# lostinc0de/sparsemat

Measured on AMD Instinct MI355X. Metric: csr_spmv_effective_hbm_GBps, higher is better.
Workload: dtype f32

## Files before the change

### include/sparsemat_hip.h

```cpp
#ifndef SPARSEMAT_HIP_H
#define SPARSEMAT_HIP_H

#include <stddef.h>
#include <stdint.h>

#ifdef __cplusplus
extern "C" {
#endif

#define SMH_ABI_VERSION 3

enum {
    SMH_OK = 0,
    SMH_ERR_DIM_MISMATCH = 1,
    SMH_ERR_NOT_SQUARE = 2,
    SMH_ERR_INDEX_RANGE = 3,
    SMH_ERR_INVALID = 4,
    SMH_ERR_HIP = 5,
    SMH_ERR_OOM = 6,
    SMH_ERR_NO_DEVICE = 7,
    SMH_ERR_CAPACITY = 8,
    SMH_ERR_COMM = 9
};

// ... 28 lines not shown
int smh_crs_create(smh_dtype dtype, size_t n_rows, size_t n_cols, size_t nnz,
                   const uint32_t *offset_rows, const uint32_t *columns, const void *values,
                   int validate, smh_crs **out);
int smh_crs_create_dev(smh_dtype dtype, size_t n_rows, size_t n_cols, size_t nnz,
                       const uint32_t *offset_rows_dev, const uint32_t *columns_dev,
                       const void *values_dev, int validate, smh_crs **out);
int smh_crs_assemble(smh_dtype dtype, size_t n_ops, const uint32_t *rows, const uint32_t *cols,
                     const void *values, const uint8_t *ops, smh_crs **out);
int smh_crs_assemble_dev(smh_dtype dtype, size_t n_ops, const uint32_t *rows_dev,
                         const uint32_t *cols_dev, const void *values_dev, const uint8_t *ops_dev,
                         smh_crs **out);
int smh_crs_replay(smh_dtype dtype, size_t n_ops, const uint32_t *rows, const uint32_t *cols,
                   const void *values, const uint8_t *ops, smh_crs **out);
int smh_crs_replay_dev(smh_dtype dtype, size_t n_ops, const uint32_t *rows_dev,
                       const uint32_t *cols_dev, const void *values_dev, const uint8_t *ops_dev,
                       smh_crs **out);
int smh_crs_transpose(const smh_crs *a, smh_crs **out);
int smh_last_transpose_route(void);
int smh_crs_column_info(const smh_crs *m, uint32_t *rows, uint32_t *col_ptr, uint32_t *entries);
int smh_crs_column_info_dev(const smh_crs *m, uint32_t *rows_dev, uint32_t *col_ptr_dev,
                            uint32_t *entries_dev);
int smh_crs_prod(const smh_crs *a, const smh_crs *b, smh_crs **out);
int smh_crs_permute(const smh_crs *a, const uint32_t *row_perm, size_t n_row_perm, const uint32_t *col_perm, size_t n_col_perm, smh_crs **out);
int smh_crs_permute_dev(const smh_crs *a, const uint32_t *row_perm_dev, size_t n_row_perm, const uint32_t *col_perm_dev, size_t n_col_perm,
                        smh_crs **out);
int smh_crs_permute_symmetric(const smh_crs *a, const uint32_t *perm, size_t n_perm, smh_crs **out);
int smh_crs_permute_symmetric_dev(const smh_crs *a, const uint32_t *perm_dev, size_t n_perm, smh_crs **out);
int smh_crs_bandwidth(const smh_crs *m, uint32_t *lower_out, uint32_t *upper_out);
int smh_crs_span_fraction(smh_crs *m, double *out);
int smh_crs_rcm(const smh_crs *m, uint32_t *perm_out, size_t *n_components_out, size_t *n_levels_out);
int smh_crs_rcm_dev(const smh_crs *m, uint32_t *perm_out_dev, size_t *n_components_out, size_t *n_levels_out);
int smh_crs_color(const smh_crs *m, uint32_t seed, uint32_t *colors_out, uint32_t *perm_out, size_t *n_colors_out, size_t *n_rounds_out);
int smh_crs_color_dev(const smh_crs *m, uint32_t seed, uint32_t *colors_out_dev, uint32_t *perm_out_dev, size_t *n_colors_out, size_t *n_rounds_out);
int smh_crs_clone(const smh_crs *a, smh_crs **out);
int smh_crs_add(const smh_crs *a, const smh_crs *b, smh_crs **out);
int smh_crs_sub(const smh_crs *a, const smh_crs *b, smh_crs **out);
int smh_crs_add_assign(smh_crs *a, const smh_crs *b);
int smh_crs_sub_assign(smh_crs *a, const smh_crs *b);
int smh_last_add_route(void);
int smh_crs_get(const smh_crs *m, size_t i, size_t j, void *value_out);
int smh_crs_get_many(const smh_crs *m, size_t n, const uint32_t *rows, const uint32_t *cols, void *values_out);
int smh_crs_get_many_dev(const smh_crs *m, size_t n, const uint32_t *rows_dev, const uint32_t *cols_dev, void *values_out_dev);
int smh_crs_apply(smh_crs *m, size_t n_ops, const uint32_t *rows, const uint32_t *cols, const void *values, const uint8_t *ops);
int smh_crs_apply_dev(smh_crs *m, size_t n_ops, const uint32_t *rows_dev, const uint32_t *cols_dev, const void *values_dev,
                      const uint8_t *ops_dev);
int smh_last_apply_route(void);
typedef struct smh_update_plan smh_update_plan;
int smh_update_plan_create(const smh_crs *m, size_t n_ops, const uint32_t *rows, const uint32_t *cols, const uint8_t *ops,
                           smh_update_plan **out);
int smh_update_plan_create_dev(const smh_crs *m, size_t n_ops, const uint32_t *rows_dev, const uint32_t *cols_dev,
                               const uint8_t *ops_dev, smh_update_plan **out);
int smh_update_plan_execute(smh_update_plan *p, smh_crs *m, const void *values, int from_zero);
int smh_update_plan_execute_dev(smh_update_plan *p, smh_crs *m, const void *values_dev, int from_zero);
int smh_update_plan_stats(const smh_update_plan *p, size_t *n_ops, size_t *n_targets, size_t *n_live_ops, size_t *longest_run,
                          size_t *long_run_threshold, size_t *device_bytes);
int smh_update_plan_destroy(smh_update_plan *p);
int smh_crs_eye(smh_dtype dtype, size_t dim, smh_crs **out);
int smh_crs_is_symmetric(const smh_crs *m, int *out);
int smh_crs_is_sorted(const smh_crs *m, int *out);
int smh_crs_sort_rows(smh_crs *m);
int smh_crs_destroy(smh_crs *m);
int smh_crs_update_values(smh_crs *m, const void *values_host);
int smh_crs_download(const smh_crs *m, uint32_t *offset_rows, uint32_t *columns, void *values);
size_t smh_crs_n_rows(const smh_crs *m);
size_t smh_crs_n_cols(const smh_crs *m);
size_t smh_crs_nnz(const smh_crs *m);
size_t smh_crs_orphans(const smh_crs *m);
int smh_crs_dtype(const smh_crs *m);
int smh_crs_max_row_len(const smh_crs *m, uint32_t *out);
int smh_crs_col_range(const smh_crs *m, uint32_t *min_out, uint32_t *max_out);
int smh_crs_scale(smh_crs *m, double a);
int smh_crs_resolved_variant(const smh_crs *m, int *variant_out, int *lanes_out);
int smh_crs_set_vector_lanes(smh_crs *m, int lanes);
int smh_crs_set_stream_xs(smh_crs *m, int mode);
int smh_crs_stream_layout(smh_crs *m, int *coded_out, int *byte_lengths_out, int *small_tiles_out, int *xs_chunks_out);
int smh_crs_stream_value_dict(smh_crs *m, int *n_values_out, void *values_out);
int smh_crs_set_stream_value_dict(smh_crs *m, int mode);
int smh_crs_set_stream_direct(smh_crs *m, int mode);
int smh_crs_stream_direct(smh_crs *m, int *direct_out);
int smh_crs_set_vector_chunks(smh_crs *m, int chunks);
int smh_crs_set_ring(smh_crs *m, int mode);
int smh_crs_ring_entries(smh_crs *m, uint32_t *out);
int smh_crs_ring_column_form(smh_crs *m, int *form_out);
int smh_crs_ring_bands(smh_crs *m, uint32_t *bands_out, uint32_t *intervals_out);
int smh_crs_ring_plan(smh_crs *m, uint32_t *n_blocks_out, size_t *n_phases_out,
                      double *ring_fraction_out, int *active_out, uint32_t *phase_ptr_out,
                      uint32_t *phases_out);
int smh_crs_ring_regular(smh_crs *m, uint32_t *len_out);

int smh_crs_set_colblock_shift(smh_crs *m, uint32_t shift);
int smh_crs_colblock(smh_crs *m, uint32_t *shift_out, size_t *n_blocks_out, int *rows_per_thread_out,
                     double *span_fraction_out, uint32_t *offsets_out, uint32_t *columns_out,
                     void *values_out);

int smh_crs_colfused(smh_crs *m, int *fits_out, uint32_t *shift_out, size_t *n_blocks_out, uint32_t *rows_per_lane_out,
                     size_t *n_tiles_out, uint32_t *tile_rows_out, uint32_t *segments_out, uint8_t *counts_out,
                     uint32_t *columns_out, void *values_out);

int smh_crs_tiled_layout(smh_crs *m, uint32_t *n_slices_out, uint32_t *slice_columns_out, uint32_t *rows_per_block_out,
                         uint32_t *n_row_blocks_out, size_t *copy_entries_out);
int smh_crs_tiled_products(smh_crs *m, size_t *n_products_out);

int smh_crs_tiled_array(smh_crs *m, int which, void *out, size_t capacity_bytes, size_t *bytes_out);

int smh_crs_colsplit(smh_crs *m, int *split_out, uint32_t *min_long_out, size_t *n_long_out, uint32_t *long_rows_out,
                     smh_crs **long_out, smh_crs **short_out);

int smh_crs_spmv(smh_crs *m, const void *x_host, size_t x_len, void *y_host, int variant);
int smh_crs_prepare(smh_crs *m, int variant);
int smh_crs_prepare_stats(smh_crs *m, int variant, double *prepare_ms_out, size_t *derived_bytes_out);
int smh_crs_spmv_dev(smh_crs *m, const void *x_dev, size_t x_len, void *y_dev, int variant,
                     void *stream);
int smh_crs_inner_prod(smh_crs *m, const void *lhs_host, size_t lhs_len, const void *rhs_host,
                       size_t rhs_len, int variant, double *out);
size_t smh_crs_merge_tiles(const smh_crs *m);
size_t smh_crs_merge_tile_items(const smh_crs *m);
int smh_crs_merge_table(smh_crs *m, uint32_t *row_out, uint32_t *nnz_out);

int smh_vec_create(smh_dtype dtype, size_t n, smh_vec **out);
int smh_vec_from_host(smh_dtype dtype, size_t n, const void *host, smh_vec **out);
int smh_vec_wrap_dev(smh_dtype dtype, size_t n, void *dev_ptr, smh_vec **out);
int smh_vec_destroy(smh_vec *v);
int smh_vec_upload(smh_vec *v, const void *host);
int smh_vec_download(const smh_vec *v, void *host);
size_t smh_vec_dim(const smh_vec *v);
int smh_vec_dtype(const smh_vec *v);
void *smh_vec_data(const smh_vec *v);
int smh_vec_copy(smh_vec *dst, const smh_vec *src);
int smh_vec_permute(smh_vec *dst, const smh_vec *src, const uint32_t *perm, size_t n_perm, int inverse);
int smh_vec_permute_dev(smh_vec *dst, const smh_vec *src, const uint32_t *perm_dev, size_t n_perm, int inverse);
int smh_vec_add(smh_vec *x, const smh_vec *y);
int smh_vec_sub(smh_vec *x, const smh_vec *y);
int smh_vec_scale(smh_vec *x, double a);
int smh_vec_axpy(smh_vec *y, double a, const smh_vec *x);
int smh_vec_xpby(smh_vec *p, double b, const smh_vec *r);
int smh_vec_dot(const smh_vec *x, const smh_vec *y, double *out);
int smh_vec_norm_squared(const smh_vec *x, double *out);
int smh_vec_norm(const smh_vec *x, double *out);
int smh_blas_dot_dev(smh_dtype dtype, const void *x_dev, const void *y_dev, size_t n, void *result_dev,
                     void *scratch_dev, void *stream);
size_t smh_blas_dot_scratch_bytes(void);
int smh_blas_axpy_dev(smh_dtype dtype, void *y_dev, const void *a_dev, const void *x_dev, size_t n, void *stream);
int smh_blas_xpby_dev(smh_dtype dtype, void *p_dev, const void *b_dev, const void *r_dev, size_t n, void *stream);
int smh_crs_spmv_vec(smh_crs *m, const smh_vec *x, smh_vec *y, int variant);
int smh_crs_inner_prod_vec(smh_crs *m, const smh_vec *lhs, const smh_vec *rhs, int variant, double *out);

int smh_mvec_create(smh_dtype dtype, size_t n, size_t k, smh_mvec **out);
int smh_mvec_from_host(smh_dtype dtype, size_t n, size_t k, const void *host, smh_mvec **out);
int smh_mvec_upload(smh_mvec *mv, const void *host);
int smh_mvec_download(const smh_mvec *mv, void *host);
int smh_mvec_destroy(smh_mvec *mv);
size_t smh_mvec_dim(const smh_mvec *mv);
size_t smh_mvec_count(const smh_mvec *mv);
size_t smh_mvec_ld(const smh_mvec *mv);
int smh_mvec_dtype(const smh_mvec *mv);
void *smh_mvec_data(const smh_mvec *mv);
int smh_mvec_set_column(smh_mvec *mv, size_t c, const smh_vec *v);
int smh_mvec_get_column(const smh_mvec *mv, size_t c, smh_vec *v);
int smh_mvec_copy(smh_mvec *dst, const smh_mvec *src);
int smh_mvec_add(smh_mvec *x, const smh_mvec *y);
int smh_mvec_sub(smh_mvec *x, const smh_mvec *y);
int smh_mvec_scale(smh_mvec *x, const double *a);
int smh_mvec_dot(const smh_mvec *x, const smh_mvec *y, double *out);
int smh_mvec_norm_squared(const smh_mvec *x, double *out);

int smh_crs_spmv_many(smh_crs *m, const smh_mvec *x, smh_mvec *y);
// ... 211 lines not shown
```

### rust/src/ffi.rs

```rust
#![allow(non_camel_case_types)]
use std::os::raw::{c_char, c_double, c_int, c_void};

#[repr(C)] pub struct smh_crs { _private: [u8; 0] }
#[repr(C)] pub struct smh_vec { _private: [u8; 0] }
#[repr(C)] pub struct smh_update_plan { _private: [u8; 0] }
#[repr(C)] pub struct smh_par { _private: [u8; 0] }
#[repr(C)] pub struct smh_par_vec { _private: [u8; 0] }
#[repr(C)] pub struct smh_comm { _private: [u8; 0] }

pub const SMH_OK: c_int = 0;
pub const SMH_ERR_DIM_MISMATCH: c_int = 1;
pub const SMH_F32: c_int = 0;
pub const SMH_F64: c_int = 1;
pub const SMH_SPMV_AUTO: c_int = 0;
pub const SMH_TRI_LOWER: c_int = 0;
pub const SMH_TRI_UPPER: c_int = 1;
pub const SMH_DIAG_NON_UNIT: c_int = 0;
pub const SMH_DIAG_UNIT: c_int = 1;
pub const SMH_PRECOND_NONE: c_int = 0;
pub const SMH_PRECOND_JACOBI: c_int = 1;
pub const SMH_PRECOND_SGS: c_int = 2;
pub const SMH_PRECOND_ILU: c_int = 3;
pub const SMH_PRECOND_FSAI: c_int = 4;
pub const SMH_INNER_CG: c_int = 0;
// ... 43 lines not shown
                                   iters_out: *mut usize, rr_out: *mut c_double, cycles_out: *mut usize, breakdown_out: *mut c_int) -> c_int;
    pub fn smh_gmres_precond_solve_vec(a: *mut smh_crs, precond: c_int, f: *mut smh_crs, b: *const smh_vec, x: *mut smh_vec,
                                       tol: c_double, iter_max: usize, restart: usize, variant: c_int, check_every: usize,
                                       iters_out: *mut usize, rr_out: *mut c_double, cycles_out: *mut usize, breakdown_out: *mut c_int) -> c_int;
    pub fn smh_bicgstab_precond_solve(a: *mut smh_crs, precond: c_int, f: *mut smh_crs, b_host: *const c_void, b_len: usize,
                                      x_host_inout: *mut c_void, x_len: usize, tol: c_double, iter_max: usize, variant: c_int,
                                      iters_out: *mut usize, rr_out: *mut c_double, breakdown_out: *mut c_int) -> c_int;
    pub fn smh_bicgstab_precond_solve_vec(a: *mut smh_crs, precond: c_int, f: *mut smh_crs, b: *const smh_vec, x: *mut smh_vec,
                                          tol: c_double, iter_max: usize, variant: c_int, check_every: usize,
                                          iters_out: *mut usize, rr_out: *mut c_double, breakdown_out: *mut c_int) -> c_int;
    pub fn smh_crs_trisolve_levels(m: *mut smh_crs, uplo: c_int, n_levels_out: *mut usize, level_of_row_out: *mut u32,
                                   n_launches_out: *mut usize, small_level_rows_out: *mut usize) -> c_int;
    pub fn smh_crs_trisolve(m: *mut smh_crs, uplo: c_int, diag: c_int, b_host: *const c_void, b_len: usize, x_host: *mut c_void,
                            x_len: usize) -> c_int;
    pub fn smh_crs_trisolve_vec(m: *mut smh_crs, uplo: c_int, diag: c_int, b: *const smh_vec, x: *mut smh_vec) -> c_int;
    pub fn smh_crs_sgs_apply_vec(m: *mut smh_crs, r: *const smh_vec, z: *mut smh_vec) -> c_int;
    pub fn smh_pcg_sgs_solve(m: *mut smh_crs, b_host: *const c_void, b_len: usize, x_host_inout: *mut c_void,
                             x_len: usize, tol: c_double, iter_max: usize, variant: c_int,
                             iters_out: *mut usize, rr_out: *mut c_double) -> c_int;
    pub fn smh_pcg_sgs_solve_vec(m: *mut smh_crs, b: *const smh_vec, x: *mut smh_vec, tol: c_double, iter_max: usize,
                                 variant: c_int, check_every: usize, iters_out: *mut usize, rr_out: *mut c_double) -> c_int;
    pub fn smh_crs_ilu0(a: *const smh_crs, f_out: *mut *mut smh_crs, zero_pivot_out: *mut usize) -> c_int;
    pub fn smh_crs_ilu0_refactor(f: *mut smh_crs, a: *const smh_crs, zero_pivot_out: *mut usize) -> c_int;
    pub fn smh_crs_ilu_apply_vec(f: *mut smh_crs, r: *const smh_vec, z: *mut smh_vec) -> c_int;
    pub fn smh_pcg_ilu_solve(a: *mut smh_crs, f: *mut smh_crs, b_host: *const c_void, b_len: usize, x_host_inout: *mut c_void,
                             x_len: usize, tol: c_double, iter_max: usize, variant: c_int,
                             iters_out: *mut usize, rr_out: *mut c_double) -> c_int;
    pub fn smh_pcg_ilu_solve_vec(a: *mut smh_crs, f: *mut smh_crs, b: *const smh_vec, x: *mut smh_vec, tol: c_double, iter_max: usize,
                                 variant: c_int, check_every: usize, iters_out: *mut usize, rr_out: *mut c_double) -> c_int;
    pub fn smh_crs_fsai(a: *const smh_crs, g_out: *mut *mut smh_crs, gt_out: *mut *mut smh_crs, not_spd_out: *mut usize) -> c_int;
    pub fn smh_crs_fsai_apply_vec(g: *mut smh_crs, gt: *mut smh_crs, r: *const smh_vec, z: *mut smh_vec) -> c_int;
    pub fn smh_pcg_fsai_solve(a: *mut smh_crs, g: *mut smh_crs, gt: *mut smh_crs, b_host: *const c_void, b_len: usize, x_host_inout: *mut c_void,
                              x_len: usize, tol: c_double, iter_max: usize, variant: c_int, iters_out: *mut usize, rr_out: *mut c_double) -> c_int;
    pub fn smh_pcg_fsai_solve_vec(a: *mut smh_crs, g: *mut smh_crs, gt: *mut smh_crs, b: *const smh_vec, x: *mut smh_vec, tol: c_double,
                                  iter_max: usize, variant: c_int, check_every: usize, iters_out: *mut usize, rr_out: *mut c_double) -> c_int;
    pub fn smh_crs_fsai_ns(a: *const smh_crs, gl_out: *mut *mut smh_crs, gu_out: *mut *mut smh_crs, singular_out: *mut usize) -> c_int;
    pub fn smh_crs_fsai_ns_apply_vec(gl: *mut smh_crs, gu: *mut smh_crs, r: *const smh_vec, z: *mut smh_vec) -> c_int;
    pub fn smh_gmres_fsai_solve(a: *mut smh_crs, g: *mut smh_crs, gt: *mut smh_crs, b_host: *const c_void, b_len: usize, x_host_inout: *mut c_void,
                                x_len: usize, tol: c_double, iter_max: usize, restart: usize, variant: c_int, iters_out: *mut usize,
                                rr_out: *mut c_double, cycles_out: *mut usize, breakdown_out: *mut c_int) -> c_int;
    pub fn smh_gmres_fsai_solve_vec(a: *mut smh_crs, g: *mut smh_crs, gt: *mut smh_crs, b: *const smh_vec, x: *mut smh_vec, tol: c_double,
                                    iter_max: usize, restart: usize, variant: c_int, check_every: usize, iters_out: *mut usize,
                                    rr_out: *mut c_double, cycles_out: *mut usize, breakdown_out: *mut c_int) -> c_int;
    pub fn smh_bicgstab_fsai_solve(a: *mut smh_crs, g: *mut smh_crs, gt: *mut smh_crs, b_host: *const c_void, b_len: usize, x_host_inout: *mut c_void,
                                   x_len: usize, tol: c_double, iter_max: usize, variant: c_int, iters_out: *mut usize, rr_out: *mut c_double,
                                   breakdown_out: *mut c_int) -> c_int;
    pub fn smh_bicgstab_fsai_solve_vec(a: *mut smh_crs, g: *mut smh_crs, gt: *mut smh_crs, b: *const smh_vec, x: *mut smh_vec, tol: c_double,
                                       iter_max: usize, variant: c_int, check_every: usize, iters_out: *mut usize, rr_out: *mut c_double,
                                       breakdown_out: *mut c_int) -> c_int;
    pub fn smh_crs_cast(a: *const smh_crs, dtype: c_int, out: *mut *mut smh_crs, overflow_out: *mut usize) -> c_int;
    pub fn smh_vec_cast(src: *const smh_vec, dst: *mut smh_vec) -> c_int;
    pub fn smh_refine_solve_vec(a: *mut smh_crs, a_lo: *mut smh_crs, inner: c_int, precond: c_int, f_lo: *mut smh_crs, f2_lo: *mut smh_crs,
                                b: *const smh_vec, x: *mut smh_vec, tol: c_double, outer_max: usize, inner_tol: c_double, inner_iter_max: usize,
                                restart: usize, variant: c_int, variant_lo: c_int, check_every: usize, outer_out: *mut usize,
                                inner_iters_out: *mut usize, rr_out: *mut c_double, code_out: *mut c_int) -> c_int;
    pub fn smh_refine_solve(a: *mut smh_crs, a_lo: *mut smh_crs, inner: c_int, precond: c_int, f_lo: *mut smh_crs, f2_lo: *mut smh_crs,
                            b_host: *const c_void, b_len: usize, x_host_inout: *mut c_void, x_len: usize, tol: c_double, outer_max: usize,
                            inner_tol: c_double, inner_iter_max: usize, restart: usize, variant: c_int, variant_lo: c_int, check_every: usize,
                            outer_out: *mut usize, inner_iters_out: *mut usize, rr_out: *mut c_double, code_out: *mut c_int) -> c_int;
    pub fn smh_crs_inner_prod(m: *mut smh_crs, lhs_host: *const c_void, lhs_len: usize, rhs_host: *const c_void,
                              rhs_len: usize, variant: c_int, out: *mut c_double) -> c_int;
    pub fn smh_crs_assemble(dtype: c_int, n_ops: usize, rows: *const u32, cols: *const u32, values: *const c_void,
                            ops: *const u8, out: *mut *mut smh_crs) -> c_int;
    pub fn smh_crs_replay(dtype: c_int, n_ops: usize, rows: *const u32, cols: *const u32, values: *const c_void,
                          ops: *const u8, out: *mut *mut smh_crs) -> c_int;
    pub fn smh_crs_transpose(a: *const smh_crs, out: *mut *mut smh_crs) -> c_int;
    pub fn smh_crs_set_stream_xs(m: *mut smh_crs, mode: c_int) -> c_int;
    pub fn smh_crs_set_stream_direct(m: *mut smh_crs, mode: c_int) -> c_int;
    pub fn smh_crs_stream_direct(m: *mut smh_crs, direct_out: *mut c_int) -> c_int;
    pub fn smh_crs_stream_layout(m: *mut smh_crs, coded_out: *mut c_int, byte_lengths_out: *mut c_int, small_tiles_out: *mut c_int, xs_chunks_out: *mut c_int) -> c_int;
    pub fn smh_last_transpose_route() -> c_int;
    pub fn smh_crs_orphans(m: *const smh_crs) -> usize;
    pub fn smh_crs_prod(a: *const smh_crs, b: *const smh_crs, out: *mut *mut smh_crs) -> c_int;
    pub fn smh_crs_clone(a: *const smh_crs, out: *mut *mut smh_crs) -> c_int;
    pub fn smh_crs_permute(a: *const smh_crs, row_perm: *const u32, n_row_perm: usize, col_perm: *const u32, n_col_perm: usize,
                           out: *mut *mut smh_crs) -> c_int;
    pub fn smh_crs_permute_dev(a: *const smh_crs, row_perm_dev: *const u32, n_row_perm: usize, col_perm_dev: *const u32,
                               n_col_perm: usize, out: *mut *mut smh_crs) -> c_int;
    pub fn smh_crs_permute_symmetric(a: *const smh_crs, perm: *const u32, n_perm: usize, out: *mut *mut smh_crs) -> c_int;
    pub fn smh_crs_permute_symmetric_dev(a: *const smh_crs, perm_dev: *const u32, n_perm: usize, out: *mut *mut smh_crs) -> c_int;
    pub fn smh_crs_bandwidth(m: *const smh_crs, lower_out: *mut u32, upper_out: *mut u32) -> c_int;
    pub fn smh_crs_span_fraction(m: *mut smh_crs, out: *mut f64) -> c_int;
    pub fn smh_crs_ring_regular(m: *mut smh_crs, len_out: *mut u32) -> c_int;
    pub fn smh_crs_rcm(m: *const smh_crs, perm_out: *mut u32, n_components_out: *mut usize, n_levels_out: *mut usize) -> c_int;
    pub fn smh_crs_rcm_dev(m: *const smh_crs, perm_out_dev: *mut u32, n_components_out: *mut usize, n_levels_out: *mut usize) -> c_int;
    pub fn smh_crs_color(m: *const smh_crs, seed: u32, colors_out: *mut u32, perm_out: *mut u32, n_colors_out: *mut usize, n_rounds_out: *mut usize) -> c_int;
    pub fn smh_crs_color_dev(m: *const smh_crs, seed: u32, colors_out_dev: *mut u32, perm_out_dev: *mut u32, n_colors_out: *mut usize, n_rounds_out: *mut usize) -> c_int;
    pub fn smh_vec_permute(dst: *mut smh_vec, src: *const smh_vec, perm: *const u32, n_perm: usize, inverse: c_int) -> c_int;
    pub fn smh_vec_permute_dev(dst: *mut smh_vec, src: *const smh_vec, perm_dev: *const u32, n_perm: usize, inverse: c_int) -> c_int;
    pub fn smh_crs_add(a: *const smh_crs, b: *const smh_crs, out: *mut *mut smh_crs) -> c_int;
    pub fn smh_crs_sub(a: *const smh_crs, b: *const smh_crs, out: *mut *mut smh_crs) -> c_int;
    pub fn smh_crs_add_assign(a: *mut smh_crs, b: *const smh_crs) -> c_int;
    pub fn smh_crs_sub_assign(a: *mut smh_crs, b: *const smh_crs) -> c_int;
    pub fn smh_last_add_route() -> c_int;
    pub fn smh_crs_get(m: *const smh_crs, i: usize, j: usize, value_out: *mut c_void) -> c_int;
    pub fn smh_crs_get_many(m: *const smh_crs, n: usize, rows: *const u32, cols: *const u32, values_out: *mut c_void) -> c_int;
    pub fn smh_crs_get_many_dev(m: *const smh_crs, n: usize, rows_dev: *const u32, cols_dev: *const u32,
                                values_out_dev: *mut c_void) -> c_int;
    pub fn smh_crs_apply(m: *mut smh_crs, n_ops: usize, rows: *const u32, cols: *const u32, values: *const c_void,
                         ops: *const u8) -> c_int;
    pub fn smh_crs_apply_dev(m: *mut smh_crs, n_ops: usize, rows_dev: *const u32, cols_dev: *const u32,
                             values_dev: *const c_void, ops_dev: *const u8) -> c_int;
    pub fn smh_last_apply_route() -> c_int;
    pub fn smh_last_solve_replays() -> c_int;
    pub fn smh_update_plan_create(m: *const smh_crs, n_ops: usize, rows: *const u32, cols: *const u32, ops: *const u8,
                                  out: *mut *mut smh_update_plan) -> c_int;
    pub fn smh_update_plan_create_dev(m: *const smh_crs, n_ops: usize, rows_dev: *const u32, cols_dev: *const u32,
                                      ops_dev: *const u8, out: *mut *mut smh_update_plan) -> c_int;
    pub fn smh_update_plan_execute(p: *mut smh_update_plan, m: *mut smh_crs, values: *const c_void, from_zero: c_int) -> c_int;
    pub fn smh_update_plan_execute_dev(p: *mut smh_update_plan, m: *mut smh_crs, values_dev: *const c_void, from_zero: c_int) -> c_int;
    pub fn smh_update_plan_stats(p: *const smh_update_plan, n_ops: *mut usize, n_targets: *mut usize, n_live_ops: *mut usize,
                                 longest_run: *mut usize, long_run_threshold: *mut usize, device_bytes: *mut usize) -> c_int;
    pub fn smh_update_plan_destroy(p: *mut smh_update_plan) -> c_int;
    pub fn smh_crs_eye(dtype: c_int, dim: usize, out: *mut *mut smh_crs) -> c_int;
    pub fn smh_crs_is_symmetric(m: *const smh_crs, out: *mut c_int) -> c_int;
    pub fn smh_crs_is_sorted(m: *const smh_crs, out: *mut c_int) -> c_int;
    pub fn smh_crs_column_info(m: *const smh_crs, rows: *mut u32, col_ptr: *mut u32, entries: *mut u32) -> c_int;
    pub fn smh_crs_sort_rows(m: *mut smh_crs) -> c_int;
    pub fn smh_par_create(dtype: c_int, n_blocks: usize, device_ids: *const c_int, n_rows: usize, n_cols: usize,
                          offset_rows: *const u32, columns: *const u32, values: *const c_void, validate: c_int,
                          out: *mut *mut smh_par) -> c_int;
    pub fn smh_par_create_split(dtype: c_int, n_blocks: usize, device_ids: *const c_int, n_rows: usize, n_cols: usize,
                                offset_rows: *const u32, columns: *const u32, values: *const c_void, validate: c_int,
                                split_mode: c_int, out: *mut *mut smh_par) -> c_int;
    pub fn smh_par_split(p: *const smh_par, rows_out: *mut usize) -> c_int;
    pub fn smh_par_set_overlap(p: *mut smh_par, on: c_int) -> c_int;
    pub fn smh_par_interior(p: *const smh_par, local_block: usize, variant: c_int, row_begin: *mut usize, row_end: *mut usize) -> c_int;
    pub fn smh_par_destroy(p: *mut smh_par) -> c_int;
    pub fn smh_par_spmv(p: *mut smh_par, x_host: *const c_void, x_len: usize, y_host: *mut c_void, variant: c_int) -> c_int;
    pub fn smh_par_cg_solve(p: *mut smh_par, b_host: *const c_void, b_len: usize, x_host_inout: *mut c_void, x_len: usize,
                            tol: c_double, iter_max: usize, variant: c_int, iters_out: *mut usize,
                            rr_out: *mut c_double) -> c_int;
    pub fn smh_par_vec_create(p: *mut smh_par, n: usize, out: *mut *mut smh_par_vec) -> c_int;
    pub fn smh_par_vec_destroy(v: *mut smh_par_vec) -> c_int;
    pub fn smh_par_vec_upload(v: *mut smh_par_vec, host: *const c_void) -> c_int;
    pub fn smh_par_vec_download(v: *const smh_par_vec, host: *mut c_void) -> c_int;
    pub fn smh_par_spmv_dev(p: *mut smh_par, x: *const smh_par_vec, y: *mut smh_par_vec, variant: c_int, exchange: c_int) -> c_int;
    pub fn smh_par_exchange(p: *mut smh_par, v: *mut smh_par_vec, mode: c_int) -> c_int;
    pub fn smh_par_synchronize(p: *mut smh_par) -> c_int;
    pub fn smh_par_cg_solve_vec(p: *mut smh_par, b: *const smh_par_vec, x: *mut smh_par_vec, tol: c_double, iter_max: usize,
                                variant: c_int, check_every: usize, iters_out: *mut usize, rr_out: *mut c_double) -> c_int;
    pub fn smh_comm_unique_id(id_out: *mut c_void) -> c_int;
    pub fn smh_comm_create(id: *const c_void, n_ranks: c_int, rank: c_int, out: *mut *mut smh_comm) -> c_int;
    pub fn smh_comm_destroy(c: *mut smh_comm) -> c_int;
    pub fn smh_par_create_rank(comm: *mut smh_comm, n_rows: usize, block: *mut smh_crs, out: *mut *mut smh_par) -> c_int;
    pub fn smh_par_create_rank_split(comm: *mut smh_comm, n_rows: usize, block: *mut smh_crs, row_begin: usize, out: *mut *mut smh_par) -> c_int;
    pub fn smh_crs_n_rows(m: *const smh_crs) -> usize;
    pub fn smh_crs_n_cols(m: *const smh_crs) -> usize;
    pub fn smh_crs_dtype(m: *const smh_crs) -> c_int;
    pub fn smh_crs_nnz(m: *const smh_crs) -> usize;
    pub fn smh_crs_download(m: *const smh_crs, offset_rows: *mut u32, columns: *mut u32, values: *mut c_void) -> c_int;
}
```

### sparsemat_amd/_lib.py

```python
import ctypes as C
import os

_HERE = os.path.dirname(os.path.abspath(__file__))
LIB_PATH = os.environ.get("SPARSEMAT_HIP_LIB") or os.path.join(_HERE, "libsparsemat_hip.so")

SMH_OK = 0
SMH_ERR_DIM_MISMATCH, SMH_ERR_NOT_SQUARE, SMH_ERR_INDEX_RANGE, SMH_ERR_INVALID = 1, 2, 3, 4
SMH_ERR_HIP, SMH_ERR_OOM, SMH_ERR_NO_DEVICE, SMH_ERR_CAPACITY, SMH_ERR_COMM = 5, 6, 7, 8, 9
SMH_F32, SMH_F64 = 0, 1
SMH_TRI_LOWER, SMH_TRI_UPPER = 0, 1
SMH_DIAG_NON_UNIT, SMH_DIAG_UNIT = 0, 1
SMH_PRECOND_NONE, SMH_PRECOND_JACOBI, SMH_PRECOND_SGS, SMH_PRECOND_ILU = 0, 1, 2, 3
PRECONDS = {None: SMH_PRECOND_NONE, "jacobi": SMH_PRECOND_JACOBI, "sgs": SMH_PRECOND_SGS, "ilu": SMH_PRECOND_ILU}
PRECOND_NAMES = tuple(PRECONDS) + ("fsai",)
SMH_INNER_CG, SMH_INNER_BICGSTAB, SMH_INNER_GMRES = 0, 1, 2
INNERS = {"cg": SMH_INNER_CG, "bicgstab": SMH_INNER_BICGSTAB, "gmres": SMH_INNER_GMRES}
SMH_PRECOND_FSAI = 4
REFINE_PRECONDS = dict(PRECONDS, fsai=SMH_PRECOND_FSAI)
UPLO = {"lower": SMH_TRI_LOWER, "upper": SMH_TRI_UPPER}
EXCHANGE_NONE, EXCHANGE_ALLGATHER, EXCHANGE_WINDOW, EXCHANGE_AUTO = 0, 1, 2, 3
EXCHANGES = {"none": EXCHANGE_NONE, "allgather": EXCHANGE_ALLGATHER, "window": EXCHANGE_WINDOW, "halo": EXCHANGE_WINDOW, "auto": EXCHANGE_AUTO}
EXCHANGE_NAMES = {EXCHANGE_NONE: "none", EXCHANGE_ALLGATHER: "allgather", EXCHANGE_WINDOW: "window", EXCHANGE_AUTO: "auto"}
PAR_BACKEND_AUTO, PAR_BACKEND_PEER, PAR_BACKEND_RCCL = 0, 1, 2
PAR_BACKENDS = {"auto": PAR_BACKEND_AUTO, "peer": PAR_BACKEND_PEER, "rccl": PAR_BACKEND_RCCL}
COMM_ID_BYTES = 128
SPMV_AUTO, SPMV_VECTOR, SPMV_MERGE, SPMV_SEQ, SPMV_STREAM, SPMV_COLBLOCK, SPMV_COLFUSED, SPMV_COLSPLIT, SPMV_TILED = 0, 1, 2, 3, 4, 5, 6, 7, 8
VARIANTS = {"auto": SPMV_AUTO, "vector": SPMV_VECTOR, "merge": SPMV_MERGE, "seq": SPMV_SEQ, "stream": SPMV_STREAM,
            "colblock": SPMV_COLBLOCK, "colfused": SPMV_COLFUSED, "colsplit": SPMV_COLSPLIT, "tiled": SPMV_TILED}

_sz = C.c_size_t
_vp = C.c_void_p
_u32p = C.POINTER(C.c_uint32)
_int = C.c_int

SIGNATURES = {
    "smh_abi_version": (_int, []),
    "smh_last_error": (C.c_char_p, []),
    "smh_status_string": (C.c_char_p, [_int]),
    "smh_device_count": (_int, [C.POINTER(_int)]),
    "smh_set_device": (_int, [_int]),
    "smh_device_synchronize": (_int, []),
    "smh_crs_create": (_int, [_int, _sz, _sz, _sz, _vp, _vp, _vp, _int, C.POINTER(_vp)]),
    "smh_crs_create_dev": (_int, [_int, _sz, _sz, _sz, _vp, _vp, _vp, _int, C.POINTER(_vp)]),
    "smh_crs_assemble": (_int, [_int, _sz, _vp, _vp, _vp, _vp, C.POINTER(_vp)]),
    "smh_crs_assemble_dev": (_int, [_int, _sz, _vp, _vp, _vp, _vp, C.POINTER(_vp)]),
    "smh_crs_replay": (_int, [_int, _sz, _vp, _vp, _vp, _vp, C.POINTER(_vp)]),
    "smh_crs_replay_dev": (_int, [_int, _sz, _vp, _vp, _vp, _vp, C.POINTER(_vp)]),
    "smh_crs_transpose": (_int, [_vp, C.POINTER(_vp)]),
    "smh_crs_column_info": (_int, [_vp, _vp, _vp, _vp]),
    "smh_crs_column_info_dev": (_int, [_vp, _vp, _vp, _vp]),
    "smh_crs_prod": (_int, [_vp, _vp, C.POINTER(_vp)]),
    "smh_crs_permute": (_int, [_vp, _vp, _sz, _vp, _sz, C.POINTER(_vp)]),
    "smh_crs_permute_dev": (_int, [_vp, _vp, _sz, _vp, _sz, C.POINTER(_vp)]),
    "smh_crs_permute_symmetric": (_int, [_vp, _vp, _sz, C.POINTER(_vp)]),
    "smh_crs_permute_symmetric_dev": (_int, [_vp, _vp, _sz, C.POINTER(_vp)]),
    "smh_crs_bandwidth": (_int, [_vp, _u32p, _u32p]),
    "smh_crs_span_fraction": (_int, [_vp, C.POINTER(C.c_double)]),
    "smh_crs_rcm": (_int, [_vp, _vp, C.POINTER(_sz), C.POINTER(_sz)]),
    "smh_crs_rcm_dev": (_int, [_vp, _vp, C.POINTER(_sz), C.POINTER(_sz)]),
    "smh_crs_color": (_int, [_vp, C.c_uint32, _vp, _vp, C.POINTER(_sz), C.POINTER(_sz)]),
    "smh_crs_color_dev": (_int, [_vp, C.c_uint32, _vp, _vp, C.POINTER(_sz), C.POINTER(_sz)]),
    "smh_vec_permute": (_int, [_vp, _vp, _vp, _sz, _int]),
    "smh_vec_permute_dev": (_int, [_vp, _vp, _vp, _sz, _int]),
    "smh_crs_clone": (_int, [_vp, C.POINTER(_vp)]),
    "smh_crs_add": (_int, [_vp, _vp, C.POINTER(_vp)]),
    "smh_crs_sub": (_int, [_vp, _vp, C.POINTER(_vp)]),
    "smh_crs_add_assign": (_int, [_vp, _vp]),
    "smh_crs_sub_assign": (_int, [_vp, _vp]),
    "smh_last_add_route": (_int, []),
    "smh_crs_get": (_int, [_vp, _sz, _sz, _vp]),
    "smh_crs_get_many": (_int, [_vp, _sz, _vp, _vp, _vp]),
    "smh_crs_get_many_dev": (_int, [_vp, _sz, _vp, _vp, _vp]),
    "smh_crs_apply": (_int, [_vp, _sz, _vp, _vp, _vp, _vp]),
    "smh_crs_apply_dev": (_int, [_vp, _sz, _vp, _vp, _vp, _vp]),
    "smh_last_apply_route": (_int, []),
    "smh_last_solve_replays": (_int, []),
    "smh_update_plan_create": (_int, [_vp, _sz, _vp, _vp, _vp, _vp]),
    "smh_update_plan_create_dev": (_int, [_vp, _sz, _vp, _vp, _vp, _vp]),
    "smh_update_plan_execute": (_int, [_vp, _vp, _vp, _int]),
    "smh_update_plan_execute_dev": (_int, [_vp, _vp, _vp, _int]),
    "smh_update_plan_stats": (_int, [_vp, _vp, _vp, _vp, _vp, _vp, _vp]),
    "smh_update_plan_destroy": (_int, [_vp]),
    "smh_crs_eye": (_int, [_int, _sz, C.POINTER(_vp)]),
    "smh_crs_is_symmetric": (_int, [_vp, C.POINTER(_int)]),
    "smh_crs_is_sorted": (_int, [_vp, C.POINTER(_int)]),
    "smh_crs_sort_rows": (_int, [_vp]),
    "smh_crs_destroy": (_int, [_vp]),
    "smh_crs_update_values": (_int, [_vp, _vp]),
    "smh_crs_download": (_int, [_vp, _vp, _vp, _vp]),
    "smh_crs_n_rows": (_sz, [_vp]),
    "smh_crs_n_cols": (_sz, [_vp]),
    "smh_crs_nnz": (_sz, [_vp]),
    "smh_crs_orphans": (_sz, [_vp]),
    "smh_crs_dtype": (_int, [_vp]),
    "smh_crs_max_row_len": (_int, [_vp, _u32p]),
    "smh_crs_col_range": (_int, [_vp, _u32p, _u32p]),
    "smh_crs_scale": (_int, [_vp, C.c_double]),
    "smh_crs_resolved_variant": (_int, [_vp, C.POINTER(_int), C.POINTER(_int)]),
    "smh_crs_set_vector_lanes": (_int, [_vp, _int]),
    "smh_crs_set_vector_chunks": (_int, [_vp, _int]),
    "smh_crs_set_ring": (_int, [_vp, _int]),
    "smh_crs_ring_entries": (_int, [_vp, _u32p]),
    "smh_crs_ring_column_form": (_int, [_vp, C.POINTER(_int)]),
    "smh_crs_ring_bands": (_int, [_vp, _u32p, _vp]),
    "smh_crs_ring_regular": (_int, [_vp, _vp]),
    "smh_crs_ring_plan": (_int, [_vp, _u32p, C.POINTER(_sz), C.POINTER(C.c_double), C.POINTER(_int), _vp, _vp]),
    "smh_crs_set_colblock_shift": (_int, [_vp, C.c_uint32]),
    "smh_crs_tiled_layout": (_int, [_vp, _u32p, _u32p, _u32p, _u32p, C.POINTER(_sz)]),
    "smh_crs_tiled_products": (_int, [_vp, C.POINTER(_sz)]),
    "smh_crs_prepare_stats": (_int, [_vp, _int, C.POINTER(C.c_double), C.POINTER(_sz)]),
    "smh_crs_tiled_array": (_int, [_vp, _int, _vp, _sz, C.POINTER(_sz)]),
    "smh_crs_colblock": (_int, [_vp, _u32p, C.POINTER(_sz), C.POINTER(_int), C.POINTER(C.c_double), _vp, _vp, _vp]),
    "smh_crs_colfused": (_int, [_vp, C.POINTER(_int), _u32p, C.POINTER(_sz), _u32p, C.POINTER(_sz), _vp, _vp, _vp, _vp, _vp]),
    "smh_crs_colsplit": (_int, [_vp, C.POINTER(_int), _u32p, C.POINTER(_sz), _vp, C.POINTER(_vp), C.POINTER(_vp)]),
    "smh_crs_spmv": (_int, [_vp, _vp, _sz, _vp, _int]),
    "smh_crs_spmv_dev": (_int, [_vp, _vp, _sz, _vp, _int, _vp]),
    "smh_crs_prepare": (_int, [_vp, _int]),
    "smh_crs_merge_tiles": (_sz, [_vp]),
    "smh_crs_merge_tile_items": (_sz, [_vp]),
    "smh_crs_merge_table": (_int, [_vp, _vp, _vp]),
    "smh_vec_create": (_int, [_int, _sz, C.POINTER(_vp)]),
    "smh_vec_from_host": (_int, [_int, _sz, _vp, C.POINTER(_vp)]),
    "smh_vec_wrap_dev": (_int, [_int, _sz, _vp, C.POINTER(_vp)]),
    "smh_vec_destroy": (_int, [_vp]),
    "smh_vec_upload": (_int, [_vp, _vp]),
    "smh_vec_download": (_int, [_vp, _vp]),
    "smh_vec_dim": (_sz, [_vp]),
    "smh_vec_dtype": (_int, [_vp]),
    "smh_vec_data": (_vp, [_vp]),
    "smh_vec_copy": (_int, [_vp, _vp]),
    "smh_vec_add": (_int, [_vp, _vp]),
    "smh_vec_sub": (_int, [_vp, _vp]),
    "smh_vec_scale": (_int, [_vp, C.c_double]),
    "smh_vec_axpy": (_int, [_vp, C.c_double, _vp]),
    "smh_vec_xpby": (_int, [_vp, C.c_double, _vp]),
    "smh_vec_dot": (_int, [_vp, _vp, C.POINTER(C.c_double)]),
    "smh_vec_norm_squared": (_int, [_vp, C.POINTER(C.c_double)]),
    "smh_vec_norm": (_int, [_vp, C.POINTER(C.c_double)]),
    "smh_blas_dot_dev": (_int, [_int, _vp, _vp, _sz, _vp, _vp, _vp]),
    "smh_blas_dot_scratch_bytes": (_sz, []),
    "smh_blas_axpy_dev": (_int, [_int, _vp, _vp, _vp, _sz, _vp]),
    "smh_blas_xpby_dev": (_int, [_int, _vp, _vp, _vp, _sz, _vp]),
    "smh_crs_spmv_vec": (_int, [_vp, _vp, _vp, _int]),
    "smh_crs_inner_prod": (_int, [_vp, _vp, _sz, _vp, _sz, _int, C.POINTER(C.c_double)]),
    "smh_crs_inner_prod_vec": (_int, [_vp, _vp, _vp, _int, C.POINTER(C.c_double)]),
    "smh_mvec_create": (_int, [_int, _sz, _sz, C.POINTER(_vp)]),
    "smh_mvec_from_host": (_int, [_int, _sz, _sz, _vp, C.POINTER(_vp)]),
    "smh_mvec_upload": (_int, [_vp, _vp]),
    "smh_mvec_download": (_int, [_vp, _vp]),
    "smh_mvec_destroy": (_int, [_vp]),
    "smh_mvec_dim": (_sz, [_vp]),
    "smh_mvec_count": (_sz, [_vp]),
    "smh_mvec_ld": (_sz, [_vp]),
    "smh_mvec_dtype": (_int, [_vp]),
    "smh_mvec_data": (_vp, [_vp]),
    "smh_mvec_set_column": (_int, [_vp, _sz, _vp]),
    "smh_mvec_get_column": (_int, [_vp, _sz, _vp]),
    "smh_mvec_copy": (_int, [_vp, _vp]),
    "smh_mvec_add": (_int, [_vp, _vp]),
    "smh_mvec_sub": (_int, [_vp, _vp]),
    "smh_mvec_scale": (_int, [_vp, C.POINTER(C.c_double)]),
    "smh_mvec_dot": (_int, [_vp, _vp, C.POINTER(C.c_double)]),
    "smh_mvec_norm_squared": (_int, [_vp, C.POINTER(C.c_double)]),
    "smh_crs_spmv_many": (_int, [_vp, _vp, _vp]),
    "smh_crs_spmv_many_dev": (_int, [_vp, _vp, _sz, _vp, _sz, _sz, _vp]),
    "smh_crs_spmv_many_host": (_int, [_vp, _vp, _sz, _sz, _vp]),
    "smh_cg_solve": (_int, [_vp, _vp, _sz, _vp, _sz, C.c_double, _sz, _int, C.POINTER(_sz),
                            C.POINTER(C.c_double)]),
    "smh_cg_solve_vec": (_int, [_vp, _vp, _vp, C.c_double, _sz, _int, _sz, C.POINTER(_sz),
                                C.POINTER(C.c_double)]),
    "smh_cg_solve_many": (_int, [_vp, _vp, _vp, C.c_double, _sz, _sz, C.POINTER(_sz), C.POINTER(C.c_double)]),
    "smh_cg_solve_many_host": (_int, [_vp, _vp, _sz, _sz, _vp, C.c_double, _sz, C.POINTER(_sz), C.POINTER(C.c_double)]),
    "smh_pcg_jacobi_solve": (_int, [_vp, _vp, _sz, _vp, _sz, C.c_double, _sz, _int, C.POINTER(_sz),
                                    C.POINTER(C.c_double)]),
    "smh_crs_trisolve_levels": (_int, [_vp, _int, C.POINTER(_sz), _vp, C.POINTER(_sz), C.POINTER(_sz)]),
    "smh_crs_trisolve": (_int, [_vp, _int, _int, _vp, _sz, _vp, _sz]),
    "smh_crs_trisolve_vec": (_int, [_vp, _int, _int, _vp, _vp]),
    "smh_crs_sgs_apply_vec": (_int, [_vp, _vp, _vp]),
    "smh_pcg_sgs_solve": (_int, [_vp, _vp, _sz, _vp, _sz, C.c_double, _sz, _int, C.POINTER(_sz),
                                 C.POINTER(C.c_double)]),
    "smh_pcg_sgs_solve_vec": (_int, [_vp, _vp, _vp, C.c_double, _sz, _int, _sz, C.POINTER(_sz),
                                     C.POINTER(C.c_double)]),
    "smh_crs_ilu0": (_int, [_vp, C.POINTER(_vp), C.POINTER(_sz)]),
    "smh_crs_ilu0_refactor": (_int, [_vp, _vp, C.POINTER(_sz)]),
    "smh_crs_ilu_apply_vec": (_int, [_vp, _vp, _vp]),
    "smh_pcg_ilu_solve": (_int, [_vp, _vp, _vp, _sz, _vp, _sz, C.c_double, _sz, _int, C.POINTER(_sz),
# ... 174 lines not shown
```

### sparsemat_amd/build.py

```python
import os
import subprocess
import sys

HERE = os.path.dirname(os.path.abspath(__file__))
CSRC = os.path.join(HERE, "csrc")
LIB = os.path.join(HERE, "libsparsemat_hip.so")
SOURCES = ["capi.hip", "crs_forms.hip", "spmv_dispatch.hip", "spmv_vector.hip", "spmv_ring.hip", "spmv_ring2.hip", "spmv_stream.hip", "spmv_stream_xd.hip", "spmv_many.hip", "mvec.hip", "mvec_blas.hip", "cg_many.hip","spmv_colblock.hip", "spmv_colfused.hip", "spmv_colsplit.hip", "spmv_tiled.hip", "spmv_merge.hip", "blas1.hip", "cg.hip", "synth.hip", "assemble.hip", "matops.hip", "matadd.hip", "matupdate.hip", "matplan.hip", "par.hip", "pcg.hip", "trisolve.hip", "bicgstab.hip", "gmres.hip", "pool.hip", "transpose_bucket.hip", "permute.hip", "reorder.hip", "color.hip", "ilu.hip", "fsai.hip", "refine.hip"]
HEADERS = [os.path.join(CSRC, "internal.hpp"), os.path.join(CSRC, "crs_forms.hpp"), os.path.join(CSRC, "mvec_tree.hpp"), os.path.join(CSRC, "ring_col12.hpp"), os.path.join(CSRC, "solver_tree.hpp"), os.path.join(CSRC, "solver_host.hpp"), os.path.join(CSRC, "precond.hpp"), os.path.join(HERE, "..", "include", "sparsemat_hip.h")]
FLAGS = ["-O3", "-std=c++17", "--offload-arch=gfx950", "-fPIC", "-Wall", "-Wno-unused-function",
         "-fno-gpu-rdc", "-ffp-contract=off"]


def hipcc():
    for cand in (os.environ.get("HIPCC"), "/opt/rocm/bin/hipcc", "hipcc"):
        if cand and (os.path.isabs(cand) and os.path.exists(cand) or not os.path.isabs(cand)):
            return cand
    raise RuntimeError("hipcc not found")


def stale():
    if not os.path.exists(LIB):
        return True
    t = os.path.getmtime(LIB)
    deps = [os.path.join(CSRC, s) for s in SOURCES] + HEADERS + [os.path.abspath(__file__)]
    return any(os.path.getmtime(d) > t for d in deps)


def build(force=False, verbose=False, extra_flags=(), out=None, objsuffix=""):
    global LIB
    lib = out or LIB
    if out is None and not force and not stale():
        return LIB
    objdir = os.path.join(HERE, "csrc", "_obj" + objsuffix)
    os.makedirs(objdir, exist_ok=True)
    objs = []
    procs = []
    for s in SOURCES:
        o = os.path.join(objdir, s.replace(".hip", ".o"))
        objs.append(o)
        cmd = [hipcc()] + FLAGS + list(extra_flags) + ["-c", os.path.join(CSRC, s), "-o", o]
        if verbose:
            print(" ".join(cmd))
        procs.append((s, subprocess.Popen(cmd, stdout=subprocess.PIPE, stderr=subprocess.STDOUT)))
    failed = []
    for s, p in procs:
        log, _ = p.communicate()
        if p.returncode != 0:
            failed.append((s, log.decode(errors="replace")))
        elif verbose and log:
            print(log.decode(errors="replace"))
    if failed:
        raise RuntimeError("hipcc failed:\n" + "\n".join("%s:\n%s" % f for f in failed))
    cmd = [hipcc(), "--offload-arch=gfx950", "-shared", "-fPIC", "-o", lib] + objs + ["-L/opt/rocm/lib", "-lrccl", "-Wl,-rpath,/opt/rocm/lib"]
    subprocess.check_call(cmd)
    return lib


if __name__ == "__main__":
    print(build(force="--force" in sys.argv, verbose=True))
```

### sparsemat_amd/csrc/capi.hip

```cpp
#include <atomic>
#include <chrono>
#include <cmath>
#include <cstdarg>
#include <cstdlib>
#include <cstring>
#include <new>
#include <thread>
#include <vector>

#include "crs_forms.hpp"
#include "solver_host.hpp"

namespace smh {

static thread_local char g_err[512] = "";

void set_error(const char *fmt, ...) {
    va_list ap;
    va_start(ap, fmt);
    vsnprintf(g_err, sizeof g_err, fmt, ap);
    va_end(ap);
}

void clear_error() { g_err[0] = 0; }
// ... 976 lines not shown
    SMH_TRY(build_eye(dtype, dim, arrays.off, arrays.col, arrays.val, nullptr));
    return wrap_arrays(dtype, nullptr, dim, dim, dim, arrays, 0, out);
}

int smh_crs_is_symmetric(const smh_crs *m, int *out) {
    if (!m || !out) return fail(SMH_ERR_INVALID, "NULL argument");
    return crs_is_symmetric(m->dtype, m->d_off, m->d_col, m->d_val, m->n_rows, out, m->stream);
}

int smh_crs_is_sorted(const smh_crs *m, int *out) {
    if (!m || !out) return fail(SMH_ERR_INVALID, "NULL argument");
    return crs_is_sorted(m->d_off, m->d_col, m->n_rows, out, m->stream);
}

int smh_crs_sort_rows(smh_crs *m) {
    if (!m) return fail(SMH_ERR_INVALID, "NULL handle");
    SMH_TRY(sort_rows(m->dtype, m->d_off, m->d_col, m->d_val, m->n_rows, m->nnz, m->max_col, m->stream));
    invalidate(m, Changed::Order);
    ++m->epoch;
    return SMH_OK;
}

int smh_crs_destroy(smh_crs *m) {
    if (!m) return SMH_OK;
    if (m->stream) { (void)hipStreamSynchronize(m->stream); (void)hipStreamDestroy(m->stream); }
    if (m->owns) { (void)hipFree(m->d_off); (void)hipFree(m->d_col); (void)hipFree(m->d_val); }
    (void)hipGetLastError();
    delete m;
    return SMH_OK;
}

int smh_crs_update_values(smh_crs *m, const void *values_host) {
    if (!m) return fail(SMH_ERR_INVALID, "NULL argument");
    if (m->nnz && values_host) SMH_HIP(hipMemcpy(m->d_val, values_host, m->nnz * dtype_size(m->dtype), hipMemcpyHostToDevice));
    invalidate(m, Changed::Values);
    if (m->codes.state != Form::NotTried && m->codes.direct) {
        StreamCfg c;
        SMH_TRY(stream_cfg(m, &c, true));
    }
    return SMH_OK;
}

int smh_crs_download(const smh_crs *m, uint32_t *offset_rows, uint32_t *columns, void *values) {
    if (!m) return fail(SMH_ERR_INVALID, "NULL handle");
    SMH_HIP(hipStreamSynchronize(m->stream));
    if (offset_rows) SMH_HIP(hipMemcpy(offset_rows, m->d_off, (m->n_rows + 1) * sizeof(uint32_t), hipMemcpyDeviceToHost));
    if (columns && m->nnz) SMH_HIP(hipMemcpy(columns, m->d_col, m->nnz * sizeof(uint32_t), hipMemcpyDeviceToHost));
    if (values && m->nnz) SMH_HIP(hipMemcpy(values, m->d_val, m->nnz * dtype_size(m->dtype), hipMemcpyDeviceToHost));
    return SMH_OK;
}

size_t smh_crs_n_rows(const smh_crs *m) { return m ? m->n_rows : 0; }
size_t smh_crs_n_cols(const smh_crs *m) { return m ? m->n_cols : 0; }
size_t smh_crs_nnz(const smh_crs *m) { return m ? m->nnz : 0; }
size_t smh_crs_orphans(const smh_crs *m) { return m ? m->orphans : 0; }
int smh_crs_dtype(const smh_crs *m) { return m ? m->dtype : -1; }

int smh_crs_max_row_len(const smh_crs *m, uint32_t *out) {
    if (!m || !out) return fail(SMH_ERR_INVALID, "NULL argument");
    *out = m->max_row_len;
    return SMH_OK;
}

int smh_crs_col_range(const smh_crs *m, uint32_t *min_out, uint32_t *max_out) {
    if (!m) return fail(SMH_ERR_INVALID, "NULL handle");
    if (min_out) *min_out = m->min_col;
    if (max_out) *max_out = m->max_col;
    return SMH_OK;
}

int smh_crs_scale(smh_crs *m, double a) {
    if (!m) return fail(SMH_ERR_INVALID, "NULL handle");
    SMH_TRY(launch_scale_values(m->dtype, m->d_val, m->nnz, a, m->stream));
    if (m->has_first_op) {
        Scratch scr;
        char *d = nullptr;
        SMH_TRY(scr.alloc(&d, 16));
        SMH_HIP(hipMemcpyAsync(d, &m->first_val_bits, 8, hipMemcpyHostToDevice, m->stream));
        SMH_TRY(launch_scale_values(m->dtype, d, 1, a, m->stream));
        SMH_HIP(hipMemcpyAsync(&m->first_val_bits, d, 8, hipMemcpyDeviceToHost, m->stream));
        SMH_HIP(hipStreamSynchronize(m->stream));
    }
    if (m->dict.state == Form::Ready) SMH_TRY(launch_scale_values(m->dtype, m->dict.values.get(), 32, a, m->stream));
    if (m->cb.state == Form::Ready) SMH_TRY(launch_scale_values(m->dtype, m->cb.val.get(), m->nnz, a, m->stream));
    if (m->cf.state == Form::Ready) SMH_TRY(launch_scale_values(m->dtype, m->cf.val.get(), m->nnz, a, m->stream));
    if (m->tiled.state == Form::Ready) SMH_TRY(launch_scale_values(m->dtype, m->tiled.val.get(), (size_t)m->tiled.tot, a, m->stream));
    if (m->split.state == Form::Ready) {
        SMH_TRY(smh_crs_scale(m->split.long_part, a));
        SMH_TRY(smh_crs_scale(m->split.short_part, a));
    }
    SMH_HIP(hipStreamSynchronize(m->stream));
    return SMH_OK;
}

int smh_crs_tiled_layout(smh_crs *m, uint32_t *n_slices_out, uint32_t *slice_columns_out, uint32_t *rows_per_block_out, uint32_t *n_row_blocks_out,
                         size_t *copy_entries_out) {
    if (!m) return fail(SMH_ERR_INVALID, "NULL handle");
    SMH_TRY(tiled_build(m));
    if (n_slices_out) *n_slices_out = m->tiled.n_cb;
    if (slice_columns_out) *slice_columns_out = tiled_slice_columns(m->dtype);
    if (rows_per_block_out) *rows_per_block_out = m->tiled.R;
    if (n_row_blocks_out) *n_row_blocks_out = m->tiled.n_rb;
    if (copy_entries_out) *copy_entries_out = (size_t)m->tiled.tot;
    return SMH_OK;
}

int smh_crs_tiled_products(smh_crs *m, size_t *n_products_out) {
    if (!m) return fail(SMH_ERR_INVALID, "NULL handle");
    SMH_TRY(tiled_build(m));
    if (n_products_out) *n_products_out = (size_t)m->tiled.n_prod;
    return SMH_OK;
}

int smh_crs_tiled_array(smh_crs *m, int which, void *out, size_t capacity_bytes, size_t *bytes_out) {
    if (!m) return fail(SMH_ERR_INVALID, "NULL handle");
    SMH_TRY(tiled_build(m));
    return tiled_array(m, which, out, capacity_bytes, bytes_out);
}

int smh_crs_set_colblock_shift(smh_crs *m, uint32_t shift) {
    if (!m) return fail(SMH_ERR_INVALID, "NULL handle");
    if (shift > 31) return fail(SMH_ERR_INVALID, "column block shift must be 0 (automatic) or 1..31");
    if (shift != m->knobs.cb_forced_shift) invalidate(m, Changed::BlockWidth);
    m->knobs.cb_forced_shift = shift;
    return SMH_OK;
}

int smh_crs_colblock(smh_crs *m, uint32_t *shift_out, size_t *n_blocks_out, int *rows_per_thread_out,
                     double *span_fraction_out, uint32_t *offsets_out, uint32_t *columns_out, void *values_out) {
    if (!m) return fail(SMH_ERR_INVALID, "NULL handle");
    SMH_TRY(ensure_ring_plan(m, false));
    SMH_TRY(ensure_colblock(m));
    if (shift_out) *shift_out = m->cb.shift;
    if (n_blocks_out) *n_blocks_out = m->cb.blocks;
    if (rows_per_thread_out) *rows_per_thread_out = m->cb.rpt;
    if (span_fraction_out) *span_fraction_out = m->span_fraction;
    if (offsets_out)
        SMH_HIP(hipMemcpy(offsets_out, m->cb.off.get(), m->cb.blocks * (m->n_rows + 1) * sizeof(uint32_t), hipMemcpyDeviceToHost));
    if (columns_out && m->nnz) SMH_HIP(hipMemcpy(columns_out, m->cb.col.get(), m->nnz * sizeof(uint32_t), hipMemcpyDeviceToHost));
    if (values_out && m->nnz) SMH_HIP(hipMemcpy(values_out, m->cb.val.get(), m->nnz * dtype_size(m->dtype), hipMemcpyDeviceToHost));
    return SMH_OK;
}

int smh_crs_colfused(smh_crs *m, int *fits_out, uint32_t *shift_out, size_t *n_blocks_out, uint32_t *rows_per_lane_out,
                     size_t *n_tiles_out, uint32_t *tile_rows_out, uint32_t *segments_out, uint8_t *counts_out, uint32_t *columns_out,
                     void *values_out) {
    if (!m) return fail(SMH_ERR_INVALID, "NULL handle");
    SMH_TRY(ensure_colfused(m));
    const size_t tile_rows = (size_t)64 * m->cf.rt, n_tiles = (m->cf.state == Form::Ready) ? m->cf.tiles : 0;
    if (fits_out) *fits_out = (m->cf.state == Form::Ready) ? 1 : 0;
    if (shift_out) *shift_out = m->cf.shift;
    if (n_blocks_out) *n_blocks_out = m->cf.blocks;
    if (rows_per_lane_out) *rows_per_lane_out = m->cf.rt;
    if (n_tiles_out) *n_tiles_out = n_tiles;
    if (m->cf.state != Form::Ready) return SMH_OK;
    SMH_HIP(hipStreamSynchronize(m->stream));
    if (tile_rows_out) SMH_HIP(hipMemcpy(tile_rows_out, m->cf.tile_row.get(), (n_tiles + 1) * sizeof(uint32_t), hipMemcpyDeviceToHost));
    if (segments_out) SMH_HIP(hipMemcpy(segments_out, m->cf.seg.get(), (n_tiles * m->cf.blocks + 1) * sizeof(uint32_t), hipMemcpyDeviceToHost));
    if (counts_out && n_tiles) SMH_HIP(hipMemcpy(counts_out, m->cf.cnt.get(), n_tiles * m->cf.blocks * tile_rows, hipMemcpyDeviceToHost));
    if (columns_out && m->nnz) SMH_HIP(hipMemcpy(columns_out, m->cf.col.get(), m->nnz * sizeof(uint32_t), hipMemcpyDeviceToHost));
    if (values_out && m->nnz) SMH_HIP(hipMemcpy(values_out, m->cf.val.get(), m->nnz * dtype_size(m->dtype), hipMemcpyDeviceToHost));
    return SMH_OK;
}

int smh_crs_colsplit(smh_crs *m, int *split_out, uint32_t *min_long_out, size_t *n_long_out, uint32_t *long_rows_out, smh_crs **long_out,
                     smh_crs **short_out) {
// ... 32 lines not shown
}

int smh_crs_stream_direct(smh_crs *m, int *direct_out) {
    if (!m || !direct_out) return fail(SMH_ERR_INVALID, "NULL argument");
    StreamCfg c;
    SMH_TRY(stream_cfg(m, &c));
    *direct_out = c.direct && c.xs != 0;
    return SMH_OK;
}

int smh_crs_stream_value_dict(smh_crs *m, int *n_values_out, void *values_out) {
    if (!m || !n_values_out) return fail(SMH_ERR_INVALID, "NULL argument");
    StreamCfg c;
    SMH_TRY(stream_cfg(m, &c));
    *n_values_out = c.dict ? (int)m->dict.n : 0;
    if (c.dict && values_out) {
        SMH_HIP(hipMemcpyAsync(values_out, m->dict.values.get(), (size_t)m->dict.n * dtype_size(m->dtype), hipMemcpyDeviceToHost, m->stream));
        SMH_HIP(hipStreamSynchronize(m->stream));
    }
    return SMH_OK;
}

int smh_crs_set_stream_value_dict(smh_crs *m, int mode) {
    if (!m) return fail(SMH_ERR_INVALID, "NULL handle");
    if (mode < -1 || mode > 0) return fail(SMH_ERR_INVALID, "mode must be -1 (automatic: whenever the values allow) or 0 (never)");
    m->knobs.use_stream_vdict = mode;
    return recode_stream(m);
}

int smh_crs_stream_layout(smh_crs *m, int *coded_out, int *byte_lengths_out, int *small_tiles_out, int *xs_chunks_out) {
    if (!m) return fail(SMH_ERR_INVALID, "NULL handle");
    StreamCfg c;
    SMH_TRY(stream_cfg(m, &c));
    if (coded_out) *coded_out = c.code && c.cwin;
    if (byte_lengths_out) *byte_lengths_out = c.len8 && c.tbase;
    if (small_tiles_out) *small_tiles_out = c.small;
    if (xs_chunks_out) *xs_chunks_out = c.xs;
    return SMH_OK;
}

int smh_crs_set_vector_chunks(smh_crs *m, int chunks) {
    if (!m) return fail(SMH_ERR_INVALID, "NULL handle");
    if (chunks < 0 || chunks > 3) return fail(SMH_ERR_INVALID, "chunks per lane must be 0 (automatic), 1, 2 or 3");
    m->knobs.forced_chunks = chunks;
    return SMH_OK;
}

int smh_crs_set_ring(smh_crs *m, int mode) {
    if (!m) return fail(SMH_ERR_INVALID, "NULL handle");
    if (mode < -1 || mode > 1) return fail(SMH_ERR_INVALID, "ring mode must be -1 (auto), 0 (plain K1) or 1 (K1r)");
    m->knobs.use_ring = mode;
    return SMH_OK;
}

int smh_crs_ring_plan(smh_crs *m, uint32_t *n_blocks_out, size_t *n_phases_out, double *ring_fraction_out,
                      int *active_out, uint32_t *phase_ptr_out, uint32_t *phases_out) {
    if (!m) return fail(SMH_ERR_INVALID, "NULL handle");
    SMH_TRY(ensure_ring_plan(m));
    bool ring = false;
    SMH_TRY(vector_uses_ring(m, &ring));
    if (n_blocks_out) *n_blocks_out = m->ring.blocks;
    if (n_phases_out) *n_phases_out = m->ring.n_phases;
    if (ring_fraction_out) *ring_fraction_out = m->ring.fraction;
    if (active_out) *active_out = ring ? 1 : 0;
    if (phase_ptr_out)
        SMH_HIP(hipMemcpy(phase_ptr_out, m->ring.phase_ptr.get(), (m->ring.blocks + 1) * sizeof(uint32_t), hipMemcpyDeviceToHost));
    if (phases_out && m->ring.n_phases)
        SMH_HIP(hipMemcpy(phases_out, m->ring.phases.get(), m->ring.n_phases * sizeof(RingPhase), hipMemcpyDeviceToHost));
    return SMH_OK;
}

int smh_crs_ring_regular(smh_crs *m, uint32_t *len_out) {
    if (!m || !len_out) return fail(SMH_ERR_INVALID, "NULL argument");
    SMH_TRY(ensure_ring_plan(m));
    if (m->ring.n_phases)
        SMH_HIP(hipMemcpy(len_out, m->ring.reg_len.get(), m->ring.n_phases * sizeof(uint32_t), hipMemcpyDeviceToHost));
    return SMH_OK;
}

int smh_crs_ring_column_form(smh_crs *m, int *form_out) {
    if (!m || !form_out) return fail(SMH_ERR_INVALID, "NULL argument");
    bool ring = false;
    SMH_TRY(vector_uses_ring(m, &ring));
    *form_out = !ring ? 0 : m->ring.lo8.get() ? 2 : m->ring.col16.get() ? 1 : 0;
    return SMH_OK;
}

int smh_crs_ring_entries(smh_crs *m, uint32_t *out) {
    if (!m || !out) return fail(SMH_ERR_INVALID, "NULL argument");
    SMH_TRY(ensure_ring_plan(m));
    *out = m->ring.entries;
    return SMH_OK;
}

int smh_crs_ring_bands(smh_crs *m, uint32_t *bands_out, uint32_t *intervals_out) {
    if (!m || !bands_out) return fail(SMH_ERR_INVALID, "NULL argument");
    SMH_TRY(ensure_ring_plan(m));
    *bands_out = m->ring.bands;
    if (intervals_out && m->ring.bands == 4 && m->ring.win.get())
        SMH_HIP(hipMemcpy(intervals_out, m->ring.win.get(), ((m->n_rows + 63) / 64) * 8 * sizeof(uint32_t), hipMemcpyDeviceToHost));
    return SMH_OK;
}

int smh_crs_set_vector_lanes(smh_crs *m, int lanes) {
    if (!m) return fail(SMH_ERR_INVALID, "NULL handle");
    if (lanes != 0 && (lanes < 1 || lanes > 64 || (lanes & (lanes - 1))))
        return fail(SMH_ERR_INVALID, "lanes per row must be 0 or a power of two in 1..64");
    m->knobs.forced_lanes = lanes;
    return SMH_OK;
}

int smh_crs_prepare(smh_crs *m, int variant) {
    if (!m) return fail(SMH_ERR_INVALID, "NULL handle");
    const auto t0 = std::chrono::steady_clock::now();
    const long long b0 = pool_thread_net_bytes();
    int rc = prepare_forms(m, variant);
    if (rc == SMH_OK && m->stream) {
        const hipError_t e = hipStreamSynchronize(m->stream);
        if (e != hipSuccess) rc = hip_fail(e, "hipStreamSynchronize", __FILE__, __LINE__);
    }
    m->prepare_ms += std::chrono::duration<double, std::milli>(std::chrono::steady_clock::now() - t0).count();
    m->prepare_bytes += pool_thread_net_bytes() - b0;
    return rc;
}

int smh_crs_prepare_stats(smh_crs *m, int variant, double *prepare_ms_out, size_t *derived_bytes_out) {
    if (!m) return fail(SMH_ERR_INVALID, "NULL handle");
    SMH_TRY(smh_crs_prepare(m, variant));
    if (prepare_ms_out) *prepare_ms_out = m->create_ms + m->prepare_ms;
    if (derived_bytes_out) *derived_bytes_out = (size_t)(m->prepare_bytes + m->create_bytes > 0 ? m->prepare_bytes + m->create_bytes : 0);
    return SMH_OK;
}

int smh_crs_spmv_dev(smh_crs *m, const void *x_dev, size_t x_len, void *y_dev, int variant, void *stream) {
    if (!m) return fail(SMH_ERR_INVALID, "NULL handle");
    if (m->n_rows && (!y_dev || (m->nnz && !x_dev))) return fail(SMH_ERR_INVALID, "NULL device vector");
    return spmv_enqueue(m, x_dev, x_len, y_dev, variant, (hipStream_t)stream);
}

int smh_crs_spmv(smh_crs *m, const void *x_host, size_t x_len, void *y_host, int variant) {
    if (!m) return fail(SMH_ERR_INVALID, "NULL handle");
    if (m->n_rows == 0) return SMH_OK;
    if (!y_host || (x_len && !x_host)) return fail(SMH_ERR_INVALID, "NULL host vector");
    const size_t vs = dtype_size(m->dtype);
    SMH_TRY(m->stage_x.ensure_cap(x_len * vs));
    SMH_TRY(m->stage_y.ensure_cap(m->n_rows * vs));
    if (x_len) SMH_HIP(hipMemcpyAsync(m->stage_x.d.get(), x_host, x_len * vs, hipMemcpyHostToDevice, m->stream));
    SMH_TRY(spmv_enqueue(m, m->stage_x.d.get(), x_len, m->stage_y.d.get(), variant, m->stream));
    SMH_HIP(hipMemcpyAsync(y_host, m->stage_y.d.get(), m->n_rows * vs, hipMemcpyDeviceToHost, m->stream));
    SMH_HIP(hipStreamSynchronize(m->stream));
    return SMH_OK;
}

size_t smh_crs_merge_tiles(const smh_crs *m) {
    if (!m) return 0;
    return (size_t)(((uint64_t)m->n_rows + m->nnz + kMergeTile - 1) / kMergeTile);
}

size_t smh_crs_merge_tile_items(const smh_crs *) { return kMergeTile; }

int smh_crs_merge_table(smh_crs *m, uint32_t *row_out, uint32_t *nnz_out) {
    if (!m || !row_out || !nnz_out) return fail(SMH_ERR_INVALID, "NULL argument");
    SMH_TRY(ensure_merge_ws(m));
    if (m->merge.n_tiles == 0) { row_out[0] = 0; nnz_out[0] = 0; return SMH_OK; }
    SMH_HIP(hipMemcpy(row_out, m->merge.tile_row.get(), (m->merge.n_tiles + 1) * sizeof(uint32_t), hipMemcpyDeviceToHost));
    SMH_HIP(hipMemcpy(nnz_out, m->merge.tile_nz.get(), (m->merge.n_tiles + 1) * sizeof(uint32_t), hipMemcpyDeviceToHost));
    return SMH_OK;
// ... 366 lines not shown
```

### sparsemat_amd/csrc/crs_forms.hip

```cpp
#include <cstdlib>
#include <cstring>
#include <vector>

#include "crs_forms.hpp"

namespace smh {

void build_ring_plan(size_t n_rows, size_t ring_entries, const uint32_t *cmin, const uint32_t *cmax, size_t n_blocks,
                     uint32_t noring_mode, std::vector<uint32_t> &phase_ptr, std::vector<RingPhase> &phases,
                     double *ring_row_fraction);
void build_ring_plan_banded(size_t n_rows, size_t ring_entries, const uint32_t *win, size_t n_blocks, uint32_t noring_mode,
                            std::vector<uint32_t> &phase_ptr, std::vector<RingPhase> &phases, double *ring_row_fraction);

int ensure_merge_ws(smh_crs *m) {
    if (m->merge.state == Form::Ready) return SMH_OK;
    MergeTable t;
    const uint64_t items = (uint64_t)m->n_rows + (uint64_t)m->nnz;
    t.n_tiles = (size_t)((items + kMergeTile - 1) / kMergeTile);
    if (t.n_tiles) {
        SMH_TRY(t.tile_row.alloc(t.n_tiles + 1));
        SMH_TRY(t.tile_nz.alloc(t.n_tiles + 1));
        SMH_TRY(t.carry_row.alloc(t.n_tiles));
        SMH_TRY(t.carry_val.alloc(t.n_tiles * dtype_size(m->dtype)));
        SMH_TRY(launch_merge_table(m->d_off, m->n_rows, m->nnz, t.n_tiles, t.tile_row.get(), t.tile_nz.get(), m->stream));
        SMH_HIP(hipStreamSynchronize(m->stream));
    }
    t.state = Form::Ready;
    m->merge = std::move(t);
    return SMH_OK;
}

int ensure_ring_plan(smh_crs *m, bool with_bands) {
    if (m->ring.state == Form::Ready && (!with_bands || m->ring.bands_tried)) return SMH_OK;
    m->ring = RingPlan();
    RingPlan p;
    p.bands_tried = with_bands;
    const size_t n_tiles = (m->n_rows + 63) / 64;
    int cus = 256;
    hipDeviceProp_t prop;
    if (hipGetDeviceProperties(&prop, m->device) == hipSuccess && prop.multiProcessorCount > 0) cus = prop.multiProcessorCount;
    unsigned per_cu = 6;
    if (const char *e = getenv("SMH_RING_BLOCKS_PER_CU")) {
        const int v = atoi(e);
        if (v >= 1 && v <= 64) per_cu = (unsigned)v;
    }
    unsigned blocks = per_cu * (unsigned)cus;
    blocks = (blocks + 7u) & ~7u;
    std::vector<uint32_t> cmin(n_tiles), cmax(n_tiles);
    if (n_tiles) {
        Scratch scr;
        uint32_t *d_min = nullptr, *d_max = nullptr;
        SMH_TRY(scr.alloc(&d_min, n_tiles));
        SMH_TRY(scr.alloc(&d_max, n_tiles));
        SMH_TRY(read_back(d_min, cmin.data(), n_tiles, m->stream, [&](uint32_t *) -> int {
            SMH_TRY(launch_tile_span(m->d_off, m->d_col, m->n_rows, n_tiles, d_min, d_max, m->stream));
            SMH_HIP(hipMemcpyAsync(cmax.data(), d_max, n_tiles * sizeof(uint32_t), hipMemcpyDeviceToHost, m->stream));
            return SMH_OK;
        }));
    }
    double span_fraction = 0.0;
    {
        double acc = 0.0;
        size_t used = 0;
        for (size_t t = 0; t < n_tiles; ++t)
            if (cmin[t] <= cmax[t]) { acc += (double)(cmax[t] - cmin[t]) + 1.0; ++used; }
        span_fraction = used && m->n_cols ? acc / (double)used / (double)m->n_cols : 0.0;
    }
    std::vector<uint32_t> phase_ptr;
    std::vector<RingPhase> phases;
    uint32_t noring_mode = 0;
    if (const char *e = getenv("SMH_GATHER_NT")) noring_mode = atoi(e) ? 2u : 0u;
    build_ring_plan(m->n_rows, kRingEntries, cmin.data(), cmax.data(), blocks, noring_mode, phase_ptr, phases,
                    &p.fraction);
    p.entries = kRingEntries;
    const char *wide_env = getenv("SMH_RING_WIDE");
    if (m->dtype == SMH_F32 && p.fraction < 0.5 && !(wide_env && atoi(wide_env) == 0)) {
        std::vector<uint32_t> phase_ptr_w;
        std::vector<RingPhase> phases_w;
        double frac_w = 0.0;
        const unsigned blocks_w = ((blocks / 2) + 7u) & ~7u;
        build_ring_plan(m->n_rows, kRingEntriesWide, cmin.data(), cmax.data(), blocks_w, noring_mode, phase_ptr_w, phases_w, &frac_w);
        if (frac_w >= 0.5) {
            phase_ptr.swap(phase_ptr_w);
            phases.swap(phases_w);
            p.fraction = frac_w;
            p.entries = kRingEntriesWide;
            blocks = blocks_w;
// ... 133 lines not shown
int ensure_split(smh_crs *m) {
    if (m->split.state != Form::NotTried) return SMH_OK;
    SMH_TRY(columns_within_n_cols(m, "row-length split"));
    m->split.state = Form::Refused;
    if (m->no_split || m->n_rows == 0 || m->nnz == 0) return SMH_OK;
    RowSplit sp;
    size_t nnz_long = 0;
    uint32_t *rows = nullptr;
    CrsArrays long_part, short_part;
    SMH_TRY(build_colsplit(m->dtype, m->d_off, m->d_col, m->d_val, m->n_rows, m->nnz, kSplitMinLong, &sp.n_long, &nnz_long, &rows, &long_part.off,
                           &long_part.col, &long_part.val, &short_part.off, &short_part.col, &short_part.val, m->stream));
    sp.rows.reset(rows);
    const bool worth = sp.n_long > 0 && sp.n_long * 4 <= m->n_rows && nnz_long * 4 >= m->nnz;
    if (!worth) return SMH_OK;
    auto part = [&](size_t n_rows, size_t nnz, CrsArrays &arrays, uint32_t shift, smh_crs **out) -> int {
        SMH_TRY(wrap_arrays(m->dtype, nullptr, n_rows, m->n_cols, nnz, arrays, 0, out));
        (*out)->no_split = true;
        (*out)->knobs.cb_forced_shift = shift;
        return SMH_OK;
    };
    SMH_TRY(part(sp.n_long, nnz_long, long_part, 18u, &sp.long_part));
    SMH_TRY(part(m->n_rows, m->nnz - nnz_long, short_part, 19u, &sp.short_part));
    SMH_TRY(sp.y.alloc(sp.n_long * dtype_size(m->dtype)));
    SMH_HIP(hipStreamCreateWithFlags(&sp.side, hipStreamNonBlocking));
    SMH_HIP(hipEventCreateWithFlags(&sp.fork, hipEventDisableTiming));
    SMH_HIP(hipEventCreateWithFlags(&sp.join, hipEventDisableTiming));
    sp.state = Form::Ready;
    m->split = std::move(sp);
    return SMH_OK;
}
RowSplit::~RowSplit() {
    (void)smh_crs_destroy(long_part);
    (void)smh_crs_destroy(short_part);
    rows.reset();
    y.reset();
    if (side) { (void)hipStreamSynchronize(side); (void)hipStreamDestroy(side); }
    if (fork) (void)hipEventDestroy(fork);
    if (join) (void)hipEventDestroy(join);
}

static int ensure_stream_codes(smh_crs *m) {
    if (m->codes.state != Form::NotTried) return SMH_OK;
    StreamCodes c;
    c.state = Form::Refused;
    const size_t n_tiles = (m->n_rows + kStreamRows - 1) / kStreamRows;
    if (n_tiles && m->nnz) {
        uint32_t h_count = 0;
        SMH_TRY(c.cwin.alloc(n_tiles * 8));
        SMH_TRY(read_back(&h_count, 1, m->stream, [&](uint32_t *d_count) {
            return launch_stream_windows(m->d_off, m->d_col, m->n_rows, c.cwin.get(), d_count, m->stream);
        }));
        if ((size_t)h_count == n_tiles) c.state = Form::Ready;
        else c.cwin.reset();
    }
    if (c.state == Form::Ready) {
        const size_t n_out = ((m->nnz + 3) & ~size_t(3)) + 4;
        SMH_TRY(c.code.alloc(n_out));
        SMH_HIP(hipMemsetAsync(c.code.get(), 0, n_out * sizeof(uint16_t), m->stream));
        SMH_TRY(launch_stream_codes(m->d_off, m->d_col, c.cwin.get(), m->n_rows, c.code.get(), m->stream));
        if (m->max_row_len <= 255u) {
            SMH_TRY(c.len8.alloc(n_tiles * kStreamRows));
            SMH_TRY(c.tbase.alloc(n_tiles + 1));
            SMH_TRY(launch_stream_len8(m->d_off, m->n_rows, c.len8.get(), c.tbase.get(), m->stream));
            uint32_t h_xs[2] = {0xFFFFFFFFu, 0};
            SMH_TRY(read_back(h_xs, 2, m->stream, [&](uint32_t *d_xs) { return launch_stream_xs_stats(c.cwin.get(), n_tiles, d_xs, m->stream); }));
            c.xs_chunks = h_xs[0];
            c.xs_end = h_xs[1];
            unsigned long long h_odd = 0;
            SMH_TRY(read_back(&h_odd, 1, m->stream, [&](unsigned long long *d_odd) {
                return launch_stream_odd_rows(c.len8.get(), n_tiles * kStreamRows, d_odd, m->stream);
            }));
            c.odd_rows = (uint64_t)h_odd;
        }
        SMH_HIP(hipStreamSynchronize(m->stream));
    }
    m->codes = std::move(c);
    return SMH_OK;
}

static void drop_ring_col12(smh_crs *m) {
    m->ring.lo8.reset();
    m->ring.hdr.reset();
    m->ring.escapes.reset();
}
static int ensure_ring_col12(smh_crs *m, bool forced, bool *use) {
    RingPlan &r = m->ring;
    *use = forced || r.c12 == Form::Ready;
    if (r.c12 != Form::NotTried && (!*use || r.lo8.get())) return SMH_OK;
    Scratch scr;
    uint32_t *jobs = nullptr;
    unsigned long long *d_counts = nullptr, h_counts[2] = {0, 0};
    SMH_TRY(scr.alloc(&jobs, 2 * r.n_phases));
    SMH_TRY(scr.alloc(&d_counts, 2));
    SMH_TRY(read_back(d_counts, h_counts, 2, m->stream, [&](unsigned long long *d) {
        return launch_col12_count(m->d_off, m->d_col, m->nnz, r.phases.get(), r.n_phases, jobs, d, m->stream);
    }));
    r.c12_chunks = h_counts[0];
    r.c12_escapes = h_counts[1];
    r.c12 = r.c12_escapes * 1024ull <= r.c12_chunks ? Form::Ready : Form::Refused;
    *use = forced || r.c12 == Form::Ready;
    if (!*use) return SMH_OK;
    const size_t n_chunks_out = ((m->nnz + 3) >> 2) + 1;
    DevArray<uint8_t> lo8;
    DevArray<uint16_t> hdr;
    DevArray<uint32_t> escapes;
    SMH_TRY(lo8.alloc(n_chunks_out * 4));
    SMH_TRY(hdr.alloc(n_chunks_out));
    SMH_TRY(escapes.alloc(2 * (size_t)(r.c12_escapes ? r.c12_escapes : 1)));
    SMH_TRY(launch_col12_encode(m->d_col, m->nnz, jobs, r.n_phases, n_chunks_out, lo8.get(), hdr.get(), escapes.get(), d_counts, m->stream));
    SMH_HIP(hipStreamSynchronize(m->stream));
    r.lo8 = std::move(lo8);
    r.hdr = std::move(hdr);
    r.escapes = std::move(escapes);
    return SMH_OK;
}

int vector_uses_ring(smh_crs *m, bool *out) {
    *out = false;
    if (m->knobs.use_ring == 0 || m->n_rows == 0) return SMH_OK;
    SMH_TRY(ensure_ring_plan(m));
    *out = true;
    int want = m->knobs.use_col16;
    if (const char *e = getenv("SMH_RING_COL16")) want = atoi(e) ? 1 : 0;
    int want12 = m->knobs.use_col12;
    if (const char *e = getenv("SMH_RING_COL12")) want12 = strcmp(e, "auto") == 0 ? -1 : (atoi(e) ? 1 : 0);
    const bool can12 = m->dtype == SMH_F32 && m->ring.bands == 1 && m->ring.entries == (unsigned)kRingEntries && m->nnz > 0;
    bool use12 = can12 && (want12 == 1 || (want12 < 0 && want < 0 && m->ring.fraction >= 0.25));
    if (use12) SMH_TRY(ensure_ring_col12(m, want12 == 1, &use12));
    if (!use12) drop_ring_col12(m);
    const bool use16 = m->ring.bands == 4 || want == 1 || (want < 0 && m->ring.fraction >= 0.25);
    if (use16 && !m->ring.col16.get() && m->nnz) {
        const size_t n_out = ((m->nnz + 3) & ~size_t(3)) + 4;
        DevArray<uint16_t> col16;
        SMH_TRY(col16.alloc(n_out));
        if (m->ring.bands == 4) {
            SMH_HIP(hipMemsetAsync(col16.get(), 0, n_out * sizeof(uint16_t), m->stream));
            SMH_TRY(launch_ring_band_codes(m->d_off, m->d_col, m->ring.win.get(), m->n_rows, m->ring.entries / 4, col16.get(), m->stream));
        } else {
            SMH_TRY(launch_narrow_columns(m->d_col, m->nnz, col16.get(), n_out, m->stream));
        }
        SMH_HIP(hipStreamSynchronize(m->stream));
        m->ring.col16 = std::move(col16);
    } else if (!use16) {
        m->ring.col16.reset();
    }
    return SMH_OK;
}

void invalidate(smh_crs *m, Changed what) {
    m->cb = ColBlock();
    m->cf = ColFused();
    m->split = RowSplit();
    m->tiled = Tiled();
    if (what == Changed::Values) m->dict.state = Form::NotTried;
    if (what == Changed::Order) {
        m->codes = StreamCodes();
        m->ring.col16.reset();
        drop_ring_col12(m);
        m->ring.c12 = Form::NotTried;
        m->tri[0] = TriSchedule();
        m->tri[1] = TriSchedule();
    }
}

static int stream_rpt(const smh_crs *m) {
    int want = m->knobs.stream_rows_per_thread;
    if (const char *e = getenv("SMH_STREAM_RPT")) want = atoi(e);
    return want == 2 && m->max_tile512_entries <= (uint32_t)kStreamCap ? 2 : 1;
}

int stream_cfg(smh_crs *m, StreamCfg *c, bool recode) {
    *c = StreamCfg();
    c->rpt = stream_rpt(m);
    c->single_pass = m->have_stats && (c->rpt == 2 || m->max_tile_entries <= (uint32_t)kStreamCap);
    const char *c16_env = getenv("SMH_STREAM_C16");
    if (!(c16_env && atoi(c16_env) == 0) && c->rpt == 1 && c->single_pass) {
        const bool first = m->codes.state == Form::NotTried;
        SMH_TRY(ensure_stream_codes(m));
        if (first) recode = true;
        c->code = m->codes.code.get();
        c->cwin = m->codes.code.get() ? m->codes.cwin.get() : nullptr;
        static const bool l8_off = getenv("SMH_STREAM_L8") && atoi(getenv("SMH_STREAM_L8")) == 0;
        if (c->cwin && !l8_off) { c->len8 = m->codes.len8.get(); c->tbase = m->codes.tbase.get(); }
        static const bool small_off = getenv("SMH_STREAM_SMALL") && atoi(getenv("SMH_STREAM_SMALL")) == 0;
        c->small = !small_off && m->have_stats && m->max_tile_entries <= (uint32_t)kStreamCapSmall;
        static const bool xs_off = getenv("SMH_STREAM_XS") && atoi(getenv("SMH_STREAM_XS")) == 0;
        const bool forced = m->knobs.use_stream_xs == 1;
        const size_t x_bytes = m->n_cols * dtype_size(m->dtype);
        const bool on2 = forced || x_bytes >= ((size_t)1 << 20), on4 = forced || (x_bytes >= ((size_t)8 << 20) && m->dtype == SMH_F32);
        c->xs = (xs_off || m->knobs.use_stream_xs == 0 || !c->small || !c->len8) ? 0
                : (m->codes.xs_chunks <= 2u * kBlock && on2) ? 2
                : (m->codes.xs_chunks <= 4u * kBlock && on4) ? 4 : 0;
        static const bool xd_off = getenv("SMH_STREAM_XD") && atoi(getenv("SMH_STREAM_XD")) == 0;
        const bool want_direct = c->code && c->xs != 0 && !xd_off && m->knobs.use_stream_direct != 0 &&
                                 (m->knobs.use_stream_direct == 1 || 2 * m->codes.odd_rows >= (uint64_t)m->n_rows);
        static const bool vd_off = getenv("SMH_STREAM_VDICT") && atoi(getenv("SMH_STREAM_VDICT")) == 0;
        bool want_vdict = want_direct && !vd_off && m->knobs.use_stream_vdict != 0 && m->dict.state != Form::Refused;
        bool dict_rebuilt = false;
        if (recode && want_vdict && m->dict.state == Form::NotTried) {
            if (!m->dict.values.get()) SMH_TRY(m->dict.values.alloc(32 * dtype_size(m->dtype)));
            SMH_HIP(hipDeviceSynchronize());
            uint32_t n_vals = 0;
            SMH_TRY(stream_value_dict(m->dtype, m->d_val, m->nnz, m->dict.values.get(), &n_vals, m->stream));
            m->dict.n = n_vals;
            m->dict.state = n_vals ? Form::Ready : Form::Refused;
            dict_rebuilt = true;
        }
        want_vdict = want_vdict && m->dict.state == Form::Ready && m->dict.n <= stream_value_dict_capacity(c->xs);
        const bool form_ok = want_direct == m->codes.direct && want_vdict == m->codes.vdict && (!want_vdict || m->codes.vdict_xs == c->xs) &&
                             !(dict_rebuilt && (want_vdict || m->codes.vdict));
        if (recode && c->code && !form_ok) {
            SMH_HIP(hipDeviceSynchronize());
            if (want_direct)
                SMH_TRY(launch_stream_stage_codes(m->d_off, m->d_col, m->codes.cwin.get(), m->n_rows, (uint32_t)dtype_size(m->dtype), m->codes.code.get(), m->stream));
            else
                SMH_TRY(launch_stream_codes(m->d_off, m->d_col, m->codes.cwin.get(), m->n_rows, m->codes.code.get(), m->stream));
            if (want_vdict)
                SMH_TRY(launch_stream_value_codes(m->dtype, m->d_val, m->nnz, m->dict.values.get(), m->dict.n, c->xs, m->codes.code.get(), m->stream));
            SMH_HIP(hipStreamSynchronize(m->stream));
            m->codes.direct = want_direct;
            m->codes.vdict = want_vdict;
            m->codes.vdict_xs = want_vdict ? c->xs : 0;
        }
        c->direct = c->code && m->codes.direct;
        c->dict = c->direct && m->codes.vdict ? m->dict.values.get() : nullptr;
        c->dict_high = c->dict && stream_value_dict_high(m->dtype, m->dict.n, m->codes.vdict_xs);
    }
    return SMH_OK;
}

int recode_stream(smh_crs *m) {
    if (m->codes.state == Form::NotTried) return SMH_OK;
    StreamCfg c;
    return stream_cfg(m, &c, true);
}

}
// ... 1 lines not shown
```

### sparsemat_amd/csrc/crs_forms.hpp

```cpp
#pragma once
#include "internal.hpp"

namespace smh {

void clear_error();
int wrap_arrays(int dtype, const ::smh_crs *like, size_t n_rows, size_t n_cols, size_t nnz, CrsArrays &arrays, int validate, ::smh_crs **out);

template <typename U, typename F> int read_back(U *d, U *host, size_t count, hipStream_t s, F &&launch) {
    SMH_TRY(launch(d));
    SMH_HIP(hipMemcpyAsync(host, d, count * sizeof(U), hipMemcpyDeviceToHost, s));
    SMH_HIP(hipStreamSynchronize(s));
    return SMH_OK;
}
template <typename U, typename F> int read_back(U *host, size_t count, hipStream_t s, F &&launch) {
    Scratch scr;
    U *d = nullptr;
    SMH_TRY(scr.alloc(&d, count));
    return read_back(d, host, count, s, launch);
}

extern const uint32_t kSplitMinLong;
int ensure_merge_ws(::smh_crs *m);
int ensure_ring_plan(::smh_crs *m, bool with_bands = true);
int ensure_colblock(::smh_crs *m);
int ensure_colfused(::smh_crs *m);
int ensure_split(::smh_crs *m);
int vector_uses_ring(::smh_crs *m, bool *out);
enum class Changed { Values, Order, BlockWidth };
void invalidate(::smh_crs *m, Changed what);
struct StreamCfg {
    int rpt = 1;
    bool single_pass = false;
    const uint16_t *code = nullptr;
    const uint32_t *cwin = nullptr;
    const uint8_t *len8 = nullptr;
    const uint32_t *tbase = nullptr;
    bool small = false;
    int xs = 0;
    bool direct = false;
    const void *dict = nullptr;
    bool dict_high = false;
};
int stream_cfg(::smh_crs *m, StreamCfg *c, bool recode = false);
int recode_stream(::smh_crs *m);

extern const size_t kColblockMinXBytes;
uint32_t cb_shift_for(const ::smh_crs *m);
uint32_t cf_shift_for(const ::smh_crs *m);
size_t blocks_for(size_t n_cols, uint32_t shift);
int auto_lanes(const ::smh_crs *m);
int resolve_variant(const ::smh_crs *m, int variant);
int prepare_forms(::smh_crs *m, int variant);
int spmv_inner_prod(::smh_crs *m, const void *d_lhs, const void *d_rhs, size_t rhs_len, int variant, void *scratch, void *res);

}
```

### sparsemat_amd/csrc/internal.hpp

```cpp
#pragma once
#include <hip/hip_runtime.h>

#include <cstddef>
#include <cstdint>
#include <cstdio>
#include <cstring>
#include <string>
#include <utility>
#include <vector>

#include "../../include/sparsemat_hip.h"

namespace smh {

void set_error(const char *fmt, ...);
int fail(int status, const char *fmt, ...);
int hip_fail(hipError_t e, const char *what, const char *file, int line);

extern __thread bool t_thread_counted;
extern __thread int t_solve_replays;
void count_thread();
inline void note_thread() { if (!t_thread_counted) count_thread(); }
bool capture_enter();
void capture_leave();
// ... 342 lines not shown
                      bool reverse_rows, bool all_set, bool repeats_adjacent, size_t *n_rows_out, size_t *n_cols_out, size_t *nnz_out,
                      uint32_t **off_out, uint32_t **col_out, void **val_out, hipStream_t s);
int expand_rows(const uint32_t *off, size_t n_rows, uint32_t *rows_out, hipStream_t s);
int column_lists_bucketed(const uint32_t *off, const uint32_t *col, size_t n_rows, size_t n_cols, size_t nnz, uint32_t max_col, uint32_t *col_ptr,
                          uint32_t *entries, bool *done, hipStream_t s);
int transpose_bucketed(int dtype, const uint32_t *off, const uint32_t *col, const void *val, size_t n_rows, size_t nnz, uint32_t max_col,
                       uint32_t **off_out, uint32_t **col_out, void **val_out, size_t *n_rows_out, size_t *n_cols_out, bool *done, hipStream_t s);
int append_to_row(int dtype, uint32_t *off, uint32_t **col, void **val, size_t n_rows, size_t *nnz, size_t row, uint32_t column,
                  const void *value_host, hipStream_t s);
int column_info(const uint32_t *off, const uint32_t *col, size_t n_rows, size_t n_cols, size_t nnz, uint32_t max_col, uint32_t *rows,
                uint32_t *col_ptr, uint32_t *entries, hipStream_t s);
int sort_rows(int dtype, const uint32_t *off, uint32_t *col, void *val, size_t n_rows, size_t nnz, uint32_t max_col,
              hipStream_t s);
int crs_is_sorted(const uint32_t *off, const uint32_t *col, size_t n_rows, int *out, hipStream_t s);
int crs_is_symmetric(int dtype, const uint32_t *off, const uint32_t *col, const void *val, size_t n_rows, int *out, hipStream_t s);
int prod_crs(int dtype, const uint32_t *a_off, const uint32_t *a_col, const void *a_val, size_t a_rows, size_t a_nnz, uint32_t a_max_col,
             const uint32_t *b_off, const uint32_t *b_col, const void *b_val, size_t b_rows, size_t *n_rows_out, size_t *n_cols_out,
             size_t *nnz_out, uint32_t **off_out, uint32_t **col_out, void **val_out, hipStream_t s);
struct AddOperand {
    const uint32_t *off = nullptr, *col = nullptr;
    const void *val = nullptr;
    size_t n_rows = 0, n_cols = 0, nnz = 0, orphans = 0;
    uint32_t max_row_len = 0, max_col = 0;
};
struct AddResult {
    size_t n_rows = 0, n_cols = 0, nnz = 0;
    CrsArrays arrays;
    int route = 0;
    bool values_only = false;
};
int add_crs(int dtype, bool subtract, const AddOperand &a, const AddOperand &b, bool in_place, bool alias, bool force_general, AddResult *res,
            hipStream_t s);
struct UpdMatrix {
    const uint32_t *off = nullptr, *col = nullptr;
    void *val = nullptr;
    size_t n_rows = 0, n_cols = 0, nnz = 0, orphans = 0;
    uint32_t max_row_len = 0;
};
struct UpdResult {
    size_t n_rows = 0, n_cols = 0, nnz = 0;
    CrsArrays arrays;
    int route = 0;
    bool values_only = false;
};
int crs_get_many(int dtype, const UpdMatrix &m, size_t n, const uint32_t *rows, const uint32_t *cols, void *values_out, hipStream_t s);
int crs_apply(int dtype, const UpdMatrix &m, size_t n, const uint32_t *rows, const uint32_t *cols, const void *vals, const uint8_t *ops,
              bool force_general, UpdResult *res, hipStream_t s);
int build_eye(int dtype, size_t dim, uint32_t *off, uint32_t *col, void *val, hipStream_t s);
int validate_permutation(const uint32_t *perm, size_t n, uint32_t *first, const char *what, hipStream_t s);
int permute_crs(int dtype, const uint32_t *a_off, const uint32_t *a_col, const void *a_val, size_t n_rows, size_t nnz, const uint32_t *row_perm,
                const uint32_t *col_inv, CrsArrays *out, hipStream_t s);
int launch_vec_permute(int dtype, void *dst, const void *src, const uint32_t *perm, size_t n, bool inverse, hipStream_t s);
int launch_bandwidth(const uint32_t *off, const uint32_t *col, size_t n_rows, uint32_t *d_out2, hipStream_t s);
int rcm_order(const uint32_t *off, const uint32_t *col, size_t n, size_t nnz, uint32_t *perm_out, size_t *n_components, size_t *n_levels, hipStream_t s);
int symmetrised_pattern(const uint32_t *off, const uint32_t *col, size_t n, size_t nnz, Scratch &scr, uint32_t **adj_off_out, uint32_t **adj_col_out,
                        hipStream_t s);
int color_order(const uint32_t *off, const uint32_t *col, size_t n, size_t nnz, uint32_t seed, uint32_t *colors_out, uint32_t *perm_out, size_t *n_colors,
                size_t *n_rounds, hipStream_t s);
constexpr uint32_t kPlanLongRun = 64;
struct UpdPlan {
    size_t n_ops = 0, n_targets = 0, n_live = 0, longest_run = 0, n_short = 0, device_bytes = 0;
    DevArray<uint32_t> pos;
    DevArray<uint32_t> off;
    DevArray<uint32_t> tgt;
    DevArray<uint32_t> setbits;
};
int crs_plan_targets(const UpdMatrix &m, size_t n, const uint32_t *rows, const uint32_t *cols, uint32_t *key_out, uint32_t *src_out,
                     uint64_t *n_absent_out, hipStream_t s);
int plan_build(size_t n, const uint32_t *key, const uint32_t *src, const uint8_t *ops, UpdPlan *plan, hipStream_t s);
int plan_execute(int dtype, const UpdPlan &plan, const void *values, void *m_val, bool from_zero, hipStream_t s);
struct RingPhase {
    uint32_t row_begin, row_end;
    uint32_t load_lo, load_hi;
    uint32_t use_ring;
    uint32_t band_lo[3], band_hi[3];
};
constexpr int kRingPhaseWords = 11;
int launch_tile_span(const uint32_t *off, const uint32_t *col, size_t n_rows, size_t n_tiles, uint32_t *cmin,
                     uint32_t *cmax, hipStream_t s);
struct RingCol12 {
    const uint8_t *lo8 = nullptr;
    const uint16_t *hdr = nullptr;
    const uint32_t *escapes = nullptr;
};
int launch_spmv_ring2(int dtype, int lanes, int chunks, const uint32_t *off, const uint32_t *col, const uint16_t *col16, const RingCol12 &c12,
                      const void *val, const void *x, void *y, size_t n_rows, size_t nnz, bool padded, unsigned n_blocks,
                      const uint32_t *phase_ptr, const RingPhase *phases, unsigned ring_entries, unsigned bands,
                      hipStream_t s, void *dot_partials = nullptr ,
                      unsigned block_begin = 0, unsigned block_end = ~0u ,
                      const uint32_t *reg_len = nullptr );
int launch_ring_regular(const uint32_t *off, const RingPhase *phases, size_t n_phases, uint32_t *reg_len, hipStream_t s);
int launch_tile_intervals(const uint32_t *off, const uint32_t *col, size_t n_rows, size_t tile_rows, size_t max_width,
                          uint32_t *win, uint32_t *d_count, hipStream_t s);
int launch_ring_band_codes(const uint32_t *off, const uint32_t *col, const uint32_t *win, size_t n_rows, uint32_t S,
                           uint16_t *code, hipStream_t s);
int launch_narrow_columns(const uint32_t *col, size_t nnz, uint16_t *col16, size_t n_out, hipStream_t s);
int launch_col12_count(const uint32_t *off, const uint32_t *col, size_t nnz, const RingPhase *phases, size_t n_phases, uint32_t *jobs,
                       unsigned long long *counts, hipStream_t s);
int launch_col12_encode(const uint32_t *col, size_t nnz, const uint32_t *jobs, size_t n_phases, size_t n_chunks_out, uint8_t *lo8,
                        uint16_t *hdr, uint32_t *escapes, unsigned long long *counts, hipStream_t s);
struct CrsStats {
    uint32_t max_row_len;
    uint32_t max_col;
    uint32_t min_col_inv;
    uint32_t bad;
};
int launch_crs_stats(const uint32_t *off, const uint32_t *col, size_t n_rows, size_t nnz, CrsStats *d_stats,
                     hipStream_t s);
void tiled_geometry(size_t n_rows, size_t n_cols, size_t nnz, int dtype, uint32_t *n_cb, uint32_t *rows_per_block, uint32_t *n_rb);
int tiled_build(::smh_crs *m);
uint32_t tiled_slice_columns(int dtype);
int columns_within_n_cols(const ::smh_crs *m, const char *what);
int tiled_array(::smh_crs *m, int which, void *out, size_t capacity_bytes, size_t *bytes_out);
int launch_spmv_tiled(::smh_crs *m, const void *x, size_t x_len, void *y, hipStream_t s);
size_t spmv_fused_dot_partials(::smh_crs *m, size_t x_len, int variant, bool any_lhs = false);
int spmv_enqueue(::smh_crs *m, const void *x, size_t x_len, void *y, int variant, hipStream_t s, void *dot_partials = nullptr,
                 const void *dot_lhs = nullptr);
int spmv_rows_granularity(::smh_crs *m, int variant, size_t *gran_out);
int spmv_enqueue_rows(::smh_crs *m, const void *x, size_t x_len, void *y, int variant, hipStream_t s, size_t row0, size_t row1,
                      void *dot_partials = nullptr, const void *dot_lhs = nullptr);
int spmv_enqueue_rows_short(::smh_crs *m, const void *x, size_t x_len, void *y, int variant, hipStream_t s, size_t row0, size_t row1);
enum class Ew { Add, Sub, Scale, Axpy, Xpby, RSubInto };
int launch_ew(int dtype, Ew op, void *x, const void *y, size_t n, double a, const void *a_dev, hipStream_t s);
int launch_dot(int dtype, const void *x, const void *y, size_t n, void *partials, void *result_dev,
               hipStream_t s, const uint32_t *rows_off = nullptr);
int launch_fold2(int dtype, const void *in, size_t count, void *partials, void *result_dev, hipStream_t s);
int launch_scale_values(int dtype, void *v, size_t n, double a, hipStream_t s);
int ensure_tri_schedule(::smh_crs *m, int uplo);
int tri_lanes(const ::smh_crs *m);
int trisolve_enqueue(::smh_crs *m, int uplo, int diag, bool scale_rhs, const void *b, void *x, const uint32_t *active, hipStream_t s);
int ilu_check(const ::smh_crs *a, const char *what);

template <typename T>
struct CgScalars {
    T rr, rr_prev, pap, alpha, beta;
    uint32_t converged;
    uint32_t active;
    uint32_t entered;
    uint32_t pad_;
    uint64_t iters;
    uint64_t iter_max;
    double tol;
};
template <template <typename> class S, typename T> constexpr bool scalars_like_cg_t() {
    return sizeof(S<T>) == sizeof(CgScalars<T>) && offsetof(S<T>, rr) == offsetof(CgScalars<T>, rr) &&
           offsetof(S<T>, converged) == offsetof(CgScalars<T>, converged) && offsetof(S<T>, iters) == offsetof(CgScalars<T>, iters);
}
template <template <typename> class S> constexpr bool scalars_like_cg() { return scalars_like_cg_t<S, float>() && scalars_like_cg_t<S, double>(); }
size_t cg_scalars_bytes(int dtype);
void cg_read_scalars(int dtype, const void *host_copy, int *converged, uint64_t *iters, double *rr);

template <typename Body>
int solve_in_batches(int dtype, hipStream_t s, size_t iter_max, size_t check_every, Body &&body, const void *d_sc, void *h_sc, int *converged,
                     size_t *iters, double *rr, bool capture = true) {
    Graph graph;
    GraphExec exec;
    t_solve_replays = 0;
    const bool may_capture = capture && iter_max > check_every && capture_enter();
    if (may_capture && hipStreamBeginCapture(s, hipStreamCaptureModeThreadLocal) == hipSuccess) {
        int crc = SMH_OK;
        for (size_t i = 0; i < check_every && crc == SMH_OK; ++i) crc = body();
        const hipError_t ce = graph.end_capture(s);
        if (crc != SMH_OK || ce != hipSuccess || !graph.get() || exec.instantiate(graph.get()) != hipSuccess)
            (void)hipGetLastError();
    } else {
        (void)hipGetLastError();
    }
    if (may_capture) capture_leave();
    auto poll = [&]() -> int {
        SMH_HIP(hipMemcpyAsync(h_sc, d_sc, cg_scalars_bytes(dtype), hipMemcpyDeviceToHost, s));
        SMH_HIP(hipStreamSynchronize(s));
        uint64_t it64 = 0;
        cg_read_scalars(dtype, h_sc, converged, &it64, rr);
        *iters = (size_t)it64;
        return SMH_OK;
    };
    auto run = [&]() -> int {
        size_t launched = 0;
        while (launched < iter_max) {
            size_t batch = iter_max - launched < check_every ? iter_max - launched : check_every;
            if (exec.get()) {
                SMH_HIP(hipGraphLaunch(exec.get(), s));
                ++t_solve_replays;
                batch = check_every;
            } else {
                for (size_t i = 0; i < batch; ++i) SMH_TRY(body());
            }
            launched += batch;
            SMH_TRY(poll());
            if (*converged) break;
        }
        if (iter_max == 0) SMH_TRY(poll());
        return SMH_OK;
    };
    const int rc = run();
    if (rc != SMH_OK) (void)hipStreamSynchronize(s);
    return rc;
}

enum class Form {
    NotTried,
    Ready,
    Refused,
};
struct MergeTable {
    Form state = Form::NotTried;
    size_t n_tiles = 0;
    DevArray<uint32_t> tile_row, tile_nz, carry_row;
    DevArray<char> carry_val;
};
struct RingPlan {
    Form state = Form::NotTried;
    bool bands_tried = false;
    unsigned blocks = 0;
    double fraction = 0.0;
    unsigned entries = kRingEntries;
    unsigned bands = 1;
    size_t n_phases = 0;
    DevArray<uint32_t> phase_ptr;
    DevArray<RingPhase> phases;
    DevArray<uint32_t> reg_len;
    bool reg_applies = false;
    DevArray<uint32_t> win;
    DevArray<uint16_t> col16;
    Form c12 = Form::NotTried;
    uint64_t c12_chunks = 0, c12_escapes = 0;
    DevArray<uint8_t> lo8;
    DevArray<uint16_t> hdr;
    DevArray<uint32_t> escapes;
};
struct StreamCodes {
    Form state = Form::NotTried;
    DevArray<uint32_t> cwin;
    DevArray<uint16_t> code;
    DevArray<uint8_t> len8;
    DevArray<uint32_t> tbase;
    uint32_t xs_chunks = 0xFFFFFFFFu, xs_end = 0;
    uint64_t odd_rows = 0;
    bool direct = false;
    bool vdict = false;
    int vdict_xs = 0;
};
struct StreamDict {
    Form state = Form::NotTried;
    uint32_t n = 0;
    DevArray<char> values;
};
struct ColBlock {
    Form state = Form::NotTried;
    uint32_t shift = 0;
    size_t blocks = 0;
    int rpt = 1;
    bool single_pass = false;
    DevArray<uint32_t> off, col;
    DevArray<char> val;
};
struct ColFused {
    Form state = Form::NotTried;
    uint32_t shift = 0, rt = 0;
    size_t blocks = 0, tiles = 0;
    DevArray<uint32_t> seg, col, tile_row;
    DevArray<uint8_t> cnt;
    DevArray<char> val;
};
struct RowSplit {
    Form state = Form::NotTried;
    ::smh_crs *long_part = nullptr, *short_part = nullptr;
    DevArray<uint32_t> rows;
    DevArray<char> y;
    size_t n_long = 0;
    hipStream_t side = nullptr;
    hipEvent_t fork = nullptr, join = nullptr;
    RowSplit() = default;
    RowSplit(RowSplit &&o) noexcept { swap(o); }
    RowSplit &operator=(RowSplit &&o) noexcept {
        RowSplit old(std::move(*this));
        swap(o);
        return *this;
    }
    ~RowSplit();
    void swap(RowSplit &o) noexcept {
        std::swap(state, o.state); std::swap(long_part, o.long_part); std::swap(short_part, o.short_part);
        std::swap(rows, o.rows); std::swap(y, o.y); std::swap(n_long, o.n_long);
        std::swap(side, o.side); std::swap(fork, o.fork); std::swap(join, o.join);
    }
};
struct Tiled {
    Form state = Form::NotTried;
    uint32_t n_cb = 0, n_rb = 0, R = 0;
    uint64_t tot = 0;
    DevArray<char> val, prod;
    DevArray<uint16_t> code, row;
    DevArray<uint32_t> tstart;
    DevArray<uint32_t> rbstart;
    DevArray<uint32_t> cptr;
    DevArray<char> chunk;
    uint32_t n_chunks = 0, max_slice_chunks = 0;
    bool dups = false;
    uint64_t n_prod = 0;
};
struct TriSchedule {
    Form state = Form::NotTried;
    size_t n_levels = 0;
    uint64_t first_no_diag = ~0ull;
    DevArray<uint32_t> rows;
    DevArray<uint32_t> level_ptr;
    DevArray<uint32_t> level;
    DevArray<uint32_t> diagpos;
    struct Launch { uint32_t level_begin, level_end, row_begin, row_end; bool small; };
    std::vector<Launch> launches;
};
constexpr uint32_t kTriSmallRows = 128;
constexpr uint32_t kTriSmallBlock = 1024;
struct StageBuf {
    DevArray<char> d;
    size_t cap = 0;
    int ensure_cap(size_t bytes) {
        if (cap >= bytes && d.get()) return SMH_OK;
        cap = 0;
        const size_t want = bytes < 256 ? 256 : bytes;
        SMH_TRY(d.alloc(want));
        cap = want;
        return SMH_OK;
    }
};
struct Knobs {
    int forced_lanes = 0;
    int forced_chunks = 0;
    int stream_rows_per_thread = 0;
    uint32_t cb_forced_shift = 0;
    int use_ring = -1;
    int use_stream_xs = -1;
    int use_stream_direct = -1;
    int use_stream_vdict = -1;
    int use_col16 = -1;
    int use_col12 = -1;
};

}

namespace smh {
uint64_t next_crs_id();
}
struct smh_crs {
    uint64_t id = smh::next_crs_id();
    uint64_t epoch = 0;
    int dtype = SMH_F32;
    int device = 0;
    size_t n_rows = 0, n_cols = 0, nnz = 0;
    size_t orphans = 0;
    bool has_first_op = false;
    uint32_t first_row = 0, first_col = 0;
    uint64_t first_val_bits = 0;
    uint32_t *d_off = nullptr;
    uint32_t *d_col = nullptr;
    void *d_val = nullptr;
    bool owns = true;
    bool no_split = false;
    hipStream_t stream = nullptr;
    uint32_t max_row_len = 0;
    uint32_t max_col = 0;
    uint32_t min_col = 0;
    uint32_t max_tile_entries = 0;
    uint32_t max_tile512_entries = 0;
    bool have_stats = false;
    double span_fraction = 0.0;
    smh::Knobs knobs;
    smh::MergeTable merge;
    smh::RingPlan ring;
    smh::StreamCodes codes;
    smh::StreamDict dict;
    smh::ColBlock cb;
    smh::ColFused cf;
    smh::RowSplit split;
    smh::Tiled tiled;
    smh::TriSchedule tri[2];
    smh::StageBuf stage_x, stage_y;
    double create_ms = 0.0, prepare_ms = 0.0;
    long long create_bytes = 0, prepare_bytes = 0;
};

struct smh_vec {
    int dtype = SMH_F32;
    int device = 0;
    size_t n = 0;
    void *d = nullptr;
    bool owns = true;
};

struct smh_mvec {
    int dtype = SMH_F32;
    int device = 0;
    size_t n = 0, k = 0, ld = 0;
    smh::DevArray<char> d;
};

namespace smh {
int cg_solve_many(::smh_crs *m, const ::smh_mvec *b, ::smh_mvec *x, double tol, size_t iter_max, size_t check_every, size_t *iters_out,
                  double *rr_out);
}

#ifndef SMH_POOL_IMPL
#define hipMalloc(p, n) (::smh::note_thread(), ::smh::pool_malloc((void **)(p), (n)))
#define hipFree(p) (::smh::note_thread(), ::smh::pool_free((void *)(p)))
#endif
```

### sparsemat_amd/csrc/spmv_dispatch.hip

```cpp
#include <cstdlib>
#include <cstring>

#include "crs_forms.hpp"

namespace smh {

static double mean_row(const smh_crs *m) { return m->n_rows ? (double)m->nnz / (double)m->n_rows : 0.0; }

static int mean_lanes(const smh_crs *m) {
    const double mean = mean_row(m);
    const double need = mean < 16.0 ? mean + 3.0 : mean;
    int lanes = 1;
    while (lanes < 64 && 4.0 * lanes < need) lanes <<= 1;
    return lanes;
}

int auto_lanes(const smh_crs *m) {
    if (m->knobs.forced_lanes) return m->knobs.forced_lanes;
    const double mean = mean_row(m);
    int lanes = mean_lanes(m);
    if (m->knobs.use_ring != 0) {
        if (mean >= 128.0) lanes = 16;
        else if (lanes > 32) lanes = 32;
        if (mean > 32.0 && m->ring.state == Form::Ready && m->ring.fraction < 0.5) lanes = 8;
    }
    return lanes;
}

static int auto_chunks(const smh_crs *m) {
    const int lanes = auto_lanes(m);
    if (m->knobs.forced_chunks) {
        if (lanes == 1) return m->knobs.forced_chunks;
        if (lanes == 2) return m->knobs.forced_chunks > 2 ? 2 : m->knobs.forced_chunks;
        return 1;
    }
    return 1;
}

uint32_t cb_shift_for(const smh_crs *m) { return m->knobs.cb_forced_shift ? m->knobs.cb_forced_shift : 19u; }
uint32_t cf_shift_for(const smh_crs *m) { return m->knobs.cb_forced_shift ? m->knobs.cb_forced_shift : 18u; }
size_t blocks_for(size_t n_cols, uint32_t shift) {
    const uint64_t w = 1ull << shift;
    const uint64_t b = ((uint64_t)n_cols + w - 1) / w;
    return (size_t)(b ? b : 1);
}
const size_t kColblockMinXBytes = 4u << 20;
static bool wants_colblock(const smh_crs *m) {
    const size_t b = blocks_for(m->n_cols, cb_shift_for(m));
    return m->n_cols * dtype_size(m->dtype) >= kColblockMinXBytes && m->span_fraction > 0.25 && b >= 2 && b <= 128;
}

static bool tiled_fits(const smh_crs *m, double min_tile = 32.0) {
    static const bool tiled_off = getenv("SMH_TILED") && atoi(getenv("SMH_TILED")) == 0;
    if (tiled_off || m->tiled.state == Form::Refused) return false;
    uint32_t n_cb = 0, R = 0, n_rb = 0;
    tiled_geometry(m->n_rows, m->n_cols, m->nnz, m->dtype, &n_cb, &R, &n_rb);
    const double tile = (double)m->nnz / (double)n_cb / (double)n_rb;
    return tile >= min_tile && (double)(n_rb + 1) * (double)n_cb * 4.0 <= (double)(1u << 30);
}

int resolve_variant(const smh_crs *m, int variant) {
    if (variant != SMH_SPMV_AUTO) return variant;
    if (wants_colblock(m)) {
        static const bool fused_off = getenv("SMH_COLBLOCK_FUSED") && atoi(getenv("SMH_COLBLOCK_FUSED")) == 0;
        if (fused_off || m->cf.state == Form::Refused || blocks_for(m->n_cols, cf_shift_for(m)) > 255) return SMH_SPMV_COLBLOCK;
        const double mean = mean_row(m);
        const double similar = 2.0 * mean + 8.0 > 128.0 ? 2.0 * mean + 8.0 : 128.0;
        if ((double)m->max_row_len <= similar) {
            const size_t blocks = blocks_for(m->n_cols, cf_shift_for(m));
            const bool pays = m->dtype == SMH_F32 ? tiled_fits(m)
                              : m->no_split       ? false
                                                  : tiled_fits(m, blocks >= 24 ? 12.0 : 32.0);
            if (pays) return SMH_SPMV_TILED;
            return SMH_SPMV_COLFUSED;
        }
        if (!m->no_split && tiled_fits(m, m->dtype == SMH_F64 && blocks_for(m->n_cols, cf_shift_for(m)) >= 24 ? 12.0 : 32.0)) return SMH_SPMV_TILED;
        static const bool split_off = getenv("SMH_COLBLOCK_SPLIT") && atoi(getenv("SMH_COLBLOCK_SPLIT")) == 0;
        const double vs = (double)dtype_size(m->dtype);
        const double sweeps = (double)blocks_for(m->n_cols, cb_shift_for(m)) * (double)m->n_rows * (4.0 + 2.0 * vs), entries = (double)m->nnz * (4.0 + vs);
        if (!split_off && !m->no_split && m->split.state != Form::Refused && sweeps >= 0.6 * entries) return SMH_SPMV_COLSPLIT;
        return SMH_SPMV_COLBLOCK;
    }
    const int lanes = mean_lanes(m);
    const double mean = mean_row(m);
    const bool short_ring_rows = mean > 8.0 && m->ring.state == Form::Ready && m->ring.fraction >= 0.5 && m->knobs.use_ring != 0;
    if (mean <= 12.0 && m->max_row_len <= 64 && !short_ring_rows) return SMH_SPMV_STREAM;
    if ((uint64_t)m->max_row_len >= 8ull * 4ull * (uint64_t)lanes && m->max_row_len > 64) return SMH_SPMV_MERGE;
    if (mean > 32.0 && mean <= 128.0 && m->ring.state == Form::Ready && m->ring.fraction < 0.5) return SMH_SPMV_STREAM;
    return SMH_SPMV_VECTOR;
}

static int launch_colblock(const smh_crs *m, const void *x, void *y, hipStream_t s) {
    for (size_t b = 0; b < m->cb.blocks; ++b)
        SMH_TRY(launch_spmv_stream_block(m->dtype, m->cb.off.get() + b * (m->n_rows + 1), m->cb.col.get(), m->cb.val.get(), x, y,
                                         m->n_rows, m->nnz, m->cb.rpt, m->cb.single_pass, b > 0, s));
    return SMH_OK;
}

static int stream_launch(smh_crs *m, const StreamCfg &c, const void *x, size_t x_len, void *y, hipStream_t s, void *dot_partials,
                         const void *dot_lhs, uint64_t t0, uint64_t t1) {
    const bool xs_ok = ((m->dtype == SMH_F64 ? x_len + 1 : ((x_len + 3) & ~(size_t)3)) >= (size_t)m->codes.xs_end) &&
                       (reinterpret_cast<uintptr_t>(x) & 15u) == 0;
    if (c.direct) {
        if (xs_ok && c.xs)
            return launch_spmv_stream_xd(m->dtype, m->d_val, x, y, m->n_rows, dot_partials, c.code, c.cwin, c.len8, c.tbase, dot_lhs, s,
                                         c.xs, t0, t1, c.dict, c.dict_high);
        return launch_spmv_stream(m->dtype, m->d_off, m->d_col, m->d_val, x, y, m->n_rows, m->nnz, m->owns, c.rpt, c.single_pass,
                                  dot_partials, nullptr, nullptr, nullptr, nullptr, dot_lhs, s, false, 0, t0, t1);
    }
    return launch_spmv_stream(m->dtype, m->d_off, m->d_col, m->d_val, x, y, m->n_rows, m->nnz, m->owns, c.rpt, c.single_pass,
                              dot_partials, c.code, c.cwin, c.len8, c.tbase, dot_lhs, s, c.small, xs_ok ? c.xs : 0, t0, t1);
}

static int launch_ring(smh_crs *m, const void *x, void *y, hipStream_t s, void *dot_partials = nullptr, unsigned b0 = 0, unsigned b1 = ~0u) {
    const char *reg_env = getenv("SMH_RING_REGULAR");
    const bool reg_off = reg_env && strcmp(reg_env, "auto") != 0 && atoi(reg_env) == 0;
    const uint32_t *reg_len = m->ring.reg_applies && !reg_off && (m->ring.lo8.get() || m->ring.col16.get()) ? m->ring.reg_len.get() : nullptr;
    return launch_spmv_ring2(m->dtype, auto_lanes(m), auto_chunks(m), m->d_off, m->d_col, m->ring.col16.get(),
                             RingCol12{m->ring.lo8.get(), m->ring.hdr.get(), m->ring.escapes.get()}, m->d_val, x, y, m->n_rows, m->nnz,
                             m->owns || m->nnz % 4 == 0, m->ring.blocks, m->ring.phase_ptr.get(), m->ring.phases.get(), m->ring.entries,
                             m->ring.bands, s, dot_partials, b0, b1, reg_len);
}

size_t spmv_fused_dot_partials(smh_crs *m, size_t x_len, int variant, bool any_lhs) {
    if (const char *e = getenv("SMH_CG_FUSED_DOT")) {
        if (atoi(e) == 0) return 0;
    }
    if (resolve_variant(m, variant) != SMH_SPMV_STREAM) return 0;
    if (!any_lhs && (m->n_rows != m->n_cols || x_len < m->n_rows)) return 0;
    StreamCfg c;
    if (stream_cfg(m, &c) != SMH_OK) return 0;
    return stream_tiles(m->n_rows, c.rpt);
}

static int x_covers_columns(const smh_crs *m, size_t x_len) {
    if (m->nnz > 0 && (size_t)m->max_col >= x_len)
        return fail(SMH_ERR_INDEX_RANGE, "index out of bounds: the len is %zu but the index is %u", x_len, m->max_col);
    return SMH_OK;
}

struct Resolved {
    int v = SMH_SPMV_AUTO;
    bool ring = false;
    StreamCfg stream;
};

static int build_forms(smh_crs *m, Resolved *r, bool eager) {
    switch (r->v) {
        case SMH_SPMV_VECTOR: return vector_uses_ring(m, &r->ring);
        case SMH_SPMV_SEQ: return SMH_OK;
        case SMH_SPMV_STREAM: return stream_cfg(m, &r->stream, eager);
        case SMH_SPMV_COLSPLIT:
            SMH_TRY(ensure_split(m));
            if (m->split.state != Form::Ready) return ensure_colblock(m);
            if (eager) {
                SMH_TRY(smh_crs_prepare(m->split.short_part, SMH_SPMV_AUTO));
                return smh_crs_prepare(m->split.long_part, SMH_SPMV_AUTO);
            }
            return SMH_OK;
        case SMH_SPMV_COLFUSED:
            SMH_TRY(ensure_colfused(m));
            return (m->cf.state == Form::Ready) ? SMH_OK : ensure_colblock(m);
        case SMH_SPMV_COLBLOCK: return ensure_colblock(m);
        case SMH_SPMV_TILED: return tiled_build(m);
        case SMH_SPMV_MERGE: return ensure_merge_ws(m);
        default: return fail(SMH_ERR_INVALID, "unknown SpMV variant %d", r->v);
    }
}

static int resolve_and_build(smh_crs *m, int variant, bool eager, Resolved *r) {
    for (;;) {
        r->v = resolve_variant(m, variant);
        const int rc = build_forms(m, r, eager);
        if (rc == SMH_OK || variant != SMH_SPMV_AUTO || rc == SMH_ERR_INDEX_RANGE || resolve_variant(m, variant) == r->v) return rc;
        clear_error();
    }
}

int prepare_forms(smh_crs *m, int variant) {
    Resolved r;
    return resolve_and_build(m, variant, true, &r);
}

int spmv_enqueue(smh_crs *m, const void *x, size_t x_len, void *y, int variant, hipStream_t s, void *dot_partials, const void *dot_lhs) {
    SMH_TRY(x_covers_columns(m, x_len));
    Resolved r;
    SMH_TRY(resolve_and_build(m, variant, false, &r));
    switch (r.v) {
        case SMH_SPMV_VECTOR:
            if (r.ring) return launch_ring(m, x, y, s);
            return launch_spmv_vector(m->dtype, auto_lanes(m), m->d_off, m->d_col, m->d_val, x, y, m->n_rows, m->nnz, s);
        case SMH_SPMV_SEQ:
            return launch_spmv_seq(m->dtype, m->d_off, m->d_col, m->d_val, x, y, m->n_rows, s);
        case SMH_SPMV_STREAM:
            return stream_launch(m, r.stream, x, x_len, y, s, dot_partials, dot_lhs, 0, ~uint64_t(0));
        case SMH_SPMV_COLSPLIT:
            if (m->split.state == Form::Ready) {
                static const bool overlap = getenv("SMH_COLSPLIT_OVERLAP") && atoi(getenv("SMH_COLSPLIT_OVERLAP")) != 0;
                hipStream_t sl = overlap ? m->split.side : s;
                if (overlap) {
                    SMH_HIP(hipEventRecord(m->split.fork, s));
                    SMH_HIP(hipStreamWaitEvent(sl, m->split.fork, 0));
// ... 102 lines not shown
```

### sparsemat_amd/csrc/spmv_ring2.hip

```cpp
#include "internal.hpp"
#include "ring_col12.hpp"

#include <atomic>
#include <type_traits>

namespace smh {

typedef uint32_t u32x4 __attribute__((ext_vector_type(4)));
typedef uint32_t u32x2 __attribute__((ext_vector_type(2)));
typedef float f32x4 __attribute__((ext_vector_type(4)));
typedef double f64x2 __attribute__((ext_vector_type(2)));

#ifndef SMH_RING2_THREADS64
#define SMH_RING2_THREADS64 1024
#endif
template <typename T, int RING> struct Ring2Cfg {
    static constexpr bool kBig = (size_t)RING * sizeof(T) > 65536;
    static constexpr int kThreads = kBig ? (sizeof(T) == 8 ? SMH_RING2_THREADS64 : 1024) : 512;
    static constexpr int kWavesPerSimd = (kBig ? 1 : 2) * (kThreads / 64) / 4;
};
#ifndef SMH_RING2_SB
#define SMH_RING2_SB 2
#endif
constexpr int kRing2SB = SMH_RING2_SB;
#ifndef SMH_RING2_SB64
#define SMH_RING2_SB64 1
#endif
#ifndef SMH_RING2_SADDR
#define SMH_RING2_SADDR 0
#endif
#if SMH_RING2_SADDR
#define SMH_R2_OFF(rel, size) ((size_t)((rel) * (size)))
#else
#define SMH_R2_OFF(rel, size) ((size_t)(rel) * (size))
#endif

template <typename T, int NCH>
struct Unit {
    uint32_t o0, o1;
    uint32_t c[NCH][4];
    T v[NCH][4];
};

template <typename T, int LANES>
__device__ __forceinline__ uint32_t lane_pos(uint32_t j, int q) {
    if constexpr (sizeof(T) == 8) return q < 2 ? 2u * j + (uint32_t)q : 2u * LANES + 2u * j + (uint32_t)(q - 2);
    else return 4u * j + (uint32_t)q;
}

enum : int { kColU32 = 0, kCol16 = 1, kCol12 = 2 };
struct ColStream {
    const void *colp;
    const uint16_t *hdrp;
    const uint16_t *table;
    const u32x2 *escapes;
};
template <typename T, int CF, int LANES>
__device__ __forceinline__ void load_chunk_nb(const ColStream &cs, const T *__restrict__ valp, uint32_t pass_rel, uint32_t j,
                                              uint32_t last_rel, uint32_t (&c)[4], T (&v)[4]) {
    const void *colp = cs.colp;
    if constexpr (sizeof(T) == 4) {
        uint32_t rel = pass_rel + 4u * j;
        rel = rel < last_rel ? rel : last_rel;
        if constexpr (CF == kCol12) {
            c[0] = __builtin_nontemporal_load(reinterpret_cast<const uint32_t *>(reinterpret_cast<const char *>(colp) + SMH_R2_OFF(rel, 1u)));
            c[1] = __builtin_nontemporal_load(reinterpret_cast<const uint16_t *>(reinterpret_cast<const char *>(cs.hdrp) + (SMH_R2_OFF(rel, 1u) >> 1)));
        } else if constexpr (CF == kCol16) {
            const u32x2 cc = __builtin_nontemporal_load(reinterpret_cast<const u32x2 *>(
                reinterpret_cast<const char *>(colp) + SMH_R2_OFF(rel, 2u)));
            c[0] = cc.x; c[1] = cc.y;
        } else {
            const u32x4 cc = __builtin_nontemporal_load(reinterpret_cast<const u32x4 *>(
                reinterpret_cast<const char *>(colp) + SMH_R2_OFF(rel, 4u)));
            c[0] = cc.x; c[1] = cc.y; c[2] = cc.z; c[3] = cc.w;
        }
        const f32x4 a = __builtin_nontemporal_load(reinterpret_cast<const f32x4 *>(
            reinterpret_cast<const char *>(valp) + SMH_R2_OFF(rel, 4u)));
        v[0] = a.x; v[1] = a.y; v[2] = a.z; v[3] = a.w;
    } else {
        uint32_t e0 = pass_rel + 2u * j, e1 = pass_rel + 2u * LANES + 2u * j;
        e0 = e0 < last_rel + 2u ? e0 : last_rel + 2u;
        e1 = e1 < last_rel + 2u ? e1 : last_rel + 2u;
        static_assert(CF != kCol12, "the compact column form is an f32 form");
        if constexpr (CF == kCol16) {
            c[0] = __builtin_nontemporal_load(reinterpret_cast<const uint32_t *>(reinterpret_cast<const char *>(colp) + SMH_R2_OFF(e0, 2u)));
            c[1] = __builtin_nontemporal_load(reinterpret_cast<const uint32_t *>(reinterpret_cast<const char *>(colp) + SMH_R2_OFF(e1, 2u)));
        } else {
            const u32x2 c0 = __builtin_nontemporal_load(reinterpret_cast<const u32x2 *>(reinterpret_cast<const char *>(colp) + SMH_R2_OFF(e0, 4u)));
            const u32x2 c1 = __builtin_nontemporal_load(reinterpret_cast<const u32x2 *>(reinterpret_cast<const char *>(colp) + SMH_R2_OFF(e1, 4u)));
            c[0] = c0.x; c[1] = c0.y; c[2] = c1.x; c[3] = c1.y;
        }
        const f64x2 a = __builtin_nontemporal_load(reinterpret_cast<const f64x2 *>(reinterpret_cast<const char *>(valp) + SMH_R2_OFF(e0, 8u)));
        const f64x2 b = __builtin_nontemporal_load(reinterpret_cast<const f64x2 *>(reinterpret_cast<const char *>(valp) + SMH_R2_OFF(e1, 8u)));
        v[0] = a.x; v[1] = a.y; v[2] = b.x; v[3] = b.y;
    }
}

template <int CF, int RING>
__device__ __forceinline__ void chunk_slots(const uint32_t (&c)[4], const ColStream &cs, uint32_t (&slot)[4]) {
    constexpr uint32_t MASK = RING - 1;
    if constexpr (CF == kCol12) {
        static_assert(RING == (int)col12::kSlots, "the compact column form holds slots of the 16384-slot ring");
        col12::decode_chunk(c[1], c[0], cs.table, slot);
        const bool escaped = col12::is_escape(c[1]);
        if (__builtin_amdgcn_ballot_w64(escaped) != 0) {
            if (escaped) {
                const u32x2 e = cs.escapes[c[0]];
                col12::unpack_escape(e.x, e.y, slot);
            }
        }
    } else {
#pragma unroll
        for (int q = 0; q < 4; ++q) {
            if constexpr (CF == kCol16) slot[q] = (q & 1) ? ((c[q >> 1] >> 16) & MASK) : (c[q >> 1] & MASK);
            else slot[q] = c[q] & MASK;
        }
    }
}

__device__ __forceinline__ float r2_fma(float a, float b, float c) { return __builtin_fmaf(a, b, c); }
__device__ __forceinline__ double r2_fma(double a, double b, double c) { return __builtin_fma(a, b, c); }

template <typename T, int NCH>
__device__ __forceinline__ void load_offsets(Unit<T, NCH> &u, const uint32_t *__restrict__ off, uint64_t base,
                                             uint64_t row_end, uint32_t lane) {
    uint64_t r0 = base + lane, r1 = base + lane + 1;
    r0 = r0 < row_end ? r0 : row_end;
    r1 = r1 < row_end ? r1 : row_end;
    u.o0 = off[r0];
    u.o1 = off[r1];
}

template <typename T, int NCH>
__device__ __forceinline__ void regular_offsets(Unit<T, NCH> &u, uint32_t e0, uint32_t L, uint64_t rb, uint64_t base, uint64_t row_end,
                                                uint32_t lane) {
    const uint32_t n = (uint32_t)(row_end - rb), d = base - rb < n ? (uint32_t)(base - rb) : n, left = n - d;
    u.o0 = e0 + (d + (lane < left ? lane : left)) * L;
    u.o1 = e0 + (d + (lane + 1u < left ? lane + 1u : left)) * L;
}

template <int LANES>
__device__ __forceinline__ void row_bounds(uint32_t o0, uint32_t o1, int t, uint32_t lane, uint32_t nnz_lim,
                                           uint32_t &s, uint32_t &e) {
    if constexpr (LANES == 1) {
        s = o0;
        e = o1;
    } else {
        constexpr int RPS = kWave / LANES;
        const int src = t * RPS + (int)(lane / LANES);
        s = (uint32_t)__shfl((int)o0, src, kWave);
        e = (uint32_t)__shfl((int)o1, src, kWave);
    }
    s = s < nnz_lim ? s : nnz_lim;
    e = e < nnz_lim ? e : nnz_lim;
}

template <typename T, int LANES, int CH, int SB, int CF>
__device__ __forceinline__ void issue_unit(Unit<T, SB * CH> &u, const ColStream &cs,
                                           const T *__restrict__ valp, uint32_t kb, uint32_t nnz_lim, uint32_t last_rel,
                                           uint32_t lane) {
    const uint32_t j = lane % LANES;
#pragma unroll
    for (int t = 0; t < SB; ++t) {
        uint32_t s, e;
        row_bounds<LANES>(u.o0, u.o1, t, lane, nnz_lim, s, e);
        s = s > kb ? s : kb;
#pragma unroll
        for (int ch = 0; ch < CH; ++ch) {
            load_chunk_nb<T, CF, LANES>(cs, valp, (s & ~3u) - kb + 4u * (uint32_t)(ch * LANES), j, last_rel, u.c[t * CH + ch], u.v[t * CH + ch]);
        }
    }
}

template <typename T, int LANES, int CH, int SB, int GM, int CF, int RING, bool DOT = false>
__device__ __forceinline__ void consume_unit(const Unit<T, SB * CH> &u, uint64_t base, uint64_t row_end,
                                             const ColStream &cs, const T *__restrict__ valp,
                                             const T *__restrict__ x, const T *ring, T *__restrict__ y, uint32_t kb,
                                             uint32_t nnz_lim, uint32_t last_rel, uint32_t lane, T *dacc = nullptr) {
    constexpr int RPS = kWave / LANES;
    const uint32_t j = lane % LANES;
    T out = T(0);
#pragma unroll
    for (int t = 0; t < SB; ++t) {
        uint32_t s, e;
        row_bounds<LANES>(u.o0, u.o1, t, lane, nnz_lim, s, e);
        s = s > kb ? s : kb;
        e = e > s ? e : s;
        const uint32_t sa = s & ~3u;
        const uint32_t lo = s - sa;
        const uint32_t len = e - sa;
        T sum = T(0);
#pragma unroll
        for (int ch = 0; ch < CH; ++ch) {
            uint32_t slot[4];
            if constexpr (GM == 1) chunk_slots<CF, RING>(u.c[t * CH + ch], cs, slot);
#pragma unroll
            for (int q = 0; q < 4; ++q) {
                const uint32_t rel = 4u * (uint32_t)(ch * LANES) + lane_pos<T, LANES>(j, q);
                const bool in = rel >= lo && rel < len;
                T xv;
                if constexpr (GM == 1) xv = ring[slot[q]];
                else if constexpr (GM == 2) xv = __builtin_nontemporal_load(&x[in ? u.c[t * CH + ch][q] : 0u]);
                else xv = x[in ? u.c[t * CH + ch][q] : 0u];
                const T f = r2_fma(u.v[t * CH + ch][q], xv, sum);
                sum = in ? f : sum;
            }
        }
        for (uint32_t pass = 4u * (uint32_t)(CH * LANES); pass + lane_pos<T, LANES>(j, 0) < len; pass += 4u * LANES) {
            uint32_t cc[4];
            T vv[4];
            load_chunk_nb<T, CF, LANES>(cs, valp, sa - kb + pass, j, last_rel, cc, vv);
            uint32_t slot[4];
            if constexpr (GM == 1) chunk_slots<CF, RING>(cc, cs, slot);
#pragma unroll
            for (int q = 0; q < 4; ++q) {
                const bool in = pass + lane_pos<T, LANES>(j, q) < len;
                T xv;
                if constexpr (GM == 1) xv = ring[slot[q]];
                else if constexpr (GM == 2) xv = __builtin_nontemporal_load(&x[in ? cc[q] : 0u]);
                else xv = x[in ? cc[q] : 0u];
                const T f = r2_fma(vv[q], xv, sum);
                sum = in ? f : sum;
            }
        }
        if constexpr (LANES == 1) {
            out = sum;
        } else {
#pragma unroll
            for (int o = LANES / 2; o > 0; o >>= 1) sum += __shfl_xor(sum, o, kWave);
            const T got = __shfl(sum, (int)((lane % RPS) * LANES), kWave);
            out = ((int)(lane / RPS) == t) ? got : out;
        }
    }
    const uint64_t row = base + lane;
    if constexpr (DOT) {
        if (lane < (uint32_t)(SB * RPS) && row < row_end && u.o1 != u.o0) *dacc = r2_fma(y[row], out, *dacc);
    } else {
        if (lane < (uint32_t)(SB * RPS) && row < row_end) y[row] = out;
    }
}

template <typename T, int LANES, int CH, int GM, int CF, int RING, bool DOT = false, bool REG = false>
__device__ __forceinline__ void phase_rows(const uint32_t *__restrict__ off, const ColStream &cols,
                                           const T *__restrict__ val, const T *__restrict__ x, const T *ring,
                                           T *__restrict__ y, uint64_t rb, uint64_t re, uint32_t nnz_lim,
                                           uint64_t last_chunk, uint32_t wave, uint32_t lane, T *dacc = nullptr, uint32_t L = 0) {
    constexpr int STEPS = LANES;
    constexpr int SBMAX = sizeof(T) == 8 ? SMH_RING2_SB64 : kRing2SB;
    constexpr int SB = STEPS < SBMAX ? STEPS : SBMAX;
    constexpr int RU = SB * (kWave / LANES);
    constexpr uint64_t STRIDE = (uint64_t)(Ring2Cfg<T, RING>::kThreads / kWave) * RU;
    uint64_t base = rb + (uint64_t)wave * RU;
    if (base >= re) return;
    const uint32_t e0 = __builtin_amdgcn_readfirstlane(off[rb]);
    uint32_t kb = e0 & ~3u;
    kb = kb < (uint32_t)last_chunk ? kb : (uint32_t)last_chunk;
    const uint32_t last_rel = (uint32_t)last_chunk - kb;
    ColStream cs = cols;
    cs.colp = reinterpret_cast<const char *>(cols.colp) + (size_t)kb * (CF == kCol12 ? 1u : CF == kCol16 ? 2u : 4u);
    if constexpr (CF == kCol12) cs.hdrp = cols.hdrp + (kb >> 2);
    const T *valp = val + kb;
    if constexpr (REG) {
        Unit<T, SB * CH> A, B;
        regular_offsets(A, e0, L, rb, base, re, lane);
        regular_offsets(B, e0, L, rb, base + STRIDE, re, lane);
        issue_unit<T, LANES, CH, SB, CF>(A, cs, valp, kb, nnz_lim, last_rel, lane);
        for (;;) {
            if (base + STRIDE >= re) {
                consume_unit<T, LANES, CH, SB, GM, CF, RING, DOT>(A, base, re, cs, valp, x, ring, y, kb, nnz_lim, last_rel, lane, dacc);
                break;
            }
            issue_unit<T, LANES, CH, SB, CF>(B, cs, valp, kb, nnz_lim, last_rel, lane);
            consume_unit<T, LANES, CH, SB, GM, CF, RING, DOT>(A, base, re, cs, valp, x, ring, y, kb, nnz_lim, last_rel, lane, dacc);
            regular_offsets(A, e0, L, rb, base + 2 * STRIDE, re, lane);
            base += STRIDE;
            if (base + STRIDE >= re) {
                consume_unit<T, LANES, CH, SB, GM, CF, RING, DOT>(B, base, re, cs, valp, x, ring, y, kb, nnz_lim, last_rel, lane, dacc);
                break;
            }
            issue_unit<T, LANES, CH, SB, CF>(A, cs, valp, kb, nnz_lim, last_rel, lane);
            consume_unit<T, LANES, CH, SB, GM, CF, RING, DOT>(B, base, re, cs, valp, x, ring, y, kb, nnz_lim, last_rel, lane, dacc);
            regular_offsets(B, e0, L, rb, base + 2 * STRIDE, re, lane);
            base += STRIDE;
        }
        return;
    }
    Unit<T, SB * CH> A, B, N;
    load_offsets(A, off, base, re, lane);
    load_offsets(B, off, base + STRIDE, re, lane);
    issue_unit<T, LANES, CH, SB, CF>(A, cs, valp, kb, nnz_lim, last_rel, lane);
    for (;;) {
        if (base + STRIDE >= re) {
            consume_unit<T, LANES, CH, SB, GM, CF, RING, DOT>(A, base, re, cs, valp, x, ring, y, kb, nnz_lim, last_rel, lane, dacc);
            break;
        }
        load_offsets(N, off, base + 2 * STRIDE, re, lane);
        issue_unit<T, LANES, CH, SB, CF>(B, cs, valp, kb, nnz_lim, last_rel, lane);
        consume_unit<T, LANES, CH, SB, GM, CF, RING, DOT>(A, base, re, cs, valp, x, ring, y, kb, nnz_lim, last_rel, lane, dacc);
        A.o0 = N.o0; A.o1 = N.o1;
        base += STRIDE;
        if (base + STRIDE >= re) {
            consume_unit<T, LANES, CH, SB, GM, CF, RING, DOT>(B, base, re, cs, valp, x, ring, y, kb, nnz_lim, last_rel, lane, dacc);
            break;
        }
        load_offsets(N, off, base + 2 * STRIDE, re, lane);
        issue_unit<T, LANES, CH, SB, CF>(A, cs, valp, kb, nnz_lim, last_rel, lane);
        consume_unit<T, LANES, CH, SB, GM, CF, RING, DOT>(B, base, re, cs, valp, x, ring, y, kb, nnz_lim, last_rel, lane, dacc);
        B.o0 = N.o0; B.o1 = N.o1;
        base += STRIDE;
    }
}

__device__ const col12::Table k_col12_table = col12::make_table();

template <typename T, int LANES, int CH, int CF, int RING, bool DOT = false, bool REGK = false>
__global__ void __launch_bounds__((Ring2Cfg<T, RING>::kThreads), (Ring2Cfg<T, RING>::kWavesPerSimd))
k_spmv_ring2(const uint32_t *__restrict__ off, const uint32_t *__restrict__ col, const uint16_t *__restrict__ col16, RingCol12 c12,
             const T *__restrict__ val, const T *__restrict__ x, T *__restrict__ y, uint32_t nnz_lim, uint64_t last_chunk,
             const uint32_t *__restrict__ phase_ptr, const RingPhase *__restrict__ phases, uint32_t bands,
             T *__restrict__ dot_partials, uint32_t lb0, uint32_t lb_n, const uint32_t *__restrict__ reg_len) {
    T dacc_v = T(0);
    T *dacc = DOT ? &dacc_v : nullptr;
    extern __shared__ __attribute__((aligned(16))) unsigned char ring_raw[];
    T *ring = reinterpret_cast<T *>(ring_raw);
    const uint32_t MASK = (bands == 4u ? (uint32_t)RING / 4u : (uint32_t)RING) - 1u;
    constexpr int kRing2Threads = Ring2Cfg<T, RING>::kThreads;
    const uint32_t per_xcd = gridDim.x >> 3;
    const uint32_t lb_rel = (blockIdx.x & 7u) * per_xcd + (blockIdx.x >> 3);
    if (lb_rel >= lb_n) return;
    const uint32_t lb = lb0 + lb_rel;
    const uint32_t wave = __builtin_amdgcn_readfirstlane(threadIdx.x / kWave);
    const uint32_t lane = threadIdx.x & (kWave - 1);
    const uint32_t p0 = phase_ptr[lb], p1 = phase_ptr[lb + 1];
    ColStream ring_cols = {CF == kCol16 ? (const void *)col16 : (const void *)col, nullptr, nullptr, nullptr};
    const ColStream wide_cols = {col, nullptr, nullptr, nullptr};
    if constexpr (CF == kCol12) {
        static_assert(kRing2Threads * sizeof(uint32_t) == sizeof(col12::Table), "one dword of the table per thread");
        uint16_t *table = reinterpret_cast<uint16_t *>(ring_raw + (size_t)RING * sizeof(T));
        reinterpret_cast<uint32_t *>(table)[threadIdx.x] = reinterpret_cast<const uint32_t *>(k_col12_table.e)[threadIdx.x];
        __syncthreads();
        ring_cols = {c12.lo8, c12.hdr, table, reinterpret_cast<const u32x2 *>(c12.escapes)};
    }
    for (uint32_t p = p0; p < p1; ++p) {
        const RingPhase ph = phases[p];
        const bool more = bands == 4u && (ph.band_hi[0] > ph.band_lo[0] || ph.band_hi[1] > ph.band_lo[1] || ph.band_hi[2] > ph.band_lo[2]);
        if (ph.load_hi > ph.load_lo || more) {
            __syncthreads();
            for (uint64_t cidx = (uint64_t)ph.load_lo + threadIdx.x; cidx < ph.load_hi; cidx += kRing2Threads)
                ring[cidx & MASK] = x[cidx];
            if (more) {
#pragma unroll
                for (uint32_t k = 0; k < 3; ++k)
                    for (uint64_t cidx = (uint64_t)ph.band_lo[k] + threadIdx.x; cidx < ph.band_hi[k]; cidx += kRing2Threads)
                        ring[(k + 1u) * (MASK + 1u) + (cidx & MASK)] = x[cidx];
            }
            __syncthreads();
        }
        if constexpr (REGK) {
            static_assert(CF != kColU32, "regular phases stream one of the narrow column forms");
            const uint32_t L = reg_len[p];
            if (L != 0)
                phase_rows<T, LANES, CH, 1, CF, RING, DOT, true>(off, ring_cols, val, x, ring, y, ph.row_begin, ph.row_end, nnz_lim,
                                                                 last_chunk, wave, lane, dacc, L);
            else
                phase_rows<T, LANES, CH, 1, CF, RING, DOT>(off, ring_cols, val, x, ring, y, ph.row_begin, ph.row_end, nnz_lim, last_chunk,
                                                           wave, lane, dacc);
        } else if (ph.use_ring == 1)
            phase_rows<T, LANES, CH, 1, CF, RING, DOT>(off, ring_cols, val, x, ring, y, ph.row_begin, ph.row_end, nnz_lim, last_chunk, wave,
                                                       lane, dacc);
        else if (ph.use_ring == 2)
            phase_rows<T, LANES, CH, 2, kColU32, RING, DOT>(off, wide_cols, val, x, ring, y, ph.row_begin, ph.row_end, nnz_lim, last_chunk, wave,
                                                          lane, dacc);
        else
            phase_rows<T, LANES, CH, 0, kColU32, RING, DOT>(off, wide_cols, val, x, ring, y, ph.row_begin, ph.row_end, nnz_lim, last_chunk, wave,
                                                          lane, dacc);
    }
    if constexpr (DOT) {
        __shared__ T s_dot[kRing2Threads / kWave];
        T d = dacc_v;
#pragma unroll
        for (int o = kWave / 2; o > 0; o >>= 1) d += __shfl_down(d, o, kWave);
        if (lane == 0) s_dot[wave] = d;
        __syncthreads();
        if (threadIdx.x == 0) {
            T t = T(0);
            for (int w = 0; w < kRing2Threads / kWave; ++w) t += s_dot[w];
            dot_partials[blockIdx.x] = t;
        }
    }
}

template <typename T>
__global__ void k_ring2_tail(const uint32_t *__restrict__ off, const uint32_t *__restrict__ col,
                             const T *__restrict__ val, const T *__restrict__ x, T *__restrict__ y, uint64_t n_rows,
                             uint64_t k_begin, uint64_t nnz) {
    if (blockIdx.x != 0 || threadIdx.x != 0) return;
    uint64_t r = n_rows - 1;
    while (r > 0 && (uint64_t)off[r] > k_begin) --r;
    for (uint64_t k = k_begin; k < nnz; ++k) {
        while ((uint64_t)off[r + 1] <= k) ++r;
        y[r] = r2_fma(val[k], x[col[k]], y[r]);
    }
}

template <typename T>
__global__ void k_ring2_tail_dot(const uint32_t *__restrict__ off, const uint32_t *__restrict__ col, const T *__restrict__ val,
                                 const T *__restrict__ x, const T *__restrict__ lhs, T *__restrict__ out, uint64_t n_rows, uint64_t k_begin,
                                 uint64_t nnz) {
    if (blockIdx.x != 0 || threadIdx.x != 0) return;
    uint64_t r = n_rows - 1;
    while (r > 0 && (uint64_t)off[r] > k_begin) --r;
    T acc = T(0);
    for (uint64_t k = k_begin; k < nnz; ++k) {
        while ((uint64_t)off[r + 1] <= k) ++r;
        acc = r2_fma(lhs[r], val[k] * x[col[k]], acc);
    }
    *out = acc;
}

__global__ void __launch_bounds__(kBlock)
k_narrow_columns(const uint32_t *__restrict__ col, uint64_t nnz, uint64_t n_out, uint16_t *__restrict__ col16) {
    for (uint64_t k = (uint64_t)blockIdx.x * blockDim.x + threadIdx.x; k < n_out; k += (uint64_t)gridDim.x * blockDim.x)
        col16[k] = k < nnz ? (uint16_t)col[k] : (uint16_t)0;
}
// ... 35 lines not shown
                       reg_len);
    SMH_HIP(hipGetLastError());
    return SMH_OK;
}

__global__ void __launch_bounds__(kBlock)
k_col12_jobs(const uint32_t *__restrict__ off, const RingPhase *__restrict__ phases, uint32_t n_phases, u32x2 *__restrict__ jobs,
             unsigned long long *__restrict__ counts) {
    const uint32_t p = blockIdx.x * blockDim.x + threadIdx.x;
    if (p >= n_phases) return;
    const uint32_t e0 = off[phases[p].row_begin], e1 = off[phases[p].row_end];
    uint32_t cb = e0 >> 2, ce = (uint32_t)(((uint64_t)e1 + 3u) >> 2);
    if (phases[p].use_ring != 1u || e1 <= e0) {
        cb = ce = 0;
    } else if (e0 & 3u) {
        uint32_t q = p;
        while (q > 0 && off[phases[q - 1].row_begin] == e0) --q;
        if (q > 0 && phases[q - 1].use_ring == 1u) ++cb;
    }
    jobs[p] = u32x2{cb, ce > cb ? ce : cb};
    if (ce > cb) atomicAdd(&counts[0], (unsigned long long)(ce - cb));
}

template <bool COUNT>
__global__ void __launch_bounds__(kBlock)
k_col12_encode(const uint32_t *__restrict__ col, uint64_t nnz, const u32x2 *__restrict__ jobs, uint32_t n_jobs, uint32_t *__restrict__ lo,
               uint16_t *__restrict__ hdr, u32x2 *__restrict__ escapes, unsigned long long *__restrict__ counts) {
    unsigned long long mine = 0;
    for (uint32_t job = blockIdx.x; job < n_jobs; job += gridDim.x) {
        const u32x2 range = jobs[job];
        for (uint64_t c = (uint64_t)range.x + threadIdx.x; c < range.y; c += kBlock) {
            uint32_t slot[4];
#pragma unroll
            for (int q = 0; q < 4; ++q) slot[q] = (4u * c + q < nnz ? col[4u * c + q] : 0u) & (col12::kSlots - 1u);
            uint16_t h = 0;
            uint32_t l = 0;
            const bool ok = col12::encode_chunk(slot, &h, &l);
            if constexpr (COUNT) {
                mine += ok ? 0u : 1u;
            } else {
                if (!ok) {
                    l = (uint32_t)atomicAdd(&counts[1], 1ull);
                    h = (uint16_t)col12::kEscape;
                    uint32_t pair[2];
                    col12::pack_escape(slot, pair);
                    escapes[l] = u32x2{pair[0], pair[1]};
                }
                lo[c] = l;
                hdr[c] = h;
            }
        }
    }
    if constexpr (COUNT) {
        if (mine) atomicAdd(&counts[1], mine);
    }
}

int launch_col12_count(const uint32_t *off, const uint32_t *col, size_t nnz, const RingPhase *phases, size_t n_phases, uint32_t *jobs,
                       unsigned long long *counts, hipStream_t s) {
    SMH_HIP(hipMemsetAsync(counts, 0, 2 * sizeof(unsigned long long), s));
    if (n_phases == 0) return SMH_OK;
    hipLaunchKernelGGL(k_col12_jobs, dim3((unsigned)((n_phases + kBlock - 1) / kBlock)), dim3(kBlock), 0, s, off, phases, (uint32_t)n_phases,
                       reinterpret_cast<u32x2 *>(jobs), counts);
    SMH_HIP(hipGetLastError());
    hipLaunchKernelGGL(k_col12_encode<true>, dim3((unsigned)(n_phases < 8192 ? n_phases : 8192)), dim3(kBlock), 0, s, col, (uint64_t)nnz,
                       reinterpret_cast<const u32x2 *>(jobs), (uint32_t)n_phases, (uint32_t *)nullptr, (uint16_t *)nullptr, (u32x2 *)nullptr, counts);
    SMH_HIP(hipGetLastError());
    return SMH_OK;
}

int launch_col12_encode(const uint32_t *col, size_t nnz, const uint32_t *jobs, size_t n_phases, size_t n_chunks_out, uint8_t *lo8,
                        uint16_t *hdr, uint32_t *escapes, unsigned long long *counts, hipStream_t s) {
    SMH_HIP(hipMemsetAsync(lo8, 0, n_chunks_out * 4, s));
    SMH_HIP(hipMemsetAsync(hdr, 0, n_chunks_out * sizeof(uint16_t), s));
    SMH_HIP(hipMemsetAsync(counts + 1, 0, sizeof(unsigned long long), s));
    if (n_phases == 0) return SMH_OK;
    hipLaunchKernelGGL(k_col12_encode<false>, dim3((unsigned)(n_phases < 8192 ? n_phases : 8192)), dim3(kBlock), 0, s, col, (uint64_t)nnz,
                       reinterpret_cast<const u32x2 *>(jobs), (uint32_t)n_phases, reinterpret_cast<uint32_t *>(lo8), hdr,
                       reinterpret_cast<u32x2 *>(escapes), counts);
    SMH_HIP(hipGetLastError());
    return SMH_OK;
}

template <typename T, int RING>
static int launch_ring2_t(int lanes, int chunks, const uint32_t *off, const uint32_t *col, const uint16_t *col16, const RingCol12 &c12, const T *val,
                          const T *x, T *y, size_t n_rows, size_t nnz, bool padded, unsigned n_blocks,
                          const uint32_t *phase_ptr, const RingPhase *phases, uint32_t bands, T *dot_partials, hipStream_t s,
                          unsigned block_begin, unsigned block_end, const uint32_t *reg_len) {
    if (bands == 4u && !col16) return fail(SMH_ERR_INVALID, "banded ring plan without the 16-bit slot array");
    constexpr bool kHasCol12 = std::is_same<T, float>::value && RING == (int)col12::kSlots;
    if (c12.lo8 && (!kHasCol12 || bands != 1u || !c12.hdr || !c12.escapes))
        return fail(SMH_ERR_INVALID, "ring kernel: the compact column form is for f32 on the single-window ring of 16384 columns");
    const unsigned lb0 = block_begin < n_blocks ? block_begin : n_blocks, lb1 = block_end < n_blocks ? block_end : n_blocks;
    const bool whole = lb0 == 0 && lb1 == n_blocks;
    if (!whole && dot_partials) return fail(SMH_ERR_INVALID, "ring kernel: the DOT form takes the whole plan");
    if (lb1 <= lb0) return SMH_OK;
    const uint64_t nnz_lim = padded ? nnz : (nnz & ~uint64_t(3));
    if (dot_partials) SMH_HIP(hipMemsetAsync(dot_partials, 0, ((size_t)n_blocks + 1) * sizeof(T), s));
    if (nnz_lim == 0) {
        if (!dot_partials && lb1 == n_blocks) SMH_HIP(hipMemsetAsync(y, 0, n_rows * sizeof(T), s));
    } else {
        const uint64_t last_chunk = (nnz_lim - 1) & ~uint64_t(3);
        dim3 grid(((lb1 - lb0) + 7u) & ~7u), block(Ring2Cfg<T, RING>::kThreads);
        constexpr size_t ring_bytes = (size_t)RING * sizeof(T);
#define SMH_R2_LAUNCH2(L, C, N, D, R)                                                                                    \
    do {                                                                                                                 \
        constexpr size_t lds_bytes = ring_bytes + ((N) == kCol12 ? sizeof(col12::Table) : 0);                            \
                  \
        static std::atomic<uint64_t> attr_mask{0};                                                                       \
        const uint64_t dev_bit = 1ull << (unsigned)(current_device() & 63);                                              \
        if (!(attr_mask.load(std::memory_order_acquire) & dev_bit)) {                                                    \
            SMH_HIP(hipFuncSetAttribute(reinterpret_cast<const void *>(&k_spmv_ring2<T, L, C, N, RING, D, R>),            \
                                        hipFuncAttributeMaxDynamicSharedMemorySize, (int)lds_bytes));                    \
            attr_mask.fetch_or(dev_bit, std::memory_order_release);                                                      \
        }                                                                                                                \
        hipLaunchKernelGGL((k_spmv_ring2<T, L, C, N, RING, D, R>), grid, block, lds_bytes, s, off, col, col16, c12, val, x, y, \
                           (uint32_t)nnz_lim, last_chunk, phase_ptr, phases, bands, dot_partials, (uint32_t)lb0,         \
                           (uint32_t)(lb1 - lb0), reg_len);                                                              \
    } while (0)
#define SMH_R2_LAUNCH1(L, C, N, R)                                                               \
    do {                                                                                         \
        if (dot_partials) SMH_R2_LAUNCH2(L, C, N, true, R); else SMH_R2_LAUNCH2(L, C, N, false, R); \
    } while (0)
#define SMH_R2_LAUNCH0(L, C, N)                                                                 \
    do {                                                                                        \
        if (reg_len) SMH_R2_LAUNCH1(L, C, N, true); else SMH_R2_LAUNCH1(L, C, N, false);         \
    } while (0)
#define SMH_R2_LAUNCH(L, C)                                                   \
    do {                                                                      \
        if (c12.lo8) {                                                        \
            if constexpr (kHasCol12) SMH_R2_LAUNCH0(L, C, kCol12);            \
        } else if (col16) SMH_R2_LAUNCH0(L, C, kCol16);                       \
        else SMH_R2_LAUNCH1(L, C, kColU32, false);                            \
    } while (0)
        switch (lanes * 16 + chunks) {
            case 1 * 16 + 1: SMH_R2_LAUNCH(1, 1); break;
            case 1 * 16 + 2: SMH_R2_LAUNCH(1, 2); break;
            case 1 * 16 + 3: SMH_R2_LAUNCH(1, 3); break;
            case 2 * 16 + 1: SMH_R2_LAUNCH(2, 1); break;
            case 2 * 16 + 2: SMH_R2_LAUNCH(2, 2); break;
            case 4 * 16 + 1: SMH_R2_LAUNCH(4, 1); break;
            case 8 * 16 + 1: SMH_R2_LAUNCH(8, 1); break;
            case 16 * 16 + 1: SMH_R2_LAUNCH(16, 1); break;
            case 32 * 16 + 1: SMH_R2_LAUNCH(32, 1); break;
            case 64 * 16 + 1: SMH_R2_LAUNCH(64, 1); break;
            default:
                return fail(SMH_ERR_INVALID, "ring kernel: unsupported (lanes per row, chunks per lane) = (%d, %d)", lanes, chunks);
        }
#undef SMH_R2_LAUNCH
#undef SMH_R2_LAUNCH0
#undef SMH_R2_LAUNCH1
#undef SMH_R2_LAUNCH2
        SMH_HIP(hipGetLastError());
    }
    if (nnz_lim != nnz && lb1 == n_blocks) {
        if (dot_partials)
            hipLaunchKernelGGL(k_ring2_tail_dot<T>, dim3(1), dim3(64), 0, s, off, col, val, x, (const T *)y, dot_partials + n_blocks,
                               (uint64_t)n_rows, nnz_lim, (uint64_t)nnz);
        else
            hipLaunchKernelGGL(k_ring2_tail<T>, dim3(1), dim3(64), 0, s, off, col, val, x, y, (uint64_t)n_rows, nnz_lim, (uint64_t)nnz);
        SMH_HIP(hipGetLastError());
    }
    return SMH_OK;
}

int launch_spmv_ring2(int dtype, int lanes, int chunks, const uint32_t *off, const uint32_t *col, const uint16_t *col16, const RingCol12 &c12,
                      const void *val, const void *x, void *y, size_t n_rows, size_t nnz, bool padded, unsigned n_blocks,
                      const uint32_t *phase_ptr, const RingPhase *phases, unsigned ring_entries, unsigned bands,
                      hipStream_t s, void *dot_partials, unsigned block_begin, unsigned block_end, const uint32_t *reg_len) {
    if (n_rows == 0) return SMH_OK;
    if (bands != 1u && bands != 4u) return fail(SMH_ERR_INVALID, "ring kernel: %u bands", bands);
    if (dtype == SMH_F64) {
        if (ring_entries != (unsigned)kRingEntries) return fail(SMH_ERR_INVALID, "f64 ring kernel: ring of %u columns", ring_entries);
        return launch_ring2_t<double, kRingEntries>(lanes, chunks, off, col, col16, c12, (const double *)val, (const double *)x,
                                                    (double *)y, n_rows, nnz, padded, n_blocks, phase_ptr, phases, bands,
                                                    (double *)dot_partials, s, block_begin, block_end, reg_len);
    }
    if (ring_entries == (unsigned)kRingEntriesWide)
        return launch_ring2_t<float, kRingEntriesWide>(lanes, chunks, off, col, col16, c12, (const float *)val, (const float *)x,
                                                       (float *)y, n_rows, nnz, padded, n_blocks, phase_ptr, phases, bands,
                                                       (float *)dot_partials, s, block_begin, block_end, reg_len);
    if (ring_entries != (unsigned)kRingEntries) return fail(SMH_ERR_INVALID, "ring kernel: ring of %u columns", ring_entries);
    return launch_ring2_t<float, kRingEntries>(lanes, chunks, off, col, col16, c12, (const float *)val, (const float *)x, (float *)y,
                                               n_rows, nnz, padded, n_blocks, phase_ptr, phases, bands, (float *)dot_partials, s, block_begin, block_end, reg_len);
}

}
```

### sparsemat_amd/sparsemat_crs.py

```python
import ctypes as C
import numbers

import numpy as np

from . import _lib
from ._lib import check, lib
from .densevec import DenseVec
from .multivec import MultiVec, pack_host


def _index(i):
    i = int(i)
    if not 0 <= i <= 0xFFFFFFFF:
        raise _lib.SparseMatPanic(_lib.SMH_ERR_INVALID, "index %d does not fit the u32 index type" % i)
    return i


class SparseMatCRS:
    def __init__(self, handle, dtype, keep=None):
        self._h = handle
        self._dtype = np.dtype(dtype)
        self._keep = keep

    @classmethod
# ... 451 lines not shown
                off, col, val = np.zeros(nr + 1, np.uint32), np.zeros(nnz, np.uint32), np.zeros(nnz, self._dtype)
                check(lib().smh_crs_download(h, off.ctypes.data, col.ctypes.data if nnz else None, val.ctypes.data if nnz else None))
                var, lanes = C.c_int(), C.c_int()
                check(lib().smh_crs_resolved_variant(h, C.byref(var), C.byref(lanes)))
                out[name] = (nr, off, col, val)
                out[name + "_variant"] = {1: "vector", 2: "merge", 3: "seq", 4: "stream", 5: "colblock", 6: "colfused", 7: "colsplit", 8: "tiled"}[var.value]
        return out

    def colfused(self, arrays=True):
        fits, sh, nb, rt, nt = C.c_int(), C.c_uint32(), C.c_size_t(), C.c_uint32(), C.c_size_t()
        check(lib().smh_crs_colfused(self._h, C.byref(fits), C.byref(sh), C.byref(nb), C.byref(rt), C.byref(nt), None, None, None, None, None))
        out = {"fits": bool(fits.value), "shift": sh.value, "n_blocks": nb.value, "rows_per_lane": rt.value, "n_tiles": nt.value}
        if arrays and out["fits"]:
            nnz = self.n_non_zero_entries()
            tiles = np.zeros(nt.value + 1, np.uint32)
            seg = np.zeros(nt.value * nb.value + 1, np.uint32)
            cnt = np.zeros(nt.value * nb.value * 64 * rt.value, np.uint8)
            col = np.zeros(nnz, np.uint32)
            val = np.zeros(nnz, self._dtype)
            check(lib().smh_crs_colfused(self._h, None, None, None, None, None, tiles.ctypes.data, seg.ctypes.data,
                                         cnt.ctypes.data if len(cnt) else None, col.ctypes.data if nnz else None,
                                         val.ctypes.data if nnz else None))
            out.update(tile_rows=tiles, segments=seg, counts=cnt, columns=col, values=val)
        return out

    def colblock(self, arrays=True):
        sh, nb, rpt, span = C.c_uint32(), C.c_size_t(), C.c_int(), C.c_double()
        check(lib().smh_crs_colblock(self._h, C.byref(sh), C.byref(nb), C.byref(rpt), C.byref(span), None, None, None))
        out = dict(shift=sh.value, n_blocks=nb.value, rows_per_thread=rpt.value, span_fraction=span.value)
        if arrays:
            nnz = self.n_non_zero_entries()
            off = np.zeros((nb.value, self.n_rows() + 1), dtype=np.uint32)
            col = np.zeros(nnz, dtype=np.uint32)
            val = np.zeros(nnz, dtype=self._dtype)
            check(lib().smh_crs_colblock(self._h, None, None, None, None, off.ctypes.data,
                                         col.ctypes.data if nnz else None, val.ctypes.data if nnz else None))
            out.update(offsets=off, columns=col, values=val)
        return out

    def set_vector_lanes(self, lanes):
        check(lib().smh_crs_set_vector_lanes(self._h, lanes))

    def set_stream_xs(self, mode):
        check(lib().smh_crs_set_stream_xs(self._h, mode))

    def set_stream_direct(self, mode):
        check(lib().smh_crs_set_stream_direct(self._h, mode))

    def stream_direct(self):
        a = C.c_int()
        check(lib().smh_crs_stream_direct(self._h, C.byref(a)))
        return bool(a.value)

    def stream_value_dict(self):
        n = C.c_int()
        buf = np.zeros(32, dtype=self.dtype)
        check(lib().smh_crs_stream_value_dict(self._h, C.byref(n), buf.ctypes.data))
        return buf[:n.value].copy()

    def set_stream_value_dict(self, mode):
        check(lib().smh_crs_set_stream_value_dict(self._h, int(mode)))

    def stream_layout(self):
        a, b, c, d = C.c_int(), C.c_int(), C.c_int(), C.c_int()
        check(lib().smh_crs_stream_layout(self._h, C.byref(a), C.byref(b), C.byref(c), C.byref(d)))
        return {"coded": bool(a.value), "byte_lengths": bool(b.value), "small_tiles": bool(c.value), "xs_chunks": d.value}

    def set_vector_chunks(self, chunks):
        check(lib().smh_crs_set_vector_chunks(self._h, chunks))

    def set_ring(self, mode):
        check(lib().smh_crs_set_ring(self._h, mode))

    def ring_entries(self):
        out = C.c_uint32()
        check(lib().smh_crs_ring_entries(self._h, C.byref(out)))
        return out.value

    def ring_column_form(self):
        out = C.c_int()
        check(lib().smh_crs_ring_column_form(self._h, C.byref(out)))
        return ("u32", "col16", "col12")[out.value]

    def ring_bands(self, intervals=False):
        bands = C.c_uint32()
        check(lib().smh_crs_ring_bands(self._h, C.byref(bands), None))
        if not intervals:
            return bands.value
        if bands.value != 4:
            return bands.value, None
        table = np.zeros(((self.n_rows() + 63) // 64, 4, 2), dtype=np.uint32)
        check(lib().smh_crs_ring_bands(self._h, C.byref(bands), table.ctypes.data))
        return bands.value, table

    def ring_plan(self):
        nb, nph, frac, act = C.c_uint32(), C.c_size_t(), C.c_double(), C.c_int()
        check(lib().smh_crs_ring_plan(self._h, C.byref(nb), C.byref(nph), C.byref(frac), C.byref(act), None, None))
        ptr = np.zeros(nb.value + 1, dtype=np.uint32)
        ph = np.zeros((nph.value, 11), dtype=np.uint32)
        check(lib().smh_crs_ring_plan(self._h, None, None, None, None, ptr.ctypes.data,
                                      ph.ctypes.data if nph.value else None))
        return nb.value, frac.value, bool(act.value), ptr, ph

    def ring_regular(self):
        nph = C.c_size_t()
        check(lib().smh_crs_ring_plan(self._h, None, C.byref(nph), None, None, None, None))
        out = np.zeros(nph.value, dtype=np.uint32)
        if nph.value:
            check(lib().smh_crs_ring_regular(self._h, out.ctypes.data))
        return out

    def max_row_len(self):
        out = C.c_uint32()
        check(lib().smh_crs_max_row_len(self._h, C.byref(out)))
        return out.value

    def col_range(self):
        lo, hi = C.c_uint32(), C.c_uint32()
        check(lib().smh_crs_col_range(self._h, C.byref(lo), C.byref(hi)))
        return lo.value, hi.value

    def merge_table(self):
        n = lib().smh_crs_merge_tiles(self._h)
        rows = np.zeros(n + 1, dtype=np.uint32)
        nz = np.zeros(n + 1, dtype=np.uint32)
        check(lib().smh_crs_merge_table(self._h, rows.ctypes.data, nz.ctypes.data))
        return rows, nz, lib().smh_crs_merge_tile_items(self._h)

    def mvp(self, rhs, variant="auto"):
        var = _lib.VARIANTS[variant]
        if isinstance(rhs, DenseVec):
            ret = DenseVec.zeros(self.n_rows(), self._dtype)
            check(lib().smh_crs_spmv_vec(self._h, rhs._h, ret._h, var))
            return ret
        x = np.ascontiguousarray(rhs, dtype=self._dtype)
        y = np.zeros(self.n_rows(), dtype=self._dtype)
        check(lib().smh_crs_spmv(self._h, x.ctypes.data if x.size else None, x.size,
                                 y.ctypes.data if y.size else None, var))
        return y

    def mvp_many(self, rhs):
        if isinstance(rhs, MultiVec):
            ret = MultiVec.zeros(self.n_rows(), rhs.count(), self._dtype)
            check(lib().smh_crs_spmv_many(self._h, rhs._h, ret._h))
            return ret
        x = pack_host(rhs, self._dtype)
        y = np.zeros((x.shape[0], self.n_rows()), dtype=self._dtype)
        check(lib().smh_crs_spmv_many_host(self._h, x.ctypes.data if x.size else None, x.shape[1], x.shape[0],
                                           y.ctypes.data if y.size else None))
        return y

    def mvp_many_dev(self, x_ptr, x_len, y_ptr, k, ld, stream=None):
        check(lib().smh_crs_spmv_many_dev(self._h, C.c_void_p(x_ptr), x_len, C.c_void_p(y_ptr), k, ld, C.c_void_p(stream or 0)))

    def __mul__(self, rhs):
        if isinstance(rhs, numbers.Real):
            ret = self.clone()
            ret.scale(rhs)
            return ret
        return self.mvp(rhs)

    def __imul__(self, rhs):
        if isinstance(rhs, numbers.Real):
            self.scale(rhs)
            return self
        return NotImplemented
# ... 60 lines not shown
```

Measured before the change: 8285.

## Pack ring-kernel f32 values as exact 24-bit fixed-point records with column bytes

Adds a lossless value form for the single-window col12 ring SpMV. Each f32 value is stored as a signed 24-bit integer times a shared power-of-two scale, packed with the 8-bit column low bytes into one 16-byte record per four nonzeros. The aim is to cut the HBM bytes streamed per nonzero. The form is built only when every value round-trips exactly, and it costs extra build kernels plus decode arithmetic in the hot loop.

```diff
diff --git a/include/sparsemat_hip.h b/include/sparsemat_hip.h
--- a/include/sparsemat_hip.h
+++ b/include/sparsemat_hip.h
@@ -134,6 +134,7 @@
 int smh_crs_set_ring(smh_crs *m, int mode);
 int smh_crs_ring_entries(smh_crs *m, uint32_t *out);
 int smh_crs_ring_column_form(smh_crs *m, int *form_out);
+int smh_crs_ring_values(smh_crs *m, int *form_out, int *exponent_out);
 int smh_crs_ring_bands(smh_crs *m, uint32_t *bands_out, uint32_t *intervals_out);
 int smh_crs_ring_plan(smh_crs *m, uint32_t *n_blocks_out, size_t *n_phases_out,
                       double *ring_fraction_out, int *active_out, uint32_t *phase_ptr_out,
diff --git a/rust/src/ffi.rs b/rust/src/ffi.rs
--- a/rust/src/ffi.rs
+++ b/rust/src/ffi.rs
@@ -149,6 +149,7 @@
     pub fn smh_crs_bandwidth(m: *const smh_crs, lower_out: *mut u32, upper_out: *mut u32) -> c_int;
     pub fn smh_crs_span_fraction(m: *mut smh_crs, out: *mut f64) -> c_int;
     pub fn smh_crs_ring_regular(m: *mut smh_crs, len_out: *mut u32) -> c_int;
+    pub fn smh_crs_ring_values(m: *mut smh_crs, form_out: *mut c_int, exponent_out: *mut c_int) -> c_int;
     pub fn smh_crs_rcm(m: *const smh_crs, perm_out: *mut u32, n_components_out: *mut usize, n_levels_out: *mut usize) -> c_int;
     pub fn smh_crs_rcm_dev(m: *const smh_crs, perm_out_dev: *mut u32, n_components_out: *mut usize, n_levels_out: *mut usize) -> c_int;
     pub fn smh_crs_color(m: *const smh_crs, seed: u32, colors_out: *mut u32, perm_out: *mut u32, n_colors_out: *mut usize, n_rounds_out: *mut usize) -> c_int;
diff --git a/sparsemat_amd/_lib.py b/sparsemat_amd/_lib.py
--- a/sparsemat_amd/_lib.py
+++ b/sparsemat_amd/_lib.py
@@ -102,6 +102,7 @@
     "smh_crs_set_ring": (_int, [_vp, _int]),
     "smh_crs_ring_entries": (_int, [_vp, _u32p]),
     "smh_crs_ring_column_form": (_int, [_vp, C.POINTER(_int)]),
+    "smh_crs_ring_values": (_int, [_vp, C.POINTER(_int), C.POINTER(_int)]),
     "smh_crs_ring_bands": (_int, [_vp, _u32p, _vp]),
     "smh_crs_ring_regular": (_int, [_vp, _vp]),
     "smh_crs_ring_plan": (_int, [_vp, _u32p, C.POINTER(_sz), C.POINTER(C.c_double), C.POINTER(_int), _vp, _vp]),
diff --git a/sparsemat_amd/build.py b/sparsemat_amd/build.py
--- a/sparsemat_amd/build.py
+++ b/sparsemat_amd/build.py
@@ -6,7 +6,7 @@
 CSRC = os.path.join(HERE, "csrc")
 LIB = os.path.join(HERE, "libsparsemat_hip.so")
 SOURCES = ["capi.hip", "crs_forms.hip", "spmv_dispatch.hip", "spmv_vector.hip", "spmv_ring.hip", "spmv_ring2.hip", "spmv_stream.hip", "spmv_stream_xd.hip", "spmv_many.hip", "mvec.hip", "mvec_blas.hip", "cg_many.hip","spmv_colblock.hip", "spmv_colfused.hip", "spmv_colsplit.hip", "spmv_tiled.hip", "spmv_merge.hip", "blas1.hip", "cg.hip", "synth.hip", "assemble.hip", "matops.hip", "matadd.hip", "matupdate.hip", "matplan.hip", "par.hip", "pcg.hip", "trisolve.hip", "bicgstab.hip", "gmres.hip", "pool.hip", "transpose_bucket.hip", "permute.hip", "reorder.hip", "color.hip", "ilu.hip", "fsai.hip", "refine.hip"]
-HEADERS = [os.path.join(CSRC, "internal.hpp"), os.path.join(CSRC, "crs_forms.hpp"), os.path.join(CSRC, "mvec_tree.hpp"), os.path.join(CSRC, "ring_col12.hpp"), os.path.join(CSRC, "solver_tree.hpp"), os.path.join(CSRC, "solver_host.hpp"), os.path.join(CSRC, "precond.hpp"), os.path.join(HERE, "..", "include", "sparsemat_hip.h")]
+HEADERS = [os.path.join(CSRC, "internal.hpp"), os.path.join(CSRC, "crs_forms.hpp"), os.path.join(CSRC, "mvec_tree.hpp"), os.path.join(CSRC, "ring_col12.hpp"), os.path.join(CSRC, "ring_val24.hpp"), os.path.join(CSRC, "solver_tree.hpp"), os.path.join(CSRC, "solver_host.hpp"), os.path.join(CSRC, "precond.hpp"), os.path.join(HERE, "..", "include", "sparsemat_hip.h")]
 FLAGS = ["-O3", "-std=c++17", "--offload-arch=gfx950", "-fPIC", "-Wall", "-Wno-unused-function",
          "-fno-gpu-rdc", "-ffp-contract=off"]
 
diff --git a/sparsemat_amd/csrc/capi.hip b/sparsemat_amd/csrc/capi.hip
--- a/sparsemat_amd/csrc/capi.hip
+++ b/sparsemat_amd/csrc/capi.hip
@@ -1082,6 +1082,7 @@
         SMH_HIP(hipStreamSynchronize(m->stream));
     }
     if (m->dict.state == Form::Ready) SMH_TRY(launch_scale_values(m->dtype, m->dict.values.get(), 32, a, m->stream));
+    ring_values_changed(m);
     if (m->cb.state == Form::Ready) SMH_TRY(launch_scale_values(m->dtype, m->cb.val.get(), m->nnz, a, m->stream));
     if (m->cf.state == Form::Ready) SMH_TRY(launch_scale_values(m->dtype, m->cf.val.get(), m->nnz, a, m->stream));
     if (m->tiled.state == Form::Ready) SMH_TRY(launch_scale_values(m->dtype, m->tiled.val.get(), (size_t)m->tiled.tot, a, m->stream));
@@ -1280,7 +1281,17 @@
     if (!m || !form_out) return fail(SMH_ERR_INVALID, "NULL argument");
     bool ring = false;
     SMH_TRY(vector_uses_ring(m, &ring));
-    *form_out = !ring ? 0 : m->ring.lo8.get() ? 2 : m->ring.col16.get() ? 1 : 0;
+    *form_out = !ring ? 0 : (m->ring.lo8.get() || m->ring.rec16.get()) ? 2 : m->ring.col16.get() ? 1 : 0;
+    return SMH_OK;
+}
+
+int smh_crs_ring_values(smh_crs *m, int *form_out, int *exponent_out) {
+    if (!m || !form_out) return fail(SMH_ERR_INVALID, "NULL argument");
+    bool ring = false;
+    SMH_TRY(vector_uses_ring(m, &ring));
+    const bool rec = ring && m->ring.rec16.get();
+    *form_out = rec ? 1 : (ring && m->ring.v24 == Form::Refused) ? -1 : 0;
+    if (exponent_out) *exponent_out = rec ? m->ring.v24_exp : 0;
     return SMH_OK;
 }
 
diff --git a/sparsemat_amd/csrc/crs_forms.hip b/sparsemat_amd/csrc/crs_forms.hip
--- a/sparsemat_amd/csrc/crs_forms.hip
+++ b/sparsemat_amd/csrc/crs_forms.hip
@@ -3,6 +3,7 @@
 #include <vector>
 
 #include "crs_forms.hpp"
+#include "ring_val24.hpp"
 
 namespace smh {
 
@@ -302,11 +303,13 @@
     m->ring.lo8.reset();
     m->ring.hdr.reset();
     m->ring.escapes.reset();
+    m->ring.rec16.reset();
 }
 static int ensure_ring_col12(smh_crs *m, bool forced, bool *use) {
     RingPlan &r = m->ring;
     *use = forced || r.c12 == Form::Ready;
-    if (r.c12 != Form::NotTried && (!*use || r.lo8.get())) return SMH_OK;
+    if (r.c12 != Form::NotTried && (!*use || r.lo8.get() || r.rec16.get())) return SMH_OK;
+    r.rec16.reset();
     Scratch scr;
     uint32_t *jobs = nullptr;
     unsigned long long *d_counts = nullptr, h_counts[2] = {0, 0};
@@ -335,6 +338,45 @@
     return SMH_OK;
 }
 
+void ring_values_changed(smh_crs *m) {
+    m->ring.rec16.reset();
+    m->ring.v24 = Form::NotTried;
+    m->ring.v24_exp = 0;
+}
+static int ensure_ring_val24(smh_crs *m, bool *use) {
+    RingPlan &r = m->ring;
+    *use = r.v24 != Form::Refused;
+    if (!*use || r.rec16.get()) return SMH_OK;
+    r.v24 = Form::Refused;
+    r.v24_exp = 0;
+    *use = false;
+    Scratch scr;
+    uint32_t *jobs = nullptr;
+    unsigned long long *d_counts = nullptr, h_misses = 0;
+    uint32_t h_stats[2] = {0, 0};
+    SMH_TRY(scr.alloc(&jobs, 2 * r.n_phases));
+    SMH_TRY(scr.alloc(&d_counts, 2));
+    const float *val = (const float *)m->d_val;
+    SMH_TRY(read_back(h_stats, 2, m->stream, [&](uint32_t *d_stats) {
+        return launch_val24_count(m->d_off, val, m->nnz, r.phases.get(), r.n_phases, jobs, d_counts, d_stats, m->stream);
+    }));
+    const int E = h_stats[0] == ~0u ? 0 : (int)h_stats[0] - 1024;
+    if (h_stats[1] != 0u || !val24::exponent_ok(E)) return SMH_OK;
+    const size_t n_chunks_out = ((m->nnz + 3) >> 2) + 1;
+    DevArray<uint32_t> rec16;
+    SMH_TRY(rec16.alloc(n_chunks_out * 4));
+    SMH_TRY(read_back(d_counts, &h_misses, 1, m->stream, [&](unsigned long long *d) {
+        return launch_val24_encode(val, m->nnz, jobs, r.n_phases, n_chunks_out, r.lo8.get(), E, rec16.get(), d, m->stream);
+    }));
+    if (h_misses != 0) return SMH_OK;
+    r.rec16 = std::move(rec16);
+    r.lo8.reset();
+    r.v24 = Form::Ready;
+    r.v24_exp = E;
+    *use = true;
+    return SMH_OK;
+}
+
 int vector_uses_ring(smh_crs *m, bool *out) {
     *out = false;
     if (m->knobs.use_ring == 0 || m->n_rows == 0) return SMH_OK;
@@ -346,8 +388,15 @@
     if (const char *e = getenv("SMH_RING_COL12")) want12 = strcmp(e, "auto") == 0 ? -1 : (atoi(e) ? 1 : 0);
     const bool can12 = m->dtype == SMH_F32 && m->ring.bands == 1 && m->ring.entries == (unsigned)kRingEntries && m->nnz > 0;
     bool use12 = can12 && (want12 == 1 || (want12 < 0 && want < 0 && m->ring.fraction >= 0.25));
+    int want24 = m->knobs.use_val24;
+    if (const char *e = getenv("SMH_RING_VAL24")) want24 = strcmp(e, "auto") == 0 ? -1 : (atoi(e) ? 1 : 0);
+    const char *reg_env = getenv("SMH_RING_REGULAR");
+    const bool reg_off = reg_env && strcmp(reg_env, "auto") != 0 && atoi(reg_env) == 0;
+    bool use24 = use12 && want24 != 0 && m->ring.reg_applies && !reg_off;
+    if (!use24) m->ring.rec16.reset();
     if (use12) SMH_TRY(ensure_ring_col12(m, want12 == 1, &use12));
     if (!use12) drop_ring_col12(m);
+    if (use12 && use24) SMH_TRY(ensure_ring_val24(m, &use24));
     const bool use16 = m->ring.bands == 4 || want == 1 || (want < 0 && m->ring.fraction >= 0.25);
     if (use16 && !m->ring.col16.get() && m->nnz) {
         const size_t n_out = ((m->nnz + 3) & ~size_t(3)) + 4;
@@ -373,6 +422,7 @@
     m->split = RowSplit();
     m->tiled = Tiled();
     if (what == Changed::Values) m->dict.state = Form::NotTried;
+    if (what == Changed::Values || what == Changed::Order) ring_values_changed(m);
     if (what == Changed::Order) {
         m->codes = StreamCodes();
         m->ring.col16.reset();
diff --git a/sparsemat_amd/csrc/crs_forms.hpp b/sparsemat_amd/csrc/crs_forms.hpp
--- a/sparsemat_amd/csrc/crs_forms.hpp
+++ b/sparsemat_amd/csrc/crs_forms.hpp
@@ -28,6 +28,7 @@
 int vector_uses_ring(::smh_crs *m, bool *out);
 enum class Changed { Values, Order, BlockWidth };
 void invalidate(::smh_crs *m, Changed what);
+void ring_values_changed(::smh_crs *m);
 struct StreamCfg {
     int rpt = 1;
     bool single_pass = false;
diff --git a/sparsemat_amd/csrc/internal.hpp b/sparsemat_amd/csrc/internal.hpp
--- a/sparsemat_amd/csrc/internal.hpp
+++ b/sparsemat_amd/csrc/internal.hpp
@@ -448,6 +448,8 @@
     const uint8_t *lo8 = nullptr;
     const uint16_t *hdr = nullptr;
     const uint32_t *escapes = nullptr;
+    const uint32_t *rec16 = nullptr;
+    float scale = 0.0f;
 };
 int launch_spmv_ring2(int dtype, int lanes, int chunks, const uint32_t *off, const uint32_t *col, const uint16_t *col16, const RingCol12 &c12,
                       const void *val, const void *x, void *y, size_t n_rows, size_t nnz, bool padded, unsigned n_blocks,
@@ -465,6 +467,10 @@
                        unsigned long long *counts, hipStream_t s);
 int launch_col12_encode(const uint32_t *col, size_t nnz, const uint32_t *jobs, size_t n_phases, size_t n_chunks_out, uint8_t *lo8,
                         uint16_t *hdr, uint32_t *escapes, unsigned long long *counts, hipStream_t s);
+int launch_val24_count(const uint32_t *off, const float *val, size_t nnz, const RingPhase *phases, size_t n_phases, uint32_t *jobs,
+                       unsigned long long *counts, uint32_t *stats, hipStream_t s);
+int launch_val24_encode(const float *val, size_t nnz, const uint32_t *jobs, size_t n_phases, size_t n_chunks_out, const uint8_t *lo8, int exponent,
+                        uint32_t *rec16, unsigned long long *misses, hipStream_t s);
 struct CrsStats {
     uint32_t max_row_len;
     uint32_t max_col;
@@ -594,6 +600,9 @@
     DevArray<uint8_t> lo8;
     DevArray<uint16_t> hdr;
     DevArray<uint32_t> escapes;
+    Form v24 = Form::NotTried;
+    int v24_exp = 0;
+    DevArray<uint32_t> rec16;
 };
 struct StreamCodes {
     Form state = Form::NotTried;
@@ -701,6 +710,7 @@
     int use_stream_vdict = -1;
     int use_col16 = -1;
     int use_col12 = -1;
+    int use_val24 = -1;
 };
 
 }
diff --git a/sparsemat_amd/csrc/ring_val24.hpp b/sparsemat_amd/csrc/ring_val24.hpp
--- /dev/null
+++ b/sparsemat_amd/csrc/ring_val24.hpp
@@ -0,0 +1,77 @@
+#pragma once
+#include <stdint.h>
+#include <string.h>
+
+#if defined(__HIPCC__)
+#define SMH_V24_HD __host__ __device__
+#else
+#define SMH_V24_HD
+#endif
+
+namespace smh {
+namespace val24 {
+
+constexpr int kMinExp = -100, kMaxExp = 100;
+constexpr int32_t kMinK = -(1 << 23), kMaxK = (1 << 23) - 1;
+
+SMH_V24_HD inline uint32_t float_bits(float v) {
+    uint32_t b;
+    memcpy(&b, &v, sizeof b);
+    return b;
+}
+SMH_V24_HD inline float bits_float(uint32_t b) {
+    float v;
+    memcpy(&v, &b, sizeof v);
+    return v;
+}
+
+SMH_V24_HD inline bool exponent_ok(int E) { return E >= kMinExp && E <= kMaxExp; }
+SMH_V24_HD inline float scale_of(int E) { return bits_float((uint32_t)(E + 127) << 23); }
+
+SMH_V24_HD inline float decode(int32_t k, float scale) { return (float)k * scale; }
+
+SMH_V24_HD inline bool never_fits(uint32_t bits) {
+    const uint32_t e = (bits >> 23) & 255u, m = bits & 0x7FFFFFu;
+    return e == 255u || (e == 0u && m != 0u) || bits == 0x80000000u;
+}
+SMH_V24_HD inline int lowest_bit_exponent(uint32_t bits) {
+    const uint32_t sig = (bits & 0x7FFFFFu) | 0x800000u;
+    return (int)((bits >> 23) & 255u) - 127 - 23 + __builtin_ctz(sig);
+}
+
+SMH_V24_HD inline bool encode(float v, int E, int32_t *k_out) {
+    if (!exponent_ok(E) || never_fits(float_bits(v))) return false;
+    const float t = v * scale_of(-E);
+    if (!(t >= (float)kMinK && t <= (float)kMaxK)) return false;
+    const int32_t k = (int32_t)t;
+    if (float_bits(decode(k, scale_of(E))) != float_bits(v)) return false;
+    *k_out = k;
+    return true;
+}
+SMH_V24_HD inline bool fits(float v, int E) {
+    int32_t k;
+    return encode(v, E, &k);
+}
+
+SMH_V24_HD inline void pack(const int32_t (&k)[4], uint32_t (&w)[3]) {
+    const uint32_t a = (uint32_t)k[0] & 0xFFFFFFu, b = (uint32_t)k[1] & 0xFFFFFFu, c = (uint32_t)k[2] & 0xFFFFFFu, d = (uint32_t)k[3] & 0xFFFFFFu;
+    w[0] = a | b << 24;
+    w[1] = b >> 8 | c << 16;
+    w[2] = c >> 16 | d << 8;
+}
+SMH_V24_HD inline int32_t sext24(uint32_t x) { return (int32_t)(x << 8) >> 8; }
+SMH_V24_HD inline void unpack(uint32_t w0, uint32_t w1, uint32_t w2, int32_t (&k)[4]) {
+    k[0] = sext24(w0);
+    k[1] = sext24(w0 >> 24 | w1 << 8);
+    k[2] = sext24(w1 >> 16 | w2 << 16);
+    k[3] = (int32_t)w2 >> 8;
+}
+
+SMH_V24_HD inline void decode_chunk(uint32_t w0, uint32_t w1, uint32_t w2, float scale, float (&v)[4]) {
+    int32_t k[4];
+    unpack(w0, w1, w2, k);
+    for (int q = 0; q < 4; ++q) v[q] = decode(k[q], scale);
+}
+
+}
+}
diff --git a/sparsemat_amd/csrc/spmv_dispatch.hip b/sparsemat_amd/csrc/spmv_dispatch.hip
--- a/sparsemat_amd/csrc/spmv_dispatch.hip
+++ b/sparsemat_amd/csrc/spmv_dispatch.hip
@@ -1,3 +1,4 @@
+#include <cmath>
 #include <cstdlib>
 #include <cstring>
 
@@ -115,9 +116,10 @@
 static int launch_ring(smh_crs *m, const void *x, void *y, hipStream_t s, void *dot_partials = nullptr, unsigned b0 = 0, unsigned b1 = ~0u) {
     const char *reg_env = getenv("SMH_RING_REGULAR");
     const bool reg_off = reg_env && strcmp(reg_env, "auto") != 0 && atoi(reg_env) == 0;
-    const uint32_t *reg_len = m->ring.reg_applies && !reg_off && (m->ring.lo8.get() || m->ring.col16.get()) ? m->ring.reg_len.get() : nullptr;
-    return launch_spmv_ring2(m->dtype, auto_lanes(m), auto_chunks(m), m->d_off, m->d_col, m->ring.col16.get(),
-                             RingCol12{m->ring.lo8.get(), m->ring.hdr.get(), m->ring.escapes.get()}, m->d_val, x, y, m->n_rows, m->nnz,
+    const uint32_t *reg_len = m->ring.reg_applies && !reg_off && (m->ring.lo8.get() || m->ring.rec16.get() || m->ring.col16.get()) ? m->ring.reg_len.get() : nullptr;
+    const RingCol12 c12{m->ring.lo8.get(), m->ring.hdr.get(), m->ring.escapes.get(), m->ring.rec16.get(),
+                        m->ring.rec16.get() ? ldexpf(1.0f, m->ring.v24_exp) : 0.0f};
+    return launch_spmv_ring2(m->dtype, auto_lanes(m), auto_chunks(m), m->d_off, m->d_col, m->ring.col16.get(), c12, m->d_val, x, y, m->n_rows, m->nnz,
                              m->owns || m->nnz % 4 == 0, m->ring.blocks, m->ring.phase_ptr.get(), m->ring.phases.get(), m->ring.entries,
                              m->ring.bands, s, dot_partials, b0, b1, reg_len);
 }
diff --git a/sparsemat_amd/csrc/spmv_ring2.hip b/sparsemat_amd/csrc/spmv_ring2.hip
--- a/sparsemat_amd/csrc/spmv_ring2.hip
+++ b/sparsemat_amd/csrc/spmv_ring2.hip
@@ -1,5 +1,6 @@
 #include "internal.hpp"
 #include "ring_col12.hpp"
+#include "ring_val24.hpp"
 
 #include <atomic>
 #include <type_traits>
@@ -48,12 +49,14 @@
     else return 4u * j + (uint32_t)q;
 }
 
-enum : int { kColU32 = 0, kCol16 = 1, kCol12 = 2 };
+enum : int { kColU32 = 0, kCol16 = 1, kCol12 = 2, kRec16 = 3 };
+constexpr bool has_headers(int cf) { return cf == kCol12 || cf == kRec16; }
 struct ColStream {
     const void *colp;
     const uint16_t *hdrp;
     const uint16_t *table;
     const u32x2 *escapes;
+    float scale;
 };
 template <typename T, int CF, int LANES>
 __device__ __forceinline__ void load_chunk_nb(const ColStream &cs, const T *__restrict__ valp, uint32_t pass_rel, uint32_t j,
@@ -62,7 +65,16 @@
     if constexpr (sizeof(T) == 4) {
         uint32_t rel = pass_rel + 4u * j;
         rel = rel < last_rel ? rel : last_rel;
-        if constexpr (CF == kCol12) {
+        if constexpr (CF == kRec16) {
+            const u32x4 r = __builtin_nontemporal_load(reinterpret_cast<const u32x4 *>(
+                reinterpret_cast<const char *>(colp) + SMH_R2_OFF(rel, 4u)));
+            const uint32_t w0 = r.x, w1 = r.y, w2 = r.z;
+            c[0] = r.w;
+            c[1] = __builtin_nontemporal_load(reinterpret_cast<const uint16_t *>(reinterpret_cast<const char *>(cs.hdrp) + (SMH_R2_OFF(rel, 1u) >> 1)));
+            v[0] = __uint_as_float(w0); v[1] = __uint_as_float(w1); v[2] = __uint_as_float(w2);
+            v[3] = 0.0f;
+            return;
+        } else if constexpr (CF == kCol12) {
             c[0] = __builtin_nontemporal_load(reinterpret_cast<const uint32_t *>(reinterpret_cast<const char *>(colp) + SMH_R2_OFF(rel, 1u)));
             c[1] = __builtin_nontemporal_load(reinterpret_cast<const uint16_t *>(reinterpret_cast<const char *>(cs.hdrp) + (SMH_R2_OFF(rel, 1u) >> 1)));
         } else if constexpr (CF == kCol16) {
@@ -81,7 +93,7 @@
         uint32_t e0 = pass_rel + 2u * j, e1 = pass_rel + 2u * LANES + 2u * j;
         e0 = e0 < last_rel + 2u ? e0 : last_rel + 2u;
         e1 = e1 < last_rel + 2u ? e1 : last_rel + 2u;
-        static_assert(CF != kCol12, "the compact column form is an f32 form");
+        static_assert(!has_headers(CF), "the compact column form and the chunk records are f32 forms");
         if constexpr (CF == kCol16) {
             c[0] = __builtin_nontemporal_load(reinterpret_cast<const uint32_t *>(reinterpret_cast<const char *>(colp) + SMH_R2_OFF(e0, 2u)));
             c[1] = __builtin_nontemporal_load(reinterpret_cast<const uint32_t *>(reinterpret_cast<const char *>(colp) + SMH_R2_OFF(e1, 2u)));
@@ -99,7 +111,7 @@
 template <int CF, int RING>
 __device__ __forceinline__ void chunk_slots(const uint32_t (&c)[4], const ColStream &cs, uint32_t (&slot)[4]) {
     constexpr uint32_t MASK = RING - 1;
-    if constexpr (CF == kCol12) {
+    if constexpr (has_headers(CF)) {
         static_assert(RING == (int)col12::kSlots, "the compact column form holds slots of the 16384-slot ring");
         col12::decode_chunk(c[1], c[0], cs.table, slot);
         const bool escaped = col12::is_escape(c[1]);
@@ -119,6 +131,17 @@
 }
 
 __device__ __forceinline__ float r2_fma(float a, float b, float c) { return __builtin_fmaf(a, b, c); }
+
+template <typename T, int CF>
+__device__ __forceinline__ void chunk_values(const T (&v)[4], const ColStream &cs, T (&a)[4]) {
+    if constexpr (CF == kRec16) {
+        static_assert(sizeof(T) == 4, "the chunk records are an f32 form");
+        val24::decode_chunk(__float_as_uint(v[0]), __float_as_uint(v[1]), __float_as_uint(v[2]), cs.scale, a);
+    } else {
+#pragma unroll
+        for (int q = 0; q < 4; ++q) a[q] = v[q];
+    }
+}
 __device__ __forceinline__ double r2_fma(double a, double b, double c) { return __builtin_fma(a, b, c); }
 
 template <typename T, int NCH>
@@ -194,6 +217,8 @@
         for (int ch = 0; ch < CH; ++ch) {
             uint32_t slot[4];
             if constexpr (GM == 1) chunk_slots<CF, RING>(u.c[t * CH + ch], cs, slot);
+            T a[4];
+            chunk_values<T, CF>(u.v[t * CH + ch], cs, a);
 #pragma unroll
             for (int q = 0; q < 4; ++q) {
                 const uint32_t rel = 4u * (uint32_t)(ch * LANES) + lane_pos<T, LANES>(j, q);
@@ -202,7 +227,7 @@
                 if constexpr (GM == 1) xv = ring[slot[q]];
                 else if constexpr (GM == 2) xv = __builtin_nontemporal_load(&x[in ? u.c[t * CH + ch][q] : 0u]);
                 else xv = x[in ? u.c[t * CH + ch][q] : 0u];
-                const T f = r2_fma(u.v[t * CH + ch][q], xv, sum);
+                const T f = r2_fma(a[q], xv, sum);
                 sum = in ? f : sum;
             }
         }
@@ -212,6 +237,8 @@
             load_chunk_nb<T, CF, LANES>(cs, valp, sa - kb + pass, j, last_rel, cc, vv);
             uint32_t slot[4];
             if constexpr (GM == 1) chunk_slots<CF, RING>(cc, cs, slot);
+            T a[4];
+            chunk_values<T, CF>(vv, cs, a);
 #pragma unroll
             for (int q = 0; q < 4; ++q) {
                 const bool in = pass + lane_pos<T, LANES>(j, q) < len;
@@ -219,7 +246,7 @@
                 if constexpr (GM == 1) xv = ring[slot[q]];
                 else if constexpr (GM == 2) xv = __builtin_nontemporal_load(&x[in ? cc[q] : 0u]);
                 else xv = x[in ? cc[q] : 0u];
-                const T f = r2_fma(vv[q], xv, sum);
+                const T f = r2_fma(a[q], xv, sum);
                 sum = in ? f : sum;
             }
         }
@@ -258,7 +285,7 @@
     const uint32_t last_rel = (uint32_t)last_chunk - kb;
     ColStream cs = cols;
     cs.colp = reinterpret_cast<const char *>(cols.colp) + (size_t)kb * (CF == kCol12 ? 1u : CF == kCol16 ? 2u : 4u);
-    if constexpr (CF == kCol12) cs.hdrp = cols.hdrp + (kb >> 2);
+    if constexpr (has_headers(CF)) cs.hdrp = cols.hdrp + (kb >> 2);
     const T *valp = val + kb;
     if constexpr (REG) {
         Unit<T, SB * CH> A, B;
@@ -319,6 +346,7 @@
              const T *__restrict__ val, const T *__restrict__ x, T *__restrict__ y, uint32_t nnz_lim, uint64_t last_chunk,
              const uint32_t *__restrict__ phase_ptr, const RingPhase *__restrict__ phases, uint32_t bands,
              T *__restrict__ dot_partials, uint32_t lb0, uint32_t lb_n, const uint32_t *__restrict__ reg_len) {
+    static_assert(CF != kRec16 || REGK, "the chunk records are streamed by the REGK form only");
     T dacc_v = T(0);
     T *dacc = DOT ? &dacc_v : nullptr;
     extern __shared__ __attribute__((aligned(16))) unsigned char ring_raw[];
@@ -332,14 +360,14 @@
     const uint32_t wave = __builtin_amdgcn_readfirstlane(threadIdx.x / kWave);
     const uint32_t lane = threadIdx.x & (kWave - 1);
     const uint32_t p0 = phase_ptr[lb], p1 = phase_ptr[lb + 1];
-    ColStream ring_cols = {CF == kCol16 ? (const void *)col16 : (const void *)col, nullptr, nullptr, nullptr};
-    const ColStream wide_cols = {col, nullptr, nullptr, nullptr};
-    if constexpr (CF == kCol12) {
+    ColStream ring_cols = {CF == kCol16 ? (const void *)col16 : (const void *)col, nullptr, nullptr, nullptr, 0.0f};
+    const ColStream wide_cols = {col, nullptr, nullptr, nullptr, 0.0f};
+    if constexpr (has_headers(CF)) {
         static_assert(kRing2Threads * sizeof(uint32_t) == sizeof(col12::Table), "one dword of the table per thread");
         uint16_t *table = reinterpret_cast<uint16_t *>(ring_raw + (size_t)RING * sizeof(T));
         reinterpret_cast<uint32_t *>(table)[threadIdx.x] = reinterpret_cast<const uint32_t *>(k_col12_table.e)[threadIdx.x];
         __syncthreads();
-        ring_cols = {c12.lo8, c12.hdr, table, reinterpret_cast<const u32x2 *>(c12.escapes)};
+        ring_cols = {CF == kRec16 ? (const void *)c12.rec16 : (const void *)c12.lo8, c12.hdr, table, reinterpret_cast<const u32x2 *>(c12.escapes), c12.scale};
     }
     for (uint32_t p = p0; p < p1; ++p) {
         const RingPhase ph = phases[p];
@@ -541,6 +569,89 @@
     return SMH_OK;
 }
 
+__device__ __forceinline__ void val24_chunk_values(const float *__restrict__ val, uint64_t nnz, uint64_t c, float (&v)[4]) {
+    if (4u * c + 3u < nnz) {
+        const f32x4 a = *reinterpret_cast<const f32x4 *>(val + 4u * c);
+        v[0] = a.x; v[1] = a.y; v[2] = a.z; v[3] = a.w;
+    } else {
+#pragma unroll
+        for (int q = 0; q < 4; ++q) v[q] = 4u * c + q < nnz ? val[4u * c + q] : 0.0f;
+    }
+}
+
+__global__ void __launch_bounds__(kBlock)
+k_val24_count(const float *__restrict__ val, uint64_t nnz, const u32x2 *__restrict__ jobs, uint32_t n_jobs, uint32_t *__restrict__ stats) {
+    uint32_t lowest = ~0u, bad = 0u;
+    for (uint32_t job = blockIdx.x; job < n_jobs; job += gridDim.x) {
+        const u32x2 range = jobs[job];
+        for (uint64_t c = (uint64_t)range.x + threadIdx.x; c < range.y; c += kBlock) {
+            float v[4];
+            val24_chunk_values(val, nnz, c, v);
+#pragma unroll
+            for (int q = 0; q < 4; ++q) {
+                const uint32_t bits = val24::float_bits(v[q]);
+                if (val24::never_fits(bits)) bad = 1u;
+                else if (bits != 0u) {
+                    const uint32_t e = (uint32_t)(1024 + val24::lowest_bit_exponent(bits));
+                    lowest = e < lowest ? e : lowest;
+                }
+            }
+        }
+    }
+    if (lowest != ~0u) atomicMin(&stats[0], lowest);
+    if (bad) atomicOr(&stats[1], 1u);
+}
+
+__global__ void __launch_bounds__(kBlock)
+k_val24_encode(const float *__restrict__ val, uint64_t nnz, const u32x2 *__restrict__ jobs, uint32_t n_jobs, const uint32_t *__restrict__ lo,
+               int E, u32x4 *__restrict__ rec, unsigned long long *__restrict__ misses) {
+    unsigned long long mine = 0;
+    for (uint32_t job = blockIdx.x; job < n_jobs; job += gridDim.x) {
+        const u32x2 range = jobs[job];
+        for (uint64_t c = (uint64_t)range.x + threadIdx.x; c < range.y; c += kBlock) {
+            float v[4];
+            val24_chunk_values(val, nnz, c, v);
+            int32_t k[4];
+#pragma unroll
+            for (int q = 0; q < 4; ++q) {
+                k[q] = 0;
+                if (!val24::encode(v[q], E, &k[q])) ++mine;
+            }
+            uint32_t w[3];
+            val24::pack(k, w);
+            rec[c] = u32x4{w[0], w[1], w[2], lo[c]};
+        }
+    }
+    if (mine) atomicAdd(misses, mine);
+}
+
+int launch_val24_count(const uint32_t *off, const float *val, size_t nnz, const RingPhase *phases, size_t n_phases, uint32_t *jobs,
+                       unsigned long long *counts, uint32_t *stats, hipStream_t s) {
+    SMH_HIP(hipMemsetAsync(counts, 0, 2 * sizeof(unsigned long long), s));
+    SMH_HIP(hipMemsetAsync(stats, 0xFF, sizeof(uint32_t), s));
+    SMH_HIP(hipMemsetAsync(stats + 1, 0, sizeof(uint32_t), s));
+    if (n_phases == 0) return SMH_OK;
+    hipLaunchKernelGGL(k_col12_jobs, dim3((unsigned)((n_phases + kBlock - 1) / kBlock)), dim3(kBlock), 0, s, off, phases, (uint32_t)n_phases,
+                       reinterpret_cast<u32x2 *>(jobs), counts);
+    SMH_HIP(hipGetLastError());
+    hipLaunchKernelGGL(k_val24_count, dim3((unsigned)(n_phases < 8192 ? n_phases : 8192)), dim3(kBlock), 0, s, val, (uint64_t)nnz,
+                       reinterpret_cast<const u32x2 *>(jobs), (uint32_t)n_phases, stats);
+    SMH_HIP(hipGetLastError());
+    return SMH_OK;
+}
+
+int launch_val24_encode(const float *val, size_t nnz, const uint32_t *jobs, size_t n_phases, size_t n_chunks_out, const uint8_t *lo8, int exponent,
+                        uint32_t *rec16, unsigned long long *misses, hipStream_t s) {
+    SMH_HIP(hipMemsetAsync(rec16, 0, n_chunks_out * 16, s));
+    SMH_HIP(hipMemsetAsync(misses, 0, sizeof(unsigned long long), s));
+    if (n_phases == 0) return SMH_OK;
+    hipLaunchKernelGGL(k_val24_encode, dim3((unsigned)(n_phases < 8192 ? n_phases : 8192)), dim3(kBlock), 0, s, val, (uint64_t)nnz,
+                       reinterpret_cast<const u32x2 *>(jobs), (uint32_t)n_phases, reinterpret_cast<const uint32_t *>(lo8), exponent,
+                       reinterpret_cast<u32x4 *>(rec16), misses);
+    SMH_HIP(hipGetLastError());
+    return SMH_OK;
+}
+
 template <typename T, int RING>
 static int launch_ring2_t(int lanes, int chunks, const uint32_t *off, const uint32_t *col, const uint16_t *col16, const RingCol12 &c12, const T *val,
                           const T *x, T *y, size_t n_rows, size_t nnz, bool padded, unsigned n_blocks,
@@ -548,7 +659,7 @@
                           unsigned block_begin, unsigned block_end, const uint32_t *reg_len) {
     if (bands == 4u && !col16) return fail(SMH_ERR_INVALID, "banded ring plan without the 16-bit slot array");
     constexpr bool kHasCol12 = std::is_same<T, float>::value && RING == (int)col12::kSlots;
-    if (c12.lo8 && (!kHasCol12 || bands != 1u || !c12.hdr || !c12.escapes))
+    if ((c12.lo8 || c12.rec16) && (!kHasCol12 || bands != 1u || !c12.hdr || !c12.escapes))
         return fail(SMH_ERR_INVALID, "ring kernel: the compact column form is for f32 on the single-window ring of 16384 columns");
     const unsigned lb0 = block_begin < n_blocks ? block_begin : n_blocks, lb1 = block_end < n_blocks ? block_end : n_blocks;
     const bool whole = lb0 == 0 && lb1 == n_blocks;
@@ -564,7 +675,7 @@
         constexpr size_t ring_bytes = (size_t)RING * sizeof(T);
 #define SMH_R2_LAUNCH2(L, C, N, D, R)                                                                                    \
     do {                                                                                                                 \
-        constexpr size_t lds_bytes = ring_bytes + ((N) == kCol12 ? sizeof(col12::Table) : 0);                            \
+        constexpr size_t lds_bytes = ring_bytes + (has_headers(N) ? sizeof(col12::Table) : 0);                           \
                   \
         static std::atomic<uint64_t> attr_mask{0};                                                                       \
         const uint64_t dev_bit = 1ull << (unsigned)(current_device() & 63);                                              \
@@ -587,7 +698,10 @@
     } while (0)
 #define SMH_R2_LAUNCH(L, C)                                                   \
     do {                                                                      \
-        if (c12.lo8) {                                                        \
+        if (c12.rec16) {          \
+            if (!reg_len) return fail(SMH_ERR_INVALID, "ring kernel: the chunk records go with the table of regular phases"); \
+            if constexpr (kHasCol12) SMH_R2_LAUNCH1(L, C, kRec16, true);      \
+        } else if (c12.lo8) {                                                 \
             if constexpr (kHasCol12) SMH_R2_LAUNCH0(L, C, kCol12);            \
         } else if (col16) SMH_R2_LAUNCH0(L, C, kCol16);                       \
         else SMH_R2_LAUNCH1(L, C, kColU32, false);                            \
diff --git a/sparsemat_amd/sparsemat_crs.py b/sparsemat_amd/sparsemat_crs.py
--- a/sparsemat_amd/sparsemat_crs.py
+++ b/sparsemat_amd/sparsemat_crs.py
@@ -557,6 +557,11 @@
         check(lib().smh_crs_ring_column_form(self._h, C.byref(out)))
         return ("u32", "col16", "col12")[out.value]
 
+    def ring_value_form(self):
+        form, exp = C.c_int(), C.c_int()
+        check(lib().smh_crs_ring_values(self._h, C.byref(form), C.byref(exp)))
+        return ("val24", exp.value) if form.value == 1 else ("refused" if form.value < 0 else "plain", None)
+
     def ring_bands(self, intervals=False):
         bands = C.c_uint32()
         check(lib().smh_crs_ring_bands(self._h, C.byref(bands), None))
```

Measured after the change: 9497 (median of 6 runs). 14.6% higher.
